# fpthink/3D-WSIS

Measured on AMD Instinct MI355X. Metric: scenes/sec fwd+bwd ScanNet 2cm (~150k voxels) @1/8 GPU; HBM GB/s vs roofline, higher is better.
Workload: dtype f32; 1 GPU; C2: 1 synthetic ScanNet-shaped scene on 1 GPU, 2 cm voxels, fwd+bwd+AdamW step (SubMConv3d UNet 32..160 + ECC GNN + edge affinity + MultiTaskLoss); per-batch segment CSRs / edge graph and all rulebooks are rebuilt inside every step; active_voxels=153685, points=199790, superpoints=2289, edges=20054, scenes_per_gpu=1, global_batch=1, parallelism=scene-sharded dp1

## Files before the change

### 3d-wsis_amd/csrc/bn.hip

```cpp
#include <cstdlib>
#include <initializer_list>

#include "common.h"

using namespace wsis;

namespace {

constexpr int BN_ROWS_PER_THREAD = 8;
__host__ __device__ inline int bn_rows_per_wg(int Cp) {
  const int G = Cp >> 2;
  const int R = 256 / G > 1 ? 256 / G : 1;
  return R * BN_ROWS_PER_THREAD;
}
constexpr int BN_THREADS = 256;

struct f4 {
  float v[4];
};
template <typename T>
__device__ __forceinline__ float4 bn_ld4(const T* p, int64_t t) {
  if constexpr (sizeof(T) == 4) {
    return reinterpret_cast<const float4*>(p)[t];
  } else {
// ... 191 lines not shown
    __syncthreads();
  }
}

template <typename T>
__global__ __launch_bounds__(BN_THREADS) void bn_stats_partial_kernel(const T* __restrict__ x, int64_t M, int C, int Cp,
                                                                      float* __restrict__ partial) {
  __shared__ float s_a[BN_THREADS * 4];
  __shared__ float s_b[BN_THREADS * 4];
  bn_partial_body(BnStatsAcc<T>{x}, M, C, Cp, partial, s_a, s_b);
}

template <typename T>
__global__ __launch_bounds__(BN_THREADS) void bn_bwd_partial_kernel(
    const T* __restrict__ x, const T* __restrict__ dy, const float* __restrict__ mean,
    const float* __restrict__ var, const float* __restrict__ gamma, const float* __restrict__ beta, float eps,
    int relu, int64_t M, int C, int Cp, float* __restrict__ partial) {
  __shared__ float s_a[BN_THREADS * 4];
  __shared__ float s_b[BN_THREADS * 4];
  bn_partial_body(BnBwdAcc<T>{x, dy, mean, var, gamma, beta, eps, relu}, M, C, Cp, partial, s_a, s_b);
}

__device__ __forceinline__ double wave_sum_f64(double v) {
#pragma unroll
  for (int off = 32; off >= 1; off >>= 1) v += __shfl_xor(v, off, 64);
  return v;
}
__device__ __forceinline__ void bn_final_sums(const float* __restrict__ partial, int nblk, int Cp, int c, double& A,
                                              double& B) {
  double a = 0.0, b = 0.0;
#pragma unroll 8
  for (int k = threadIdx.x; k < nblk; k += 64) {
    a += partial[(int64_t)k * 2 * Cp + c];
    b += partial[(int64_t)k * 2 * Cp + Cp + c];
  }
  A = wave_sum_f64(a);
  B = wave_sum_f64(b);
}

template <typename T>
__global__ __launch_bounds__(64) void bn_stats_final_kernel(const float* __restrict__ partial, int nblk, int C,
                                                            int Cp, int64_t M, const T* __restrict__ x0,
                                                            float* __restrict__ mean,
                                                            float* __restrict__ var,
                                                            float* __restrict__ running_mean,
                                                            float* __restrict__ running_var, float momentum) {
  const int c = blockIdx.x;
  double S, Q;
  bn_final_sums(partial, nblk, Cp, c, S, Q);
  if (threadIdx.x == 0)
    bn_store_stats(bn_shifted_mean_var(S, Q, bn_pivot(x0, M, C, c), M), M, c, mean, var, running_mean, running_var,
                   momentum);
}

__global__ __launch_bounds__(64) void bn_bwd_final_kernel(const float* __restrict__ partial, int nblk, int C, int Cp,
                                                          float* __restrict__ dgamma, float* __restrict__ dbeta) {
  const int c = blockIdx.x;
  double A, B;
  bn_final_sums(partial, nblk, Cp, c, A, B);
  if (threadIdx.x == 0) {
    dbeta[c] = (float)A;
    dgamma[c] = (float)B;
  }
}

int64_t bn_small_rows() {
  static const int64_t v = [] {
    const char* e = getenv("WSIS_BN_SMALL_ROWS");
    return e ? (int64_t)atoll(e) : (int64_t)4096;
  }();
  return v;
}
constexpr int BN_SMALL_THREADS = 1024;

__device__ __forceinline__ void block_sum2_f64(double (&a)[4], double (&b)[4], double* sh) {
  const int lane = threadIdx.x & 63, wave = threadIdx.x >> 6;
#pragma unroll
  for (int off = 32; off >= 1; off >>= 1) {
#pragma unroll
    for (int e = 0; e < 4; ++e) {
      a[e] += __shfl_xor(a[e], off, 64);
      b[e] += __shfl_xor(b[e], off, 64);
    }
  }
  if (lane == 0) {
#pragma unroll
    for (int e = 0; e < 4; ++e) {
      sh[wave * 8 + e] = a[e];
      sh[wave * 8 + 4 + e] = b[e];
    }
  }
  __syncthreads();
#pragma unroll
  for (int e = 0; e < 4; ++e) {
    double sa = 0.0, sb = 0.0;
    for (int w = 0; w < BN_SMALL_THREADS / 64; ++w) {
      sa += sh[w * 8 + e];
      sb += sh[w * 8 + 4 + e];
    }
    a[e] = sa;
    b[e] = sb;
  }
}

template <class Acc>
__device__ __forceinline__ void bn_small_body(Acc& acc, int64_t M, int C, int c0, double* sh, double (&a)[4],
                                              double (&b)[4]) {
  const bool vec = (C & 3) == 0;
  acc.init(M, C, c0);
  float sa[4] = {0.f, 0.f, 0.f, 0.f}, sb[4] = {0.f, 0.f, 0.f, 0.f};
#pragma unroll 8
  for (int64_t r = threadIdx.x; r < M; r += BN_SMALL_THREADS) acc.row(r, C, c0, vec, sa, sb);
#pragma unroll
  for (int e = 0; e < 4; ++e) {
    a[e] = sa[e];
    b[e] = sb[e];
  }
  block_sum2_f64(a, b, sh);
}

template <typename T>
__global__ __launch_bounds__(BN_SMALL_THREADS) void bn_stats_small_kernel(const T* __restrict__ x, int64_t M, int C,
                                                                    float* __restrict__ mean, float* __restrict__ var,
                                                                    float* __restrict__ running_mean,
                                                                    float* __restrict__ running_var, float momentum) {
  __shared__ double sh[BN_SMALL_THREADS / 64 * 8];
  const int c0 = blockIdx.x * 4;
  BnStatsAcc<T> acc{x};
  double a[4], b[4];
  bn_small_body(acc, M, C, c0, sh, a, b);
  const float K[4] = {acc.K[0], acc.K[1], acc.K[2], acc.K[3]};
  if (threadIdx.x < 4 && c0 + (int)threadIdx.x < C) {
    const int e = threadIdx.x;
    bn_store_stats(bn_shifted_mean_var(a[e], b[e], K[e], M), M, c0 + e, mean, var, running_mean, running_var, momentum);
  }
}

template <typename T>
__global__ __launch_bounds__(BN_SMALL_THREADS) void bn_bwd_small_kernel(
    const T* __restrict__ x, const T* __restrict__ dy, const float* __restrict__ mean,
    const float* __restrict__ var, const float* __restrict__ gamma, const float* __restrict__ beta, float eps,
    int relu, int64_t M, int C, float* __restrict__ dgamma, float* __restrict__ dbeta) {
  __shared__ double sh[BN_SMALL_THREADS / 64 * 8];
  const int c0 = blockIdx.x * 4;
  BnBwdAcc<T> acc{x, dy, mean, var, gamma, beta, eps, relu};
  double a[4], b[4];
  bn_small_body(acc, M, C, c0, sh, a, b);
  if (threadIdx.x < 4 && c0 + (int)threadIdx.x < C) {
    dbeta[c0 + threadIdx.x] = (float)a[threadIdx.x];
    dgamma[c0 + threadIdx.x] = (float)b[threadIdx.x];
  }
}

constexpr int BN_FIN_CHUNKS = kBnFinChunks;

template <int NT>
__device__ __forceinline__ void bn_chunk_walk(const float* __restrict__ partial, int lo, int hi, int C, int64_t M, int c,
                                              double (&t)[NT]) {
  const int pl = threadIdx.x >> 5;
  if (c < C) {
#pragma unroll 4
    for (int b = lo + pl; b < hi; b += 8) {
      const float sf = partial[(int64_t)b * 2 * C + c];
      const float qf = partial[(int64_t)b * 2 * C + C + c];
      const double si = sf;
      t[0] += si;
      t[1] += qf;
      if constexpr (NT == 3) {
        const int64_t left = M - (int64_t)b * 32;
        t[2] += si * si * (left < 32 ? 1.0 / (double)left : 0.03125);
      }
    }
  }
}
template <int NT>
__device__ __forceinline__ void bn_lane_fold(const double (&t)[NT], bool own, double (&red)[NT][8][33], double (&T)[NT]) {
  const int cl = threadIdx.x & 31, pl = threadIdx.x >> 5;
#pragma unroll
  for (int k = 0; k < NT; ++k) red[k][pl][cl] = t[k];
  __syncthreads();
#pragma unroll
  for (int k = 0; k < NT; ++k) T[k] = 0.0;
  if (own) {
#pragma unroll
    for (int j = 0; j < 8; ++j)
#pragma unroll
      for (int k = 0; k < NT; ++k) T[k] += red[k][j][cl];
  }
}
__device__ __forceinline__ void bn_chunk_range(int nblk, int G, int g, int& lo, int& hi) {
  const int per = (nblk + G - 1) / G;
  lo = g * per;
  hi = lo + per < nblk ? lo + per : nblk;
}

template <int NT>
__device__ __forceinline__ bool bn_ticket_sum(double* __restrict__ chunk, unsigned* __restrict__ ticket, int g0, int G,
                                              int cgi, int C, int c, bool own, double (&T)[NT],
                                              double (&red)[NT][8][33], int& s_last) {
  if (own) {
    double* o = chunk + (int64_t)g0 * NT * C;
#pragma unroll
    for (int k = 0; k < NT; ++k) st_sc1(o + k * C + c, T[k]);
  }
  if (!ticket) return false;
  wait_stores_left();
  __syncthreads();
  if (threadIdx.x == 0) {
    const unsigned t = atomicAdd(ticket + cgi, 1u);
    s_last = t == (unsigned)G - 1;
    if (s_last) ticket[cgi] = 0u;
  }
  __syncthreads();
  if (!s_last) return false;
  double t2[NT];
#pragma unroll
  for (int k = 0; k < NT; ++k) t2[k] = 0.0;
  if (c < C)
    for (int g = threadIdx.x >> 5; g < G; g += 8) {
      const double* o = chunk + (int64_t)g * NT * C;
#pragma unroll
      for (int k = 0; k < NT; ++k) t2[k] += ld_sc1(o + k * C + c);
    }
  __syncthreads();
  bn_lane_fold<NT>(t2, own, red, T);
  return true;
}

template <int NT, class Finish>
__device__ __forceinline__ bool bn_chunk_stage(const float* __restrict__ partial, int nblk, int C, int64_t M,
                                               double* __restrict__ chunk, unsigned* __restrict__ ticket, int g0, int G,
                                               int cgi, double (&red)[NT][8][33], int& s_last, Finish finish) {
  const int c = cgi * 32 + (threadIdx.x & 31);
  const bool own = (threadIdx.x >> 5) == 0 && c < C;
  int lo, hi;
  bn_chunk_range(nblk, G, g0, lo, hi);
  double t[NT], T[NT];
#pragma unroll
  for (int k = 0; k < NT; ++k) t[k] = 0.0;
  bn_chunk_walk<NT>(partial, lo, hi, C, M, c, t);
  bn_lane_fold<NT>(t, own, red, T);
  if (G > 1 && !bn_ticket_sum<NT>(chunk, ticket, g0, G, cgi, C, c, own, T, red, s_last)) return false;
  if (own) finish(c, T);
  return true;
}

__device__ __forceinline__ bool bn_chunk_centred_stage(const float* __restrict__ partial, int nblk, int C, int64_t M,
                                                       double* __restrict__ chunk, float* __restrict__ mean,
                                                       float* __restrict__ var, float* __restrict__ running_mean,
                                                       float* __restrict__ running_var, float momentum,
                                                       unsigned* __restrict__ ticket, int g0, int G, int cgi,
                                                       double (&red)[3][8][33], int& s_last) {
  return bn_chunk_stage<3>(partial, nblk, C, M, chunk, ticket, g0, G, cgi, red, s_last, [&](int c, const double (&T)[3]) {
    bn_finish_centred(T[0], T[1], T[2], M, c, mean, var, running_mean, running_var, momentum);
  });
}
__device__ __forceinline__ bool bn_sum_chunk_stage(const float* __restrict__ partial, int nblk, int C,
                                                   double* __restrict__ chunk, float* dbeta, float* dgamma,
                                                   unsigned* __restrict__ ticket, int g0, int G, int cgi,
                                                   double (&red)[2][8][33], int& s_last) {
  return bn_chunk_stage<2>(partial, nblk, C, 0, chunk, ticket, g0, G, cgi, red, s_last, [&](int c, const double (&T)[2]) {
    dbeta[c] = (float)T[0];
    dgamma[c] = (float)T[1];
  });
}

__global__ __launch_bounds__(256) void bn_stats_chunk_centred_kernel(const float* __restrict__ partial, int nblk, int C,
                                                                     int64_t M, double* __restrict__ chunk,
                                                                     float* __restrict__ mean, float* __restrict__ var,
                                                                     float* __restrict__ running_mean,
                                                                     float* __restrict__ running_var, float momentum,
                                                                     unsigned* __restrict__ ticket) {
  __shared__ double red[3][8][33];
  __shared__ int s_last;
  bn_chunk_centred_stage(partial, nblk, C, M, chunk, mean, var, running_mean, running_var, momentum, ticket,
                         (int)blockIdx.x, (int)gridDim.x, (int)blockIdx.y, red, s_last);
}
__global__ __launch_bounds__(256) void bn_sum_chunk_kernel(const float* __restrict__ partial, int nblk, int C,
                                                           double* __restrict__ chunk, float* __restrict__ dbeta,
                                                           float* __restrict__ dgamma, unsigned* __restrict__ ticket) {
  __shared__ double red[2][8][33];
  __shared__ int s_last;
  bn_sum_chunk_stage(partial, nblk, C, chunk, dbeta, dgamma, ticket, (int)blockIdx.x, (int)gridDim.x, (int)blockIdx.y, red,
                     s_last);
}

__global__ __launch_bounds__(256) void bn_stats_final_centred_kernel(const double* __restrict__ chunk, int G, int C,
                                                                     int64_t M, float* __restrict__ mean,
                                                                     float* __restrict__ var,
                                                                     float* __restrict__ running_mean,
                                                                     float* __restrict__ running_var, float momentum) {
  const int lane = threadIdx.x & 63;
  const int c = blockIdx.x * 4 + (threadIdx.x >> 6);
  if (c >= C) return;
  const bool in = lane < G;
  const double S = wave_sum_f64(in ? chunk[(int64_t)lane * 3 * C + c] : 0.0);
  const double Q = wave_sum_f64(in ? chunk[(int64_t)lane * 3 * C + C + c] : 0.0);
  const double W = wave_sum_f64(in ? chunk[(int64_t)lane * 3 * C + 2 * C + c] : 0.0);
  if (lane == 0) bn_finish_centred(S, Q, W, M, c, mean, var, running_mean, running_var, momentum);
}
__global__ __launch_bounds__(256) void bn_sum_final_kernel(const double* __restrict__ chunk, int G, int C,
                                                           float* __restrict__ dbeta, float* __restrict__ dgamma) {
  const int lane = threadIdx.x & 63;
  const int c = blockIdx.x * 4 + (threadIdx.x >> 6);
  if (c >= C) return;
  const bool in = lane < G;
  const double A = wave_sum_f64(in ? chunk[(int64_t)lane * 2 * C + c] : 0.0);
  const double B = wave_sum_f64(in ? chunk[(int64_t)lane * 2 * C + C + c] : 0.0);
  if (lane == 0) {
    dbeta[c] = (float)A;
    dgamma[c] = (float)B;
  }
}


template <bool COHERENT>
__device__ __forceinline__ float bn_ld_stat(const float* p) {
  if (COHERENT) return __hip_atomic_load(p, __ATOMIC_RELAXED, __HIP_MEMORY_SCOPE_AGENT);
  return *p;
}

template <bool COHERENT, typename TI = float, typename TO = float>
__device__ __forceinline__ void bn_apply_body(const TI* __restrict__ x, const float* mean,
                                              const float* var, const float* __restrict__ gamma,
                                              const float* __restrict__ beta, float eps, int relu,
                                              TO* __restrict__ y, int64_t M, int C) {
  const int64_t total = M * C;
  if ((C & 3) == 0) {
    const int64_t total4 = total >> 2;
    const unsigned C4 = (unsigned)(C >> 2);
    const int64_t stride = (int64_t)gridDim.x * blockDim.x;
    int64_t t = blockIdx.x * (int64_t)blockDim.x + threadIdx.x;
    const bool fixed_c = (stride % C4) == 0;
    unsigned cg = (unsigned)(t % C4);
    float sc[4], mu[4], bt[4];
    auto coef = [&](unsigned g) {
#pragma unroll
      for (int e = 0; e < 4; ++e) {
        const int c = (int)g * 4 + e;
        sc[e] = bn_fwd_coef(gamma ? gamma[c] : 1.0f, bn_ld_stat<COHERENT>(var + c), eps);
        mu[e] = bn_ld_stat<COHERENT>(mean + c);
        bt[e] = beta ? beta[c] : 0.0f;
      }
    };
    coef(cg);
    auto body = [&](const float4 v) {
      float o[4] = {v.x, v.y, v.z, v.w};
#pragma unroll
      for (int e = 0; e < 4; ++e) o[e] = bn_fwd_elem(o[e], mu[e], sc[e], bt[e], relu);
      return make_float4(o[0], o[1], o[2], o[3]);
    };
    if (fixed_c) {
      for (; t + stride < total4; t += 2 * stride) {
        const float4 v0 = bn_ld4(x, t);
        const float4 v1 = bn_ld4(x, t + stride);
        bn_st4(y, t, body(v0));
        bn_st4(y, t + stride, body(v1));
      }
      if (t < total4) bn_st4(y, t, body(bn_ld4(x, t)));
    } else {
      for (; t < total4; t += stride) {
        cg = (unsigned)(t % C4);
        coef(cg);
        bn_st4(y, t, body(bn_ld4(x, t)));
      }
    }
  } else {
    for (int64_t t = blockIdx.x * (int64_t)blockDim.x + threadIdx.x; t < total;
         t += (int64_t)gridDim.x * blockDim.x) {
      const int c = (int)(t % C);
      const float sc = bn_fwd_coef(gamma ? gamma[c] : 1.0f, bn_ld_stat<COHERENT>(var + c), eps);
      y[t] = (TO)bn_fwd_elem((float)x[t], bn_ld_stat<COHERENT>(mean + c), sc, beta ? beta[c] : 0.0f, relu);
    }
  }
}

__global__ void bn_apply_kernel(const float* __restrict__ x, const float* __restrict__ mean,
                                const float* __restrict__ var, const float* __restrict__ gamma,
                                const float* __restrict__ beta, float eps, int relu, float* __restrict__ y,
                                int64_t M, int C) {
  bn_apply_body<false>(x, mean, var, gamma, beta, eps, relu, y, M, C);
}

template <typename TI, typename TO>
__global__ void bn_apply_lp_kernel(const TI* __restrict__ x, const float* __restrict__ mean,
                                   const float* __restrict__ var, const float* __restrict__ gamma,
                                   const float* __restrict__ beta, float eps, int relu, TO* __restrict__ y, int64_t M,
                                   int C) {
  bn_apply_body<false, TI, TO>(x, mean, var, gamma, beta, eps, relu, y, M, C);
}

template <typename TI>
void launch_bn_apply_lp(const void* x, const float* mean, const float* var, const float* gamma, const float* beta,
                        float eps, int relu, void* y, int out_fp32, int64_t M, int C, int grid, hipStream_t st) {
  if (out_fp32)
    hipLaunchKernelGGL((bn_apply_lp_kernel<TI, float>), dim3(grid), dim3(256), 0, st, static_cast<const TI*>(x), mean,
                       var, gamma, beta, eps, relu, static_cast<float*>(y), M, C);
  else
    hipLaunchKernelGGL((bn_apply_lp_kernel<TI, TI>), dim3(grid), dim3(256), 0, st, static_cast<const TI*>(x), mean, var,
                       gamma, beta, eps, relu, static_cast<TI*>(y), M, C);
}

template <bool COHERENT, typename T, typename TO>
__device__ __forceinline__ void bn_bwd_apply_body(const T* __restrict__ x, const T* __restrict__ dy,
                                                  const float* __restrict__ mean, const float* __restrict__ var,
                                                  const float* __restrict__ gamma, const float* __restrict__ beta,
                                                  const float* dgamma, const float* dbeta,
                                                  const T* __restrict__ addend, float eps, int relu, int training,
                                                  TO* __restrict__ dx, int64_t M, int C) {
  const int64_t total = M * C;
  const float inv_m = 1.0f / (float)M;
  const bool vec = (C & 3) == 0;
  const int W = vec ? 4 : 1;
  const int64_t totalw = total / W;
  const unsigned Cw = (unsigned)(C / W);
  const int64_t stride = (int64_t)gridDim.x * blockDim.x;
  int64_t t = blockIdx.x * (int64_t)blockDim.x + threadIdx.x;
  const bool fixed_c = (stride % Cw) == 0;
  BnBwdCoef k;
  float k1[4], k2[4];
  auto coef = [&](int c0) {
#pragma unroll
    for (int e = 0; e < 4; ++e) {
      if (e < W) {
        const int c = c0 + e;
        k.load(e, c, mean, var, gamma, beta, eps);
        k1[e] = training ? bn_ld_stat<COHERENT>(dbeta + c) * inv_m : 0.0f;
        k2[e] = training ? bn_ld_stat<COHERENT>(dgamma + c) * inv_m : 0.0f;
      }
    }
  };
  if (t < totalw) coef((int)(t % Cw) * W);
  auto one = [&](const float (&xv)[4], const float (&dv)[4], const float (&av)[4], float (&ov)[4]) {
#pragma unroll
    for (int e = 0; e < 4; ++e) {
      if (e < W)
        ov[e] = bn_bwd_dx(bn_bwd_elem(xv[e], dv[e], k, e, relu), k, e, k1[e], k2[e], training, addend != nullptr, av[e]);
    }
  };
  if (vec && fixed_c) {
    for (; t + stride < totalw; t += 2 * stride) {
      const int64_t u = t + stride;
      const f4 tx0 = ld4(x + t * 4, true), td0 = ld4(dy + t * 4, true);
      const f4 tx1 = ld4(x + u * 4, true), td1 = ld4(dy + u * 4, true);
      f4 ta0, ta1;
#pragma unroll
      for (int e = 0; e < 4; ++e) ta0.v[e] = ta1.v[e] = 0.f;
      if (addend) {
        ta0 = ld4(addend + t * 4, true);
        ta1 = ld4(addend + u * 4, true);
      }
      float o0[4], o1[4];
      one(tx0.v, td0.v, ta0.v, o0);
      one(tx1.v, td1.v, ta1.v, o1);
      bn_st4(dx, t, make_float4(o0[0], o0[1], o0[2], o0[3]));
      bn_st4(dx, u, make_float4(o1[0], o1[1], o1[2], o1[3]));
    }
  }
  for (; t < totalw; t += stride) {
    if (!fixed_c) coef((int)(t % Cw) * W);
    float xv[4], dv[4], av[4] = {0.f, 0.f, 0.f, 0.f}, ov[4];
    if (vec) {
      const f4 tx = ld4(x + t * 4, true), td = ld4(dy + t * 4, true);
#pragma unroll
      for (int e = 0; e < 4; ++e) {
        xv[e] = tx.v[e];
        dv[e] = td.v[e];
      }
      if (addend) {
        const f4 ta = ld4(addend + t * 4, true);
#pragma unroll
        for (int e = 0; e < 4; ++e) av[e] = ta.v[e];
      }
    } else {
      xv[0] = (float)x[t];
      dv[0] = (float)dy[t];
      if (addend) av[0] = (float)addend[t];
    }
    one(xv, dv, av, ov);
    if (vec)
      bn_st4(dx, t, make_float4(ov[0], ov[1], ov[2], ov[3]));
    else
      dx[t] = (TO)ov[0];
  }
}

template <typename T, typename TO>
__global__ void bn_bwd_apply_kernel(const T* __restrict__ x, const T* __restrict__ dy,
                                    const float* __restrict__ mean, const float* __restrict__ var,
                                    const float* __restrict__ gamma, const float* __restrict__ beta,
                                    const float* __restrict__ dgamma, const float* __restrict__ dbeta,
                                    const T* __restrict__ addend, float eps, int relu, int training,
                                    TO* __restrict__ dx, int64_t M, int C) {
  bn_bwd_apply_body<false>(x, dy, mean, var, gamma, beta, dgamma, dbeta, addend, eps, relu, training, dx, M, C);
}

constexpr int BN_SF_ROWS = 256;

template <int NT>
__device__ __forceinline__ void bn_small_totals(const float* __restrict__ partial, int nblk, int C, int64_t M, int G, int c,
                                                bool own, double (&red)[NT][8][33], double (&T)[NT]) {
#pragma unroll
  for (int k = 0; k < NT; ++k) T[k] = 0.0;
  for (int g = 0; g < G; ++g) {
    int lo, hi;
    bn_chunk_range(nblk, G, g, lo, hi);
    double t[NT], Tg[NT];
#pragma unroll
    for (int k = 0; k < NT; ++k) t[k] = 0.0;
    bn_chunk_walk<NT>(partial, lo, hi, C, M, c, t);
    if (g) __syncthreads();
    bn_lane_fold<NT>(t, own, red, Tg);
    if (own) {
#pragma unroll
      for (int k = 0; k < NT; ++k) {
        if (G == 1)
          T[k] = Tg[k];
        else
          T[k] += Tg[k];
      }
    }
  }
}

__global__ __launch_bounds__(256) void bn_small_finish_apply_kernel(
    const float* __restrict__ partial, int nblk, int C, int64_t M, float* __restrict__ mean, float* __restrict__ var,
    float* __restrict__ running_mean, float* __restrict__ running_var, float momentum, const float* __restrict__ x,
    const float* __restrict__ gamma, const float* __restrict__ beta, float eps, int relu, float* __restrict__ y, int G) {
  __shared__ double red[3][8][33];
  __shared__ float s_mu[32], s_sc[32], s_bt[32];
  const int cgi = blockIdx.y;
  const int cl = threadIdx.x & 31;
  const int c = cgi * 32 + cl;
  const bool own = (threadIdx.x >> 5) == 0 && c < C;
  double T[3];
  bn_small_totals<3>(partial, nblk, C, M, G, c, own, red, T);
  if (own) {
    const BnMeanVar s = bn_centred_mean_var(T[0], T[1], T[2], M);
    if (blockIdx.x == 0) bn_store_stats(s, M, c, mean, var, running_mean, running_var, momentum);
    s_mu[cl] = (float)s.mu;
    s_sc[cl] = bn_fwd_coef(gamma ? gamma[c] : 1.0f, (float)s.v, eps);
    s_bt[cl] = beta ? beta[c] : 0.0f;
  }
  __syncthreads();
  const int q4 = threadIdx.x & 7, rl = threadIdx.x >> 3;
  const int c4 = cgi * 32 + q4 * 4;
  if (c4 >= C) return;
  float mu4[4], sc4[4], bt4[4];
#pragma unroll
  for (int e = 0; e < 4; ++e) {
    mu4[e] = s_mu[q4 * 4 + e];
    sc4[e] = s_sc[q4 * 4 + e];
    bt4[e] = s_bt[q4 * 4 + e];
  }
  const int64_t r0 = (int64_t)blockIdx.x * BN_SF_ROWS;
#pragma unroll 4
  for (int it = 0; it < BN_SF_ROWS / 32; ++it) {
    const int64_t r = r0 + it * 32 + rl;
    if (r < M) {
      const float4 vx = *reinterpret_cast<const float4*>(x + r * C + c4);
      float o[4] = {vx.x, vx.y, vx.z, vx.w};
#pragma unroll
      for (int e = 0; e < 4; ++e) o[e] = bn_fwd_elem(o[e], mu4[e], sc4[e], bt4[e], relu);
      *reinterpret_cast<float4*>(y + r * C + c4) = make_float4(o[0], o[1], o[2], o[3]);
    }
  }
}

__global__ __launch_bounds__(256) void bn_small_bwd_finish_apply_kernel(
    const float* __restrict__ partial, int nblk, int C, int64_t M, const float* __restrict__ x,
    const float* __restrict__ dy, const float* __restrict__ mean, const float* __restrict__ var,
    const float* __restrict__ gamma, const float* __restrict__ beta, const float* __restrict__ addend, float eps, int relu,
    float* __restrict__ dx, float* __restrict__ dgamma, float* __restrict__ dbeta, int G) {
  __shared__ double red[2][8][33];
  __shared__ float s_k1[32], s_k2[32];
  const int cgi = blockIdx.y;
  const int cl = threadIdx.x & 31;
  const int c = cgi * 32 + cl;
  const bool own = (threadIdx.x >> 5) == 0 && c < C;
  double T[2];
  bn_small_totals<2>(partial, nblk, C, M, G, c, own, red, T);
  if (own) {
    const float db = (float)T[0], dg = (float)T[1];
    if (blockIdx.x == 0) {
      dbeta[c] = db;
      dgamma[c] = dg;
    }
    const float inv_m = 1.0f / (float)M;
    s_k1[cl] = db * inv_m;
    s_k2[cl] = dg * inv_m;
  }
  __syncthreads();
  const int q4 = threadIdx.x & 7, rl = threadIdx.x >> 3;
  const int c4 = cgi * 32 + q4 * 4;
  if (c4 >= C) return;
  BnBwdCoef k;
  float k1[4], k2[4];
#pragma unroll
  for (int e = 0; e < 4; ++e) {
    k.load(e, c4 + e, mean, var, gamma, beta, eps);
    k1[e] = s_k1[q4 * 4 + e];
    k2[e] = s_k2[q4 * 4 + e];
  }
  const int64_t r0 = (int64_t)blockIdx.x * BN_SF_ROWS;
#pragma unroll 2
  for (int it = 0; it < BN_SF_ROWS / 32; ++it) {
    const int64_t r = r0 + it * 32 + rl;
    if (r < M) {
      const float4 vx = *reinterpret_cast<const float4*>(x + r * C + c4);
      const float4 vd = *reinterpret_cast<const float4*>(dy + r * C + c4);
      float4 va = make_float4(0.f, 0.f, 0.f, 0.f);
      if (addend) va = *reinterpret_cast<const float4*>(addend + r * C + c4);
      const float xv[4] = {vx.x, vx.y, vx.z, vx.w}, dv[4] = {vd.x, vd.y, vd.z, vd.w}, av[4] = {va.x, va.y, va.z, va.w};
      float ov[4];
#pragma unroll
      for (int e = 0; e < 4; ++e)
        ov[e] = bn_bwd_dx(bn_bwd_elem(xv[e], dv[e], k, e, relu), k, e, k1[e], k2[e], 1, addend != nullptr, av[e]);
      *reinterpret_cast<float4*>(dx + r * C + c4) = make_float4(ov[0], ov[1], ov[2], ov[3]);
    }
  }
}

static int bn_small_gmax() {
  const char* e = getenv("WSIS_BN_SMALL_G");
  const int g = e ? atoi(e) : 4;
  return g < 1 ? 1 : g > 8 ? 8 : g;
}
static bool bn_small_fused_on() {
  const char* e = getenv("WSIS_BN_SMALL_FUSED");
  return !e || atoi(e) != 0;
}

int bn_nblk(int64_t M, int Cp) { return (int)ceil_div(M > 0 ? M : 1, (int64_t)bn_rows_per_wg(Cp)); }

#if WSIS_EXPERIMENTAL
constexpr int BN_POLL_SLEEP = 12;
constexpr unsigned long long BN_SPIN_LIMIT = 200000000ull;

__device__ __forceinline__ void bn_wait_published(SyncSlot* s) {
  if (threadIdx.x == 0) {
    const unsigned long long t0 = __builtin_amdgcn_s_memrealtime();
    while (__hip_atomic_load(&s->flag, __ATOMIC_RELAXED, __HIP_MEMORY_SCOPE_AGENT) == 0u) {
      __builtin_amdgcn_s_sleep(BN_POLL_SLEEP);
      if (__builtin_amdgcn_s_memrealtime() - t0 > BN_SPIN_LIMIT) {
        __hip_atomic_store(&s->err, 1u, __ATOMIC_RELAXED, __HIP_MEMORY_SCOPE_AGENT);
        break;
      }
    }
    const unsigned l = atomicAdd(&s->left, 1u);
    if (l == gridDim.x - 1) {
      __hip_atomic_store(&s->left, 0u, __ATOMIC_RELAXED, __HIP_MEMORY_SCOPE_AGENT);
      __hip_atomic_store(&s->flag, 0u, __ATOMIC_RELAXED, __HIP_MEMORY_SCOPE_AGENT);
    }
  }
  __syncthreads();
}
__device__ __forceinline__ void bn_publish(bool fin, SyncSlot* s, int CG) {
  if (!fin) return;
  __threadfence();
  __syncthreads();
  if (threadIdx.x == 0) {
    const unsigned d = atomicAdd(&s->done, 1u);
    if (d == (unsigned)CG - 1) {
      __hip_atomic_store(&s->done, 0u, __ATOMIC_RELAXED, __HIP_MEMORY_SCOPE_AGENT);
      __threadfence();
      __hip_atomic_store(&s->flag, 1u, __ATOMIC_RELEASE, __HIP_MEMORY_SCOPE_AGENT);
    }
  }
}

__global__ __launch_bounds__(256) void bn_finalize_apply_kernel(
    const float* __restrict__ partial, int nblk, int C, int64_t M, double* __restrict__ chunk, int G,
    float* mean, float* var, float* __restrict__ running_mean,
    float* __restrict__ running_var, float momentum, SyncSlot* __restrict__ sync, const float* __restrict__ x,
    const float* __restrict__ gamma, const float* __restrict__ beta, float eps, int relu, float* __restrict__ y) {
  __shared__ double red[3][8][33];
  __shared__ int s_last;
  const int CG = (C + 31) / 32;
  if ((int)blockIdx.x < G * CG)
    bn_publish(bn_chunk_centred_stage(partial, nblk, C, M, chunk, mean, var, running_mean, running_var, momentum,
                                      sync->ticket, (int)blockIdx.x % G, G, (int)blockIdx.x / G, red, s_last),
               sync, CG);
  bn_wait_published(sync);
  bn_apply_body<true>(x, mean, var, gamma, beta, eps, relu, y, M, C);
}

__global__ __launch_bounds__(256) void bn_bwd_finish_apply_kernel(
    const float* __restrict__ partial, int nblk, int C, double* __restrict__ chunk, int G, float* dbeta, float* dgamma,
    SyncSlot* __restrict__ sync, const float* __restrict__ x, const float* __restrict__ dy, const float* __restrict__ mean,
    const float* __restrict__ var, const float* __restrict__ gamma, const float* __restrict__ beta,
    const float* __restrict__ addend, float eps, int relu, float* __restrict__ dx, int64_t M) {
  __shared__ double red[2][8][33];
  __shared__ int s_last;
  const int CG = (C + 31) / 32;
  if ((int)blockIdx.x < G * CG)
    bn_publish(bn_sum_chunk_stage(partial, nblk, C, chunk, dbeta, dgamma, sync->ticket, (int)blockIdx.x % G, G,
                                  (int)blockIdx.x / G, red, s_last),
               sync, CG);
  bn_wait_published(sync);
  bn_bwd_apply_body<true>(x, dy, mean, var, gamma, beta, dgamma, dbeta, addend, eps, relu, 1, dx, M, C);
}

static int bn_fused_grid(int64_t M, int C, int need_chunk_wgs, int which = 0) {
  const char* e = getenv("WSIS_BN_FUSED_APPLY");
  const int on = e ? atoi(e) : 0;
  const char* ed = getenv(which ? "WSIS_BN_FUSED_BWD" : "WSIS_BN_FUSED_FWD");
  const int on_dir = ed ? atoi(ed) : on;
  const char* g = tune_env("WSIS_BN_FUSED_GRID");
  int gmax = g ? atoi(g) : 256;
  if (gmax < 64 || gmax > 512) gmax = 256;
  int n_cu = 0;
  {
    int dev = 0, v = 0;
    n_cu = (hipGetDevice(&dev) == hipSuccess &&
            hipDeviceGetAttribute(&v, hipDeviceAttributeMultiprocessorCount, dev) == hipSuccess) ? v : 0;
  }
  if (!on_dir || (C & 3) != 0) return 0;
  const int cw = C >> 2;
  const int64_t work = (M * C) >> 2;
  int gcap = (work > 600000 && gmax == 256) ? 512 : gmax;
  if (gcap > 2 * n_cu) gcap = 2 * n_cu;
  if (gcap < 1) return 0;
  int grid = gcap - (gcap % cw);
  const int need = grid_for(work, 256);
  if (need < grid) {
    grid = need;
    if (grid > cw) grid -= grid % cw;
  }
  return (grid >= need_chunk_wgs && grid >= 1) ? grid : 0;
}
#endif


static int bn_apply_grid(int64_t M, int C) {
  const bool vec = (C & 3) == 0;
  const int64_t work = vec ? (M * C) >> 2 : M * C;
  const int cw = vec ? C >> 2 : C;
  int64_t g = ceil_div(work, (int64_t)256 * 8);
  if (g < 512) {
    g = ceil_div(work, 256);
    if (g > 512) g = 512;
  }
  if (g > 16384) g = 16384;
  if (g < 1) g = 1;
  if (g > cw) g -= g % cw;
  return (int)g;
}

template <typename T, typename TO>
static int launch_bn_bwd_apply(const T* d_x, const T* d_dy, const float* d_mean, const float* d_var,
                               const float* d_gamma, const float* d_beta, const float* d_dgamma, const float* d_dbeta,
                               const T* d_addend, float eps, int relu, int training, TO* d_dx, int64_t M, int C,
                               hipStream_t st) {
  hipLaunchKernelGGL((bn_bwd_apply_kernel<T, TO>), dim3(bn_apply_grid(M, C)), dim3(256), 0, st, d_x, d_dy, d_mean, d_var,
                     d_gamma, d_beta, d_dgamma, d_dbeta, d_addend, eps, relu, training, d_dx, M, C);
  WSIS_LAUNCH_CHECK();
  return WSIS_OK;
}

template <typename T>
static int bn_stats_run(const T* d_x, int64_t M, int C, float* d_mean, float* d_var, float* d_running_mean,
                        float* d_running_var, float momentum, void* d_ws, hipStream_t st) {
  const int Cp = (C + 3) / 4 * 4;
  const int nblk = bn_nblk(M, Cp);
  float* partial = static_cast<float*>(d_ws);
  WSIS_REQUIRE(Cp / 4 <= BN_THREADS, "C > 1024 is not supported");
  if (M <= bn_small_rows()) {
    hipLaunchKernelGGL(bn_stats_small_kernel<T>, dim3(Cp / 4), dim3(BN_SMALL_THREADS), 0, st, d_x, M, C, d_mean, d_var,
                       d_running_mean, d_running_var, momentum);
    WSIS_LAUNCH_CHECK();
    return WSIS_OK;
  }
  hipLaunchKernelGGL(bn_stats_partial_kernel<T>, dim3(nblk), dim3(BN_THREADS), 0, st, d_x, M, C, Cp, partial);
  WSIS_LAUNCH_CHECK();
  hipLaunchKernelGGL(bn_stats_final_kernel<T>, dim3(C), dim3(64), 0, st, partial, nblk, C, Cp, M, d_x, d_mean, d_var,
                     d_running_mean, d_running_var, momentum);
  WSIS_LAUNCH_CHECK();
  return WSIS_OK;
}
template <typename T>
static int bn_bwd_reduce_run(const T* d_x, const T* d_dy, const float* d_mean, const float* d_var, const float* d_gamma,
                             const float* d_beta, float eps, int relu, float* d_dgamma, float* d_dbeta, int64_t M, int C,
                             void* d_ws, hipStream_t st) {
  const int Cp = (C + 3) / 4 * 4;
  const int nblk = bn_nblk(M, Cp);
  float* partial = static_cast<float*>(d_ws);
  WSIS_REQUIRE(Cp / 4 <= BN_THREADS, "C > 1024 is not supported");
  if (M <= bn_small_rows()) {
    hipLaunchKernelGGL(bn_bwd_small_kernel<T>, dim3(Cp / 4), dim3(BN_SMALL_THREADS), 0, st, d_x, d_dy, d_mean, d_var,
                       d_gamma, d_beta, eps, relu, M, C, d_dgamma, d_dbeta);
    WSIS_LAUNCH_CHECK();
  } else {
    hipLaunchKernelGGL(bn_bwd_partial_kernel<T>, dim3(nblk), dim3(BN_THREADS), 0, st, d_x, d_dy, d_mean, d_var, d_gamma,
                       d_beta, eps, relu, M, C, Cp, partial);
    WSIS_LAUNCH_CHECK();
    hipLaunchKernelGGL(bn_bwd_final_kernel, dim3(C), dim3(64), 0, st, partial, nblk, C, Cp, d_dgamma, d_dbeta);
    WSIS_LAUNCH_CHECK();
  }
  return WSIS_OK;
}
template <typename T>
static int bn_bwd_apply_lp_run(const void* d_x, const void* d_dy, const float* d_mean, const float* d_var,
                               const float* d_gamma, const float* d_beta, const float* d_dgamma, const float* d_dbeta,
                               const void* d_addend, float eps, int relu, int training, void* d_dx, int out_fp32, int64_t M,
                               int C, hipStream_t st) {
  const T *x = static_cast<const T*>(d_x), *dy = static_cast<const T*>(d_dy), *ad = static_cast<const T*>(d_addend);
  if (out_fp32)
    return launch_bn_bwd_apply(x, dy, d_mean, d_var, d_gamma, d_beta, d_dgamma, d_dbeta, ad, eps, relu, training,
                               static_cast<float*>(d_dx), M, C, st);
  return launch_bn_bwd_apply(x, dy, d_mean, d_var, d_gamma, d_beta, d_dgamma, d_dbeta, ad, eps, relu, training,
                             static_cast<T*>(d_dx), M, C, st);
}
template <typename T>
static int bn_bwd_lp_run(const void* d_x, const void* d_dy, const float* d_mean, const float* d_var, const float* d_gamma,
                         const float* d_beta, float eps, int relu, int training, void* d_dx, int out_fp32,
                         float* d_dgamma, float* d_dbeta, const void* d_addend, int64_t M, int C, void* d_ws,
                         hipStream_t st) {
  const int rc = bn_bwd_reduce_run(static_cast<const T*>(d_x), static_cast<const T*>(d_dy), d_mean, d_var, d_gamma, d_beta,
                                   eps, relu, d_dgamma, d_dbeta, M, C, d_ws, st);
  if (rc != WSIS_OK || !d_dx) return rc;
  return bn_bwd_apply_lp_run<T>(d_x, d_dy, d_mean, d_var, d_gamma, d_beta, d_dgamma, d_dbeta, d_addend, eps, relu, training,
                                d_dx, out_fp32, M, C, st);
}

static unsigned* bn_tickets(void* d_sync) {
  static const int on = [] {
    const char* e = tune_env("WSIS_BN_TICKET");
    return e ? atoi(e) : 1;
  }();
  if (!on || !d_sync) return nullptr;
  return static_cast<SyncSlot*>(d_sync)->ticket;
}

static bool bn_aligned16(std::initializer_list<const void*> ps) {
  for (const void* p : ps)
    if (reinterpret_cast<uintptr_t>(p) & 15) return false;
  return true;
}
static void* bn_align256(void* p) {
  return reinterpret_cast<void*>((reinterpret_cast<uintptr_t>(p) + 255) & ~(uintptr_t)255);
}

struct BnCentredPlan {
  int G, CG;
  bool ws_ok;
  double* chunk;
  unsigned* tickets;
};
static BnCentredPlan bn_centred_plan(int64_t n_part, int C, void* d_ws, int64_t ws_bytes, void* d_sync) {
  BnCentredPlan p;
  p.G = bn_fin_chunks(n_part);
  p.CG = (C + 31) / 32;
  p.ws_ok = p.G == 1 || (d_ws && ws_bytes >= wsis_bn_stats_finalize_workspace_bytes(n_part, C));
  p.chunk = static_cast<double*>(bn_align256(d_ws));
  p.tickets = bn_tickets(d_sync);
  return p;
}
static bool bn_small_fused_ok(const BnCentredPlan& p, int C, std::initializer_list<const void*> rows) {
  return p.G <= bn_small_gmax() && (p.G == 1 || p.tickets) && (C & 3) == 0 && bn_small_fused_on() && bn_aligned16(rows);
}

constexpr int BN_SYNC_THREADS = 64;

__global__ __launch_bounds__(BN_SYNC_THREADS) void bn_sync_pack_kernel(const float* __restrict__ mean,
                                                                       const float* __restrict__ var, int64_t M, int C,
                                                                       double* __restrict__ out) {
  const int c = blockIdx.x * BN_SYNC_THREADS + threadIdx.x;
  if (c >= C) return;
  out[c] = M > 0 ? (double)mean[c] : 0.0;
  out[C + c] = M > 0 ? (double)var[c] : 0.0;
  if (c == 0) out[2 * C] = (double)M;
}

__global__ __launch_bounds__(BN_SYNC_THREADS) void bn_sync_combine_kernel(const double* __restrict__ g, int R, int C,
                                                                          float* __restrict__ mean, float* __restrict__ var,
                                                                          float* __restrict__ running_mean,
                                                                          float* __restrict__ running_var, float momentum,
                                                                          double* __restrict__ count) {
  const int c = blockIdx.x * BN_SYNC_THREADS + threadIdx.x;
  if (c >= C) return;
  const int64_t P = 2 * (int64_t)C + 1;
  double N = g[2 * C];
  for (int r = 1; r < R; ++r) N += g[r * P + 2 * C];
  if (c == 0) count[0] = N;
  if (!(N > 0.0)) {
    mean[c] = 0.0f;
    var[c] = 0.0f;
    return;
  }
  double s = g[c] * g[2 * C];
  for (int r = 1; r < R; ++r) s += g[r * P + c] * g[r * P + 2 * C];
  const double mean64 = s / N;
  double q = 0.0;
  for (int r = 0; r < R; ++r) {
    const double dm = g[r * P + c] - mean64;
    const double t = (g[r * P + C + c] + dm * dm) * g[r * P + 2 * C];
    q = r == 0 ? t : q + t;
  }
  const double var64 = q / N;
  const float m32 = (float)mean64;
  mean[c] = m32;
  var[c] = (float)var64;
  if (running_mean) {
    const double n1 = N - 1.0 > 1.0 ? N - 1.0 : 1.0;
    running_mean[c] = (1.0f - momentum) * running_mean[c] + momentum * m32;
    running_var[c] = (1.0f - momentum) * running_var[c] + momentum * (float)(var64 * N / n1);
// ... 54 lines not shown
  if (dtype == 0)
    return bn_stats_run(static_cast<const __bf16*>(d_x), M, C, d_mean, d_var, d_running_mean, d_running_var, momentum,
                        d_ws, st);
  return bn_stats_run(static_cast<const _Float16*>(d_x), M, C, d_mean, d_var, d_running_mean, d_running_var, momentum,
                      d_ws, st);
}


__device__ __forceinline__ void colsum_block(const bool IN, const bool OUT, const float* __restrict__ x, int64_t lo,
                                             int64_t hi, int C4, float4* red, float* __restrict__ out) {
  const int RL = 256 / C4;
  const int cl = threadIdx.x % C4, rl = threadIdx.x / C4;
  float4 a = {0.f, 0.f, 0.f, 0.f};
  if (rl < RL) {
    const float4* x4 = reinterpret_cast<const float4*>(x);
#pragma unroll 8
    for (int64_t r = lo + rl; r < hi; r += RL) {
      float4 v;
      if (IN) {
        const float* p = x + (r * C4 + cl) * 4;
        v = make_float4(ld_sc1(p), ld_sc1(p + 1), ld_sc1(p + 2), ld_sc1(p + 3));
      } else {
        v = x4[r * C4 + cl];
      }
      a.x += v.x;
      a.y += v.y;
      a.z += v.z;
      a.w += v.w;
    }
    red[rl * C4 + cl] = a;
  }
  __syncthreads();
  if (threadIdx.x < C4) {
    float4 s = red[threadIdx.x];
    for (int j = 1; j < RL; ++j) {
      const float4 v = red[j * C4 + threadIdx.x];
      s.x += v.x;
      s.y += v.y;
      s.z += v.z;
      s.w += v.w;
    }
    if (OUT) {
      float* p = out + threadIdx.x * 4;
      st_sc1(p, s.x);
      st_sc1(p + 1, s.y);
      st_sc1(p + 2, s.z);
      st_sc1(p + 3, s.w);
    } else {
      reinterpret_cast<float4*>(out)[threadIdx.x] = s;
    }
  }
}

__global__ __launch_bounds__(256) void colsum_kernel(const float* __restrict__ x, int64_t M, int C, int64_t per,
                                                     float* __restrict__ chunk, float* __restrict__ out,
                                                     unsigned* __restrict__ ticket) {
  __shared__ float4 red[256];
  __shared__ int s_last;
  const int C4 = C >> 2;
  const int64_t lo = (int64_t)blockIdx.x * per;
  const int64_t hi = lo + per < M ? lo + per : M;
  if (gridDim.x == 1) {
    colsum_block(false, false, x, lo, hi, C4, red, out);
    return;
  }
  colsum_block(false, true, x, lo, hi, C4, red, chunk + (int64_t)blockIdx.x * C);
  wait_stores_left();
  __syncthreads();
  if (threadIdx.x == 0) {
    const unsigned t = atomicAdd(ticket, 1u);
    s_last = t == gridDim.x - 1;
    if (s_last) *ticket = 0u;
  }
  __syncthreads();
  if (!s_last) return;
  __syncthreads();
  colsum_block(true, false, chunk, 0, gridDim.x, C4, red, out);
}

static void colsum_plan(int64_t M, int64_t* per, int64_t* G) {
  *per = (M + 127) / 128;
  if (*per < 256) *per = 256;
  *G = (M + *per - 1) / *per;
}

int64_t wsis_bn_stats_finalize_workspace_bytes(int64_t n_part, int32_t C) {
  return (int64_t)bn_fin_chunks(n_part) * 3 * C * (int64_t)sizeof(double) + 256;
}

int wsis_bn_stats_finalize(const float* d_partials, int64_t n_part, int64_t M, int32_t C, float* d_mean, float* d_var,
                           float* d_running_mean, float* d_running_var, float momentum, void* d_ws, int64_t ws_bytes,
                           void* d_sync, void* stream) {
  WSIS_REQUIRE(n_part >= 1 && M >= 1 && C >= 1 && d_partials && d_mean && d_var, "bad args");
  WSIS_REQUIRE(n_part < ((int64_t)1 << 31), "too many partials");
  WSIS_REQUIRE((d_running_mean == nullptr) == (d_running_var == nullptr), "running stats come in pairs");
  WSIS_REQUIRE(n_part == (M + 31) / 32, "one partial per 32-row slice");
  const BnCentredPlan p = bn_centred_plan(n_part, C, d_ws, ws_bytes, d_sync);
  WSIS_REQUIRE(p.ws_ok, "workspace too small");
  WSIS_REQUIRE(C <= 512, "more than 512 channels");
  hipLaunchKernelGGL(bn_stats_chunk_centred_kernel, dim3(p.G, p.CG), dim3(256), 0, as_stream(stream), d_partials,
                     (int)n_part, C, M, p.chunk, d_mean, d_var, d_running_mean, d_running_var, momentum, p.tickets);
  WSIS_LAUNCH_CHECK();
  if (p.G > 1 && !p.tickets) {
    hipLaunchKernelGGL(bn_stats_final_centred_kernel, dim3((C + 3) / 4), dim3(256), 0, as_stream(stream), p.chunk, p.G, C,
                       M, d_mean, d_var, d_running_mean, d_running_var, momentum);
    WSIS_LAUNCH_CHECK();
  }
  return WSIS_OK;
}

int wsis_bn_stats_finalize_apply(const float* d_partials, int64_t n_part, int64_t M, int32_t C, float* d_mean,
                                 float* d_var, float* d_running_mean, float* d_running_var, float momentum,
                                 const float* d_x, const float* d_gamma, const float* d_beta, float eps, int32_t relu,
                                 float* d_y, void* d_ws, int64_t ws_bytes, void* d_sync, void* stream) {
  WSIS_REQUIRE(n_part >= 1 && M >= 1 && C >= 1 && d_partials && d_mean && d_var && d_x && d_y, "bad args");
  WSIS_REQUIRE(n_part == (M + 31) / 32 && n_part < ((int64_t)1 << 31), "one partial per 32-row slice");
  WSIS_REQUIRE(C <= 512, "more than 512 channels");
  hipStream_t st = as_stream(stream);
  const BnCentredPlan p = bn_centred_plan(n_part, C, d_ws, ws_bytes, d_sync);
  WSIS_REQUIRE(p.ws_ok, "workspace too small");
  if (bn_small_fused_ok(p, C, {d_x, d_y})) {
    hipLaunchKernelGGL(bn_small_finish_apply_kernel, dim3((unsigned)ceil_div(M, BN_SF_ROWS), (unsigned)p.CG), dim3(256), 0,
                       st, d_partials, (int)n_part, (int)C, M, d_mean, d_var, d_running_mean, d_running_var, momentum, d_x,
                       d_gamma, d_beta, eps, (int)relu, d_y, p.G);
    WSIS_LAUNCH_CHECK();
    return WSIS_OK;
  }
#if WSIS_EXPERIMENTAL
  if (const int grid = p.tickets ? bn_fused_grid(M, C, p.G * p.CG) : 0) {
    hipLaunchKernelGGL(bn_finalize_apply_kernel, dim3(grid), dim3(256), 0, st, d_partials, (int)n_part, (int)C, M, p.chunk,
                       p.G, d_mean, d_var, d_running_mean, d_running_var, momentum, static_cast<SyncSlot*>(d_sync), d_x,
                       d_gamma, d_beta, eps, (int)relu, d_y);
    WSIS_LAUNCH_CHECK();
    return WSIS_OK;
  }
#endif
  const int rc = wsis_bn_stats_finalize(d_partials, n_part, M, C, d_mean, d_var, d_running_mean, d_running_var, momentum,
                                        d_ws, ws_bytes, d_sync, stream);
  if (rc != WSIS_OK) return rc;
  return wsis_bn_apply(d_x, d_mean, d_var, d_gamma, d_beta, eps, relu, d_y, M, C, stream);
}

int wsis_bn_apply(const float* d_x, const float* d_mean, const float* d_var, const float* d_gamma,
                  const float* d_beta, float eps, int32_t relu, float* d_y, int64_t M, int32_t C, void* stream) {
  WSIS_REQUIRE(M >= 0 && C >= 1, "bad sizes");
  if (M == 0) return WSIS_OK;
  WSIS_REQUIRE(d_x && d_mean && d_var && d_y, "null pointer");
  hipLaunchKernelGGL(bn_apply_kernel, dim3(bn_apply_grid(M, C)), dim3(256), 0, as_stream(stream), d_x, d_mean, d_var,
                     d_gamma, d_beta, eps, relu, d_y, M, C);
  WSIS_LAUNCH_CHECK();
  return WSIS_OK;
}

int wsis_bn_apply_lp(const void* d_x, const float* d_mean, const float* d_var, const float* d_gamma,
                     const float* d_beta, float eps, int32_t relu, void* d_y, int32_t out_fp32, int64_t M, int32_t C,
                     int32_t dtype, void* stream) {
  WSIS_REQUIRE(M >= 0 && C >= 1, "bad sizes");
  WSIS_REQUIRE(dtype == 0 || dtype == 1, "dtype must be 0 (bf16) or 1 (fp16)");
  if (M == 0) return WSIS_OK;
  WSIS_REQUIRE(d_x && d_mean && d_var && d_y, "null pointer");
  const int grid = bn_apply_grid(M, C);
  if ((C & 3) == 0)
    WSIS_REQUIRE((reinterpret_cast<uintptr_t>(d_x) & 7) == 0 &&
                     (reinterpret_cast<uintptr_t>(d_y) & (out_fp32 ? 15 : 7)) == 0,
                 "x and y must be aligned to a quad of elements");
  hipStream_t st = as_stream(stream);
  if (dtype == 0)
    launch_bn_apply_lp<__bf16>(d_x, d_mean, d_var, d_gamma, d_beta, eps, relu, d_y, out_fp32, M, C, grid, st);
  else
    launch_bn_apply_lp<_Float16>(d_x, d_mean, d_var, d_gamma, d_beta, eps, relu, d_y, out_fp32, M, C, grid, st);
  WSIS_LAUNCH_CHECK();
  return WSIS_OK;
}

int wsis_bn_bwd_from_partials(const float* d_partials, int64_t n_part, const float* d_x, const float* d_dy,
                              const float* d_mean, const float* d_var, const float* d_gamma, const float* d_beta,
                              float eps, int32_t relu, float* d_dx, float* d_dgamma, float* d_dbeta,
                              const float* d_addend, int64_t M, int32_t C, void* d_ws, int64_t ws_bytes, void* d_sync,
                              void* stream) {
  WSIS_REQUIRE(M >= 1 && C >= 1 && d_partials && d_x && d_dy && d_mean && d_var && d_dgamma && d_dbeta, "bad args");
  WSIS_REQUIRE(n_part == (M + 31) / 32 && n_part < ((int64_t)1 << 31), "one partial per 32-row slice");
  const BnCentredPlan p = bn_centred_plan(n_part, C, d_ws, ws_bytes, d_sync);
  WSIS_REQUIRE(p.ws_ok, "workspace too small");
  hipStream_t st = as_stream(stream);
  WSIS_REQUIRE(C <= 512, "more than 512 channels");
  if (d_dx && bn_small_fused_ok(p, C, {d_x, d_dy, d_dx, d_addend})) {
    hipLaunchKernelGGL(bn_small_bwd_finish_apply_kernel, dim3((unsigned)ceil_div(M, BN_SF_ROWS), (unsigned)p.CG), dim3(256),
                       0, st, d_partials, (int)n_part, (int)C, M, d_x, d_dy, d_mean, d_var, d_gamma, d_beta, d_addend, eps,
                       (int)relu, d_dx, d_dgamma, d_dbeta, p.G);
    WSIS_LAUNCH_CHECK();
    return WSIS_OK;
  }
#if WSIS_EXPERIMENTAL
  if (const int grid = d_dx && p.tickets ? bn_fused_grid(M, C, p.G * p.CG, 1) : 0) {
    hipLaunchKernelGGL(bn_bwd_finish_apply_kernel, dim3(grid), dim3(256), 0, st, d_partials, (int)n_part, (int)C, p.chunk,
                       p.G, d_dbeta, d_dgamma, static_cast<SyncSlot*>(d_sync), d_x, d_dy, d_mean, d_var, d_gamma, d_beta,
                       d_addend, eps, (int)relu, d_dx, M);
    WSIS_LAUNCH_CHECK();
    return WSIS_OK;
  }
#endif
  hipLaunchKernelGGL(bn_sum_chunk_kernel, dim3(p.G, p.CG), dim3(256), 0, st, d_partials, (int)n_part, C, p.chunk, d_dbeta,
                     d_dgamma, p.tickets);
  WSIS_LAUNCH_CHECK();
  if (p.G > 1 && !p.tickets) {
    hipLaunchKernelGGL(bn_sum_final_kernel, dim3((C + 3) / 4), dim3(256), 0, st, p.chunk, p.G, C, d_dbeta, d_dgamma);
    WSIS_LAUNCH_CHECK();
  }
  if (!d_dx) return WSIS_OK;
  return launch_bn_bwd_apply(d_x, d_dy, d_mean, d_var, d_gamma, d_beta, d_dgamma, d_dbeta, d_addend, eps, relu, 1, d_dx, M,
                             C, st);
}

int wsis_bn_bwd_apply(const float* d_x, const float* d_dy, const float* d_mean, const float* d_var,
                      const float* d_gamma, const float* d_beta, const float* d_sum_dz_xhat, const float* d_sum_dz,
                      float eps, int32_t relu, float* d_dx, const float* d_addend, int64_t M, int32_t C, void* stream) {
  WSIS_REQUIRE(M >= 1 && C >= 1 && d_x && d_dy && d_mean && d_var && d_sum_dz_xhat && d_sum_dz && d_dx, "bad args");
  return launch_bn_bwd_apply(d_x, d_dy, d_mean, d_var, d_gamma, d_beta, d_sum_dz_xhat, d_sum_dz, d_addend, eps, relu, 1,
                             d_dx, M, C, as_stream(stream));
}

int wsis_bn_bwd(const float* d_x, const float* d_dy, const float* d_mean, const float* d_var,
                const float* d_gamma, const float* d_beta, float eps, int32_t relu, int32_t training,
                float* d_dx, float* d_dgamma, float* d_dbeta, const float* d_addend, int64_t M, int32_t C, void* d_ws,
                int64_t ws_bytes, void* stream) {
  WSIS_REQUIRE(M >= 1 && C >= 1 && d_x && d_dy && d_mean && d_var && d_dgamma && d_dbeta && d_ws, "bad args");
  WSIS_REQUIRE(ws_bytes >= wsis_bn_workspace_bytes(M, C), "workspace too small");
  hipStream_t st = as_stream(stream);
  const int rc = bn_bwd_reduce_run(d_x, d_dy, d_mean, d_var, d_gamma, d_beta, eps, relu, d_dgamma, d_dbeta, M, C, d_ws, st);
  if (rc != WSIS_OK || !d_dx) return rc;
  return launch_bn_bwd_apply(d_x, d_dy, d_mean, d_var, d_gamma, d_beta, d_dgamma, d_dbeta, d_addend, eps, relu, training,
                             d_dx, M, C, st);
}

int wsis_bn_bwd_lp(const void* d_x, const void* d_dy, const float* d_mean, const float* d_var, const float* d_gamma,
                   const float* d_beta, float eps, int32_t relu, int32_t training, void* d_dx, int32_t out_fp32,
                   float* d_dgamma, float* d_dbeta, const void* d_addend, int64_t M, int32_t C, int32_t dtype, void* d_ws,
                   int64_t ws_bytes, void* stream) {
  WSIS_REQUIRE(M >= 1 && C >= 1 && d_x && d_dy && d_mean && d_var && d_dgamma && d_dbeta && d_ws, "bad args");
  WSIS_REQUIRE(bn_lp_domain(C, dtype, {d_x, d_dy, d_dx, d_addend}),
               "16-bit BatchNorm: dtype 0 / 1, C % 8 == 0, C <= 1024, 16-byte aligned tensors");
  WSIS_REQUIRE(ws_bytes >= wsis_bn_workspace_bytes(M, C), "workspace too small");
  hipStream_t st = as_stream(stream);
  if (dtype == 0)
    return bn_bwd_lp_run<__bf16>(d_x, d_dy, d_mean, d_var, d_gamma, d_beta, eps, relu, training, d_dx, out_fp32, d_dgamma,
                                 d_dbeta, d_addend, M, C, d_ws, st);
  return bn_bwd_lp_run<_Float16>(d_x, d_dy, d_mean, d_var, d_gamma, d_beta, eps, relu, training, d_dx, out_fp32, d_dgamma,
                                 d_dbeta, d_addend, M, C, d_ws, st);
}

int wsis_bn_bwd_apply_lp(const void* d_x, const void* d_dy, const float* d_mean, const float* d_var, const float* d_gamma,
                         const float* d_beta, const float* d_sum_dz_xhat, const float* d_sum_dz, float eps, int32_t relu,
                         void* d_dx, int32_t out_fp32, const void* d_addend, int64_t M, int32_t C, int32_t dtype,
                         void* stream) {
  WSIS_REQUIRE(M >= 1 && C >= 1 && d_x && d_dy && d_mean && d_var && d_sum_dz_xhat && d_sum_dz && d_dx, "bad args");
  WSIS_REQUIRE(bn_lp_domain(C, dtype, {d_x, d_dy, d_dx, d_addend}),
               "16-bit BatchNorm: dtype 0 / 1, C % 8 == 0, C <= 1024, 16-byte aligned tensors");
  hipStream_t st = as_stream(stream);
  if (dtype == 0)
    return bn_bwd_apply_lp_run<__bf16>(d_x, d_dy, d_mean, d_var, d_gamma, d_beta, d_sum_dz_xhat, d_sum_dz, d_addend, eps,
                                       relu, 1, d_dx, out_fp32, M, C, st);
  return bn_bwd_apply_lp_run<_Float16>(d_x, d_dy, d_mean, d_var, d_gamma, d_beta, d_sum_dz_xhat, d_sum_dz, d_addend, eps,
                                       relu, 1, d_dx, out_fp32, M, C, st);
}

int wsis_bn_sync_pack(const float* d_mean, const float* d_var, int64_t M, int32_t C, double* d_out, void* stream) {
  WSIS_REQUIRE(M >= 0 && C >= 1 && d_out && (M == 0 || (d_mean && d_var)), "bad args");
  hipLaunchKernelGGL(bn_sync_pack_kernel, dim3(bn_sync_grid(C)), dim3(BN_SYNC_THREADS), 0, as_stream(stream), d_mean, d_var,
                     M, (int)C, d_out);
  WSIS_LAUNCH_CHECK();
  return WSIS_OK;
}

int wsis_bn_sync_combine(const double* d_gathered, int32_t R, int32_t C, float* d_mean, float* d_var,
                         float* d_running_mean, float* d_running_var, float momentum, double* d_count, void* stream) {
  WSIS_REQUIRE(R >= 1 && C >= 1 && d_gathered && d_mean && d_var && d_count, "bad args");
  WSIS_REQUIRE((d_running_mean == nullptr) == (d_running_var == nullptr), "running stats come in pairs");
  hipLaunchKernelGGL(bn_sync_combine_kernel, dim3(bn_sync_grid(C)), dim3(BN_SYNC_THREADS), 0, as_stream(stream), d_gathered,
                     (int)R, (int)C, d_mean, d_var, d_running_mean, d_running_var, momentum, d_count);
  WSIS_LAUNCH_CHECK();
  return WSIS_OK;
}

int wsis_bn_sync_sums_pack(const float* d_dgamma, const float* d_dbeta, int32_t C, double* d_out, void* stream) {
  WSIS_REQUIRE(C >= 1 && d_out, "bad args");
  hipLaunchKernelGGL(bn_sync_sums_pack_kernel, dim3(bn_sync_grid(C)), dim3(BN_SYNC_THREADS), 0, as_stream(stream), d_dgamma,
                     d_dbeta, (int)C, d_out);
  WSIS_LAUNCH_CHECK();
  return WSIS_OK;
}

int wsis_bn_sync_sums_scale(const double* d_sums, int64_t M, const double* d_count, int32_t C, float* d_sum_dz_xhat,
                            float* d_sum_dz, void* stream) {
  WSIS_REQUIRE(M >= 0 && C >= 1 && d_sums && d_count && d_sum_dz_xhat && d_sum_dz, "bad args");
  hipLaunchKernelGGL(bn_sync_sums_scale_kernel, dim3(bn_sync_grid(C)), dim3(BN_SYNC_THREADS), 0, as_stream(stream), d_sums, M,
                     d_count, (int)C, d_sum_dz_xhat, d_sum_dz);
  WSIS_LAUNCH_CHECK();
  return WSIS_OK;
}

int64_t wsis_sync_bytes(void) { return (int64_t)kSyncSlotsTotal * (int64_t)sizeof(SyncSlot); }

int64_t wsis_colsum_workspace_bytes(int64_t M, int32_t C) {
  if (M < 0 || C < 4) return -1;
  int64_t per, G;
  colsum_plan(M, &per, &G);
  return (G > 1 ? G : 1) * (int64_t)C * (int64_t)sizeof(float) + 256;
}

int wsis_colsum(const float* d_x, int64_t M, int32_t C, float* d_out, void* d_ws, int64_t ws_bytes, void* d_sync,
                void* stream) {
  WSIS_REQUIRE(M >= 0 && C >= 4 && C % 4 == 0 && C <= 1024 && d_out, "colsum: C must be a multiple of 4, <= 1024");
  hipStream_t st = as_stream(stream);
  if (M == 0) {
    WSIS_HIP_CHECK(hipMemsetAsync(d_out, 0, sizeof(float) * (size_t)C, st));
    return WSIS_OK;
  }
  WSIS_REQUIRE(d_x && bn_aligned16({d_x, d_out}), "colsum: 16-byte alignment");
  int64_t per, G;
  colsum_plan(M, &per, &G);
  float* chunk = nullptr;
  unsigned* ticket = nullptr;
  if (G > 1) {
    WSIS_REQUIRE(d_ws && ws_bytes >= wsis_colsum_workspace_bytes(M, C), "workspace too small");
    chunk = static_cast<float*>(bn_align256(d_ws));
    WSIS_REQUIRE(d_sync, "colsum over more than one chunk needs a sync slot");
    ticket = static_cast<SyncSlot*>(d_sync)->ticket;
  }
  hipLaunchKernelGGL(colsum_kernel, dim3((unsigned)G), dim3(256), 0, st, d_x, M, (int)C, per, chunk, d_out, ticket);
  WSIS_LAUNCH_CHECK();
  return WSIS_OK;
}

}
```

### 3d-wsis_amd/csrc/executor.hip

```cpp
#include <condition_variable>
#include <cstdlib>
#include <deque>
#include <map>
#include <mutex>
#include <string>
#include <thread>
#include <utility>
#include <vector>

#include <unistd.h>

#include <algorithm>

#include "common.h"
#if WSIS_EXPERIMENTAL
#include "deep.h"
#endif

using namespace wsis;

namespace {

constexpr int64_t ALIGN = 256;
inline int64_t up(int64_t v) { return (v + ALIGN - 1) / ALIGN * ALIGN; }
// ... 121 lines not shown
  bool pending_join = false;
  hipStream_t stream = nullptr;
  hipEvent_t join = nullptr;
  hipEvent_t mark_main = nullptr, mark_side = nullptr;
  hipEvent_t wt_fork = nullptr, wt_done = nullptr;
  std::vector<hipEvent_t> fork;
  size_t next = 0;
};

SideStream* side_stream_for(hipStream_t main) {
  static std::mutex mu;
  static std::map<std::pair<int, hipStream_t>, SideStream> pool;
  int dev = 0;
  if (hipGetDevice(&dev) != hipSuccess) return nullptr;
  std::lock_guard<std::mutex> lock(mu);
  SideStream& s = pool[std::make_pair(dev, main)];
  if (!s.stream) {
    if (hipStreamCreateWithFlags(&s.stream, hipStreamNonBlocking) != hipSuccess) return nullptr;
    if (hipEventCreateWithFlags(&s.join, hipEventDisableTiming) != hipSuccess) return nullptr;
    if (hipEventCreateWithFlags(&s.mark_main, hipEventDisableTiming) != hipSuccess) return nullptr;
    if (hipEventCreateWithFlags(&s.mark_side, hipEventDisableTiming) != hipSuccess) return nullptr;
    if (hipEventCreateWithFlags(&s.wt_fork, hipEventDisableTiming) != hipSuccess) return nullptr;
    if (hipEventCreateWithFlags(&s.wt_done, hipEventDisableTiming) != hipSuccess) return nullptr;
  }
  return &s;
}

hipEvent_t next_fork_event(SideStream* s) {
  if (s->next == s->fork.size()) {
    hipEvent_t e = nullptr;
    if (hipEventCreateWithFlags(&e, hipEventDisableTiming) != hipSuccess) return nullptr;
    s->fork.push_back(e);
  }
  return s->fork[s->next++];
}

struct DwTask {
  std::thread::id owner;
  wsis_op op;
  hipEvent_t ev;
  int dev;
  hipStream_t side;
  char* ws;
  int64_t ws_bytes;
  DwRedRec* rec = nullptr;
  const DwRedRec* flush = nullptr;
  int flush_n = 0;
};
static int issue_dw_raw(const wsis_op& op, char* dw_ws, int64_t dw_bytes, void* dw_stream) {
  if (op.flags & WSIS_OPF_LP)
    return wsis_spconv_dw_lp(op.in[0], (const int32_t*)op.in[3], (const int32_t*)op.in[4], op.in[2], (float*)op.out[1],
                             op.M_in, op.M_out, op.K, op.Cin, op.Cout, op.reserved, dw_ws, dw_bytes, dw_stream);
  if (op.flags & WSIS_OPF_BN_IN)
    return wsis_spconv_dw_bn((const float*)op.in[0], (const float*)op.in[7], (const float*)op.in[8], (const float*)op.in[9],
                             (const float*)op.in[10], op.eps, (op.flags & WSIS_OPF_RELU) ? 1 : 0, (const int32_t*)op.in[5],
                             (const int32_t*)op.in[6], (op.flags & WSIS_OPF_FLIP) ? 1 : 0, (const float*)op.in[2],
                             (float*)op.out[1], op.M_in, op.M_out, op.K, op.Cin, op.Cout, dw_ws, dw_bytes, dw_stream);
  return wsis_spconv_dw((const float*)op.in[0], (const int32_t*)op.in[3], (const int32_t*)op.in[4], (const float*)op.in[2],
                        (float*)op.out[1], op.M_in, op.M_out, op.K, op.Cin, op.Cout, dw_ws, dw_bytes, dw_stream);
}
int issue_dw(const wsis_op& op, char* dw_ws, int64_t dw_bytes, void* dw_stream, DwRedRec* rec = nullptr) {
  if (rec) *rec = DwRedRec{};
  dw2_set_defer(rec);
  const int rc = issue_dw_raw(op, dw_ws, dw_bytes, dw_stream);
  dw2_set_defer(nullptr);
  return rc;
}
class DwWorker {
 public:
  void push(DwTask t) {
    std::lock_guard<std::mutex> lock(mu_);
    const long pid = (long)getpid();
    if (started_ && pid_ != pid) {
      started_ = false;
      q_.clear();
      st_.clear();
    }
    if (!started_) {
      started_ = true;
      pid_ = pid;
      std::thread(&DwWorker::run, this).detach();
    }
    t.owner = std::this_thread::get_id();
    q_.push_back(t);
    ++st_[t.owner].pending;
    cv_.notify_one();
  }
  int drain(std::string* msg) {
    const std::thread::id me = std::this_thread::get_id();
    std::unique_lock<std::mutex> lock(mu_);
    done_.wait(lock, [&] { return st_[me].pending == 0; });
    State& s = st_[me];
    const int rc = s.err;
    if (rc != WSIS_OK && msg) *msg = s.msg;
    s.err = WSIS_OK;
    s.msg.clear();
    return rc;
  }

 private:
  struct State {
    int pending = 0, err = WSIS_OK;
    std::string msg;
  };
  void run() {
    for (;;) {
      DwTask t;
      {
        std::unique_lock<std::mutex> lock(mu_);
        cv_.wait(lock, [this] { return !q_.empty(); });
        t = q_.front();
        q_.pop_front();
      }
      int rc = WSIS_OK;
      std::string msg;
      hipError_t he = hipSetDevice(t.dev);
      if (he == hipSuccess && t.ev) he = hipStreamWaitEvent(t.side, t.ev, 0);
      if (he != hipSuccess) {
        rc = WSIS_ERR_HIP;
        msg = std::string("dW worker: ") + hipGetErrorString(he);
      } else {
        rc = t.flush ? dw2_reduce_batch(t.flush, t.flush_n, t.side) : issue_dw(t.op, t.ws, t.ws_bytes, t.side, t.rec);
        if (rc != WSIS_OK) msg = wsis_last_error();
      }
      std::lock_guard<std::mutex> lock(mu_);
      State& s = st_[t.owner];
      if (rc != WSIS_OK && s.err == WSIS_OK) {
        s.err = rc;
        s.msg = msg;
      }
      if (--s.pending == 0) done_.notify_all();
    }
  }
  std::mutex mu_;
  std::condition_variable cv_, done_;
  std::deque<DwTask> q_;
  std::map<std::thread::id, State> st_;
  bool started_ = false;
  long pid_ = 0;
};
DwWorker& dw_worker() {
  static DwWorker* w = new DwWorker();
  return *w;
}
struct PassOptions {
  bool fwd2;
  bool dw_stream;
  bool dw_thread;
  bool dw_batch_reduce;
  bool dw_tail_main;
  bool wt_side;
  bool dw_early;
  bool slab_bn_partials;
  bool prof;
  bool capturing;
  bool dw_defer() const { return dw_batch_reduce && !prof; }
};
inline bool env_flag(const char* e, bool dflt) { return e ? atoi(e) != 0 : dflt; }
PassOptions read_pass_options(const hipStream_t* st) {
  PassOptions o;
  o.fwd2 = env_flag(getenv("WSIS_FWD2"), true);
  o.dw_stream = env_flag(getenv("WSIS_DW_STREAM"), true);
  o.dw_thread = env_flag(tune_env("WSIS_DW_THREAD"), true);
  o.dw_batch_reduce = env_flag(getenv("WSIS_DW_BATCH_REDUCE"), false);
  o.dw_tail_main = env_flag(getenv("WSIS_DW_TAIL_MAIN"), true);
  o.wt_side = env_flag(getenv("WSIS_WT_SIDE"), true);
  const char* rows = getenv("WSIS_DW_EARLY_ROWS");
  o.dw_early = env_flag(getenv("WSIS_DW_EARLY"), dw2_batch_rows() < (rows ? atoll(rows) : 500000));
  o.slab_bn_partials = env_flag(getenv("WSIS_SLAB_BN_PARTIALS"), false);
  o.prof = g_prof_on;
  hipStreamCaptureStatus cs = hipStreamCaptureStatusNone;
  o.capturing = st && (hipStreamIsCapturing(*st, &cs) != hipSuccess || cs != hipStreamCaptureStatusNone);
  return o;
}
inline bool dw_tail_on_main(const wsis_op* ops, int n, int i) {
  return i == n - 1 && ops[i].kind == WSIS_OP_CONV_BWD && ops[i].out[1] && !ops[i].out[0];
}

inline int64_t wt_bytes_of(const wsis_op& op) {
  return up((int64_t)op.K * op.Cin * op.Cout * (int64_t)sizeof(float));
}

inline bool use_fwd2(const wsis_op& op, bool on) {
  const int64_t gathered = op.kind == WSIS_OP_CONV ? op.M_in * op.Cin : op.M_out * op.Cout;
  return on && wsis_spconv_fwd_t_supported(op.K, op.Cin, op.Cout) != 0 && gathered * 4 < ((int64_t)1 << 31);
}
inline bool needs_wt(const wsis_op& op, bool on) {
  if (op.flags & WSIS_OPF_LP) return false;
  if (op.kind == WSIS_OP_CONV) return use_fwd2(op, on);
  if (op.kind == WSIS_OP_CONV_BWD) return op.out[0] != nullptr && !use_fwd2(op, on);
  return false;
}

inline bool is_lp(const wsis_op& op) { return (op.flags & WSIS_OPF_LP) != 0; }
inline bool is_lp_conv(const wsis_op& op) {
  return is_lp(op) && (op.kind == WSIS_OP_CONV || (op.kind == WSIS_OP_CONV_BWD && op.out[0]));
}
inline int64_t lp_wt_bytes_of(const wsis_op& op) { return up((int64_t)op.K * op.Cin * op.Cout * 2); }
inline bool lp_below_2g(int64_t rows, int C) { return rows * C * 2 < ((int64_t)1 << 31); }
const char* lp_refusal(const wsis_op& op) {
  if (op.kind == WSIS_OP_CAST_LP && !is_lp(op)) return "CAST_LP without WSIS_OPF_LP (its dtype)";
  if (!is_lp(op)) return (op.flags & WSIS_OPF_LP_TRAIN) ? "WSIS_OPF_LP_TRAIN without WSIS_OPF_LP" : nullptr;
  const bool train_form = (op.kind == WSIS_OP_BN_RELU && (op.flags & WSIS_OPF_TRAINING)) || op.kind == WSIS_OP_BN_RELU_BWD ||
                          op.kind == WSIS_OP_CONV_BWD || op.kind == WSIS_OP_SPLIT;
  if (train_form && !(op.flags & WSIS_OPF_LP_TRAIN))
    return "16-bit training form (training BatchNorm, CONV_BWD, BN_RELU_BWD, SPLIT) without WSIS_OPF_LP_TRAIN";
  if (op.reserved != 0 && op.reserved != 1) return "16-bit op with a dtype other than 0 (bf16) or 1 (fp16)";
  if (op.flags & (WSIS_OPF_BN_IN | WSIS_OPF_STAT_FIN | WSIS_OPF_STATS))
    return "16-bit op with a fused BatchNorm form or epilogue statistics (16-bit passes run every BatchNorm as an op)";
  switch (op.kind) {
    case WSIS_OP_CONV:
      if (!wsis_spconv_lp_supported(op.K, op.Cin, op.Cout))
        return "16-bit convolution outside wsis_spconv_lp_supported (channels multiples of 32, at most 512)";
      if (op.M_in * op.Cin * 2 >= ((int64_t)1 << 31)) return "16-bit convolution input of 2 GiB or more";
      if (!op.in[3]) return "16-bit convolution without weights";
      return nullptr;
    case WSIS_OP_BN_RELU:
      if (!op.out[0]) return "16-bit BatchNorm without output";
      if (op.flags & WSIS_OPF_TRAINING) {
        if (!op.out[1] || !op.out[2]) return "16-bit training BatchNorm without mean / var outputs";
        if (op.Cin % 8 != 0 || op.Cin > 1024) return "16-bit training BatchNorm outside C % 8 == 0, C <= 1024";
        if ((op.flags & WSIS_OPF_UPDATE_RUNNING) && (!op.in[3] || !op.in[4]))
          return "16-bit BatchNorm updates running statistics it does not have";
        return nullptr;
      }
      if (op.flags & WSIS_OPF_UPDATE_RUNNING) return "16-bit evaluation BatchNorm with WSIS_OPF_UPDATE_RUNNING";
      if (!op.in[3] || !op.in[4]) return "16-bit evaluation BatchNorm without running statistics";
      return nullptr;
    case WSIS_OP_BN_RELU_BWD:
      if (op.Cin % 8 != 0 || op.Cin > 1024) return "16-bit BatchNorm backward outside C % 8 == 0, C <= 1024";
      if (!op.in[0] || !op.in[1] || !op.in[2] || !op.in[3] || !op.out[1] || !op.out[2])
        return "16-bit BatchNorm backward without x, dy, statistics or parameter-gradient outputs";
      return nullptr;
    case WSIS_OP_CAT:
    case WSIS_OP_SPLIT:
      if ((op.Cin | op.Cout) & 1) return "16-bit concatenation / split of an odd channel count";
      return nullptr;
    case WSIS_OP_CAST_LP:
      return nullptr;
    case WSIS_OP_CONV_BWD:
      if (!op.in[0] || !op.in[2]) return "16-bit backward convolution without X or dY";
      if (!lp_below_2g(op.M_out, op.Cout)) return "16-bit backward convolution with a dY of 2 GiB or more";
      if (op.out[0]) {
        if (!wsis_spconv_lp_supported(op.K, op.Cout, op.Cin))
          return "16-bit dIn product outside wsis_spconv_lp_supported (channels multiples of 32, at most 512)";
        if (!op.in[1]) return "16-bit dIn product without weights";
      }
      if (op.out[1] && (!wsis_spconv_lp_supported(op.K, op.Cin, op.Cout) || !lp_below_2g(op.M_in, op.Cin)))
        return "16-bit weight gradient outside wsis_spconv_lp_supported or with an input of 2 GiB or more";
      return nullptr;
    default:
      return "16-bit form of an op kind that has none";
  }
}

inline int64_t dw_ws_of(const wsis_op& op) {
  if (is_lp(op)) return up(wsis_spconv_dw_lp_workspace_bytes(op.M_out, op.K, op.Cin, op.Cout));
  if (op.flags & WSIS_OPF_BN_IN) return up(wsis_spconv_dw_bn_workspace_bytes(op.M_in, op.K, op.Cin, op.Cout));
  return up(wsis_spconv_dw_workspace_bytes(op.M_out, op.K, op.Cin, op.Cout));
}

int64_t op_ws_bytes(const wsis_op& op, bool on) {
  if (lp_refusal(op)) return -1;
  switch (op.kind) {
    case WSIS_OP_CONV:
      if (is_lp(op)) return up(wsis_spconv_fwd_lp_workspace_bytes(op.M_out, op.K, op.Cin, op.Cout));
#if WSIS_EXPERIMENTAL
      if (op.flags & (WSIS_OPF_BN_IN | WSIS_OPF_STAT_FIN))
        return up(std::max(wsis_spconv_fwd_f_workspace_bytes(op.M_out, op.K, op.Cin, op.Cout),
                           wsis_spconv_fwd_t_workspace_bytes(op.M_out, op.K, op.Cin, op.Cout)));
#else
      if (op.flags & (WSIS_OPF_BN_IN | WSIS_OPF_STAT_FIN)) return -1;
#endif
      if (use_fwd2(op, on)) return up(wsis_spconv_fwd_t_workspace_bytes(op.M_out, op.K, op.Cin, op.Cout));
      return up(wsis_spconv_fwd_workspace_bytes(op.M_out, op.K, op.Cin, op.Cout));
    case WSIS_OP_BN_RELU:
      if (!(op.flags & WSIS_OPF_TRAINING)) return 0;
      return up(std::max(wsis_bn_workspace_bytes(op.M_in, op.Cin),
                         wsis_bn_stats_finalize_workspace_bytes((op.M_in + 31) / 32, op.Cin)));
    case WSIS_OP_BN_RELU_BWD:
      return up(std::max(wsis_bn_workspace_bytes(op.M_in, op.Cin),
                         wsis_bn_stats_finalize_workspace_bytes((op.M_in + 31) / 32, op.Cin)));
    case WSIS_OP_CONV_BWD:
      if (!op.out[0]) return 0;
      if (is_lp(op)) return up(wsis_spconv_fwd_lp_workspace_bytes(op.M_in, op.K, op.Cout, op.Cin));
      if (use_fwd2(op, on)) return up(wsis_spconv_fwd_t_workspace_bytes(op.M_in, op.K, op.Cout, op.Cin));
      return up(wsis_spconv_fwd_workspace_bytes(op.M_in, op.K, op.Cout, op.Cin));
    default:
      return 0;
  }
}

inline int paired_bn(const wsis_op* ops, int n, int i) {
  const wsis_op& op = ops[i];
  for (int j = i + 1; j < n && j <= i + 4; ++j)
    if (ops[j].kind == WSIS_OP_BN_RELU_BWD && ops[j].in[1] == op.out[0] && (ops[j].flags & WSIS_OPF_STATS)) return j;
  return -1;
}

struct PassPlan {
  enum { LP, WT, DW, DEEP, OP, REGIONS };
  int64_t at[REGIONS], bytes[REGIONS], total = 0;
  std::vector<int64_t> lp_off, wt_off;
  int64_t dw_max = 0;
  int n_dw = 0;
};

struct PassRun {
  const wsis_op* ops;
  int n, mark_op;
  void *d_sync, *stream, *waiter_stream;
  hipStream_t st;
  PassOptions opt;
  PassPlan plan;
  char *base, *ws;
  int64_t ws_bytes;
  SideStream* side = nullptr;
  SideStream* wt_side = nullptr;
  bool wt_pending = false;
  bool forked = false;
  bool use_worker = false, worker_busy = false;
  int cur_dev = 0;
  std::vector<DwRedRec> dw_recs;
  int dw_next = 0, dw_flushed = 0;
  int64_t dw_off = 0;
  std::vector<char> bn_unfused;

  char* region(int k) const { return base + plan.at[k]; }
  const float* wt_of(int i) const { return reinterpret_cast<const float*>(region(PassPlan::WT) + plan.wt_off[i]); }
  int start();
  int fork_weight_transposes();
  int await_transposes_before(int i);
  int dw_issue(const wsis_op& op);
  int dw_flush();
  int drain_worker();
  int milestone();
  int finish(int first_err, bool defer_join);
};

#if WSIS_EXPERIMENTAL
inline int64_t deep_rows(const wsis_op& op) {
  switch (op.kind) {
    case WSIS_OP_CONV: return op.M_out;
    case WSIS_OP_CONV_BWD: return op.out[0] ? op.M_in : 0;
    default: return op.M_in;
  }
}
inline bool aligned16(const void* p) { return (reinterpret_cast<uintptr_t>(p) & 15) == 0; }

bool deep_op_ok(const wsis_op* ops, int n, int i, bool fwd2_on) {
  const wsis_op& op = ops[i];
  if (is_lp(op)) return false;
  const int64_t R = deep_max_rows();
  int nw = 0, zs = 0;
  switch (op.kind) {
    case WSIS_OP_CONV:
      if (op.flags & (WSIS_OPF_BN_IN | WSIS_OPF_STAT_FIN)) return false;
      if (!use_fwd2(op, fwd2_on) || op.M_out < 1 || op.M_out > R) return false;
      if ((int64_t)op.K * op.M_out * 4 >= ((int64_t)1 << 31)) return false;
      return deep_conv_plan(op.M_out, op.K, op.Cin, op.Cout, &nw, &zs) && aligned16(op.in[0]) && aligned16(op.out[0]);
    case WSIS_OP_CONV_BWD: {
      if (op.flags & WSIS_OPF_BN_IN) return false;
      if (!op.out[0]) return op.M_in <= R;
      if (!use_fwd2(op, fwd2_on) || op.M_in < 1 || op.M_in > R) return false;
      if (!deep_conv_plan(op.M_in, op.K, op.Cout, op.Cin, &nw, &zs)) return false;
      if (op.flags & WSIS_OPF_STATS) {
        const int j = paired_bn(ops, n, i);
        if (j < 0 || !ops[j].in[7] || ops[j].M_in != op.M_in || ops[j].Cin != op.Cin) return false;
      }
      return aligned16(op.in[2]) && aligned16(op.out[0]);
    }
    case WSIS_OP_BN_RELU:
      if (op.M_in < 1 || op.M_in > R || op.Cin % 32 || !deep_bn_rows_ok(op.M_in)) return false;
      if (op.flags & WSIS_OPF_TRAINING) {
        if (!(op.flags & WSIS_OPF_STATS) || !op.in[5]) return false;
        if (op.in[6] && (op.K % 32 || op.K <= 0 || op.K >= op.Cin)) return false;
      } else if (!op.out[0]) {
        return false;
      }
      return aligned16(op.in[0]) && (!op.out[0] || aligned16(op.out[0]));
    case WSIS_OP_BN_RELU_BWD:
      if (op.M_in < 1 || op.M_in > R || op.Cin % 32 || !deep_bn_rows_ok(op.M_in)) return false;
      if (!(op.flags & WSIS_OPF_TRAINING) || !(op.flags & WSIS_OPF_STATS) || !op.in[7]) return false;
      return aligned16(op.in[0]) && aligned16(op.in[1]) && aligned16(op.out[0]) && (!op.in[6] || aligned16(op.in[6]));
    case WSIS_OP_CAT:
      return op.M_in >= 1 && op.M_in <= R && vec4_ok(op, op.in[0], op.in[1], op.out[0]);
    case WSIS_OP_SPLIT:
      return op.M_in >= 1 && op.M_in <= R && vec4_ok(op, op.in[0], op.out[0], op.out[1]);
    default:
      return false;
  }
}

int deep_run_end(const wsis_op* ops, int n, int i0, int stop, bool fwd2_on) {
  int i1 = i0;
  while (i1 < n && (stop < 0 || i1 <= stop) && deep_op_ok(ops, n, i1, fwd2_on)) ++i1;
  for (int i = i0; i < i1; ++i)
    if (ops[i].kind == WSIS_OP_CONV_BWD && ops[i].out[0] && (ops[i].flags & WSIS_OPF_STATS)) {
      const int j = paired_bn(ops, n, i);
      if (j >= i1) {
        i1 = i;
        break;
      }
    }
  for (int j = i0; j < i1; ++j)
    if (ops[j].kind == WSIS_OP_BN_RELU_BWD) {
      bool found = false;
      for (int i = j - 1; i >= i0 && i >= j - 4 && !found; --i)
        found = ops[i].kind == WSIS_OP_CONV_BWD && ops[i].out[0] == ops[j].in[1] && (ops[i].flags & WSIS_OPF_STATS);
      if (!found) {
        i1 = j;
        break;
      }
    }
  return i1;
}

constexpr int kDeepMinOps = 4;
std::vector<std::pair<std::vector<DeepOp>, const unsigned long long*>> g_deep_log;
inline int64_t deep_table_bytes(int n_ops) { return up((int64_t)(2 * n_ops + 2) * (int64_t)sizeof(DeepOp)); }

int64_t deep_slab_bytes(const wsis_op* ops, int i0, int i1) {
  int64_t b = 0;
  for (int i = i0; i < i1; ++i) {
    const wsis_op& op = ops[i];
    int nw = 0, zs = 1;
    if (op.kind == WSIS_OP_CONV && deep_conv_plan(op.M_out, op.K, op.Cin, op.Cout, &nw, &zs) && zs > 1)
      b += up((int64_t)zs * op.M_out * op.Cout * 4);
    if (op.kind == WSIS_OP_CONV_BWD && op.out[0] && deep_conv_plan(op.M_in, op.K, op.Cout, op.Cin, &nw, &zs) && zs > 1)
      b += up((int64_t)zs * op.M_in * op.Cin * 4);
  }
  return b;
}

int64_t deep_ws_bytes(const wsis_op* ops, int n, bool fwd2_on) {
  if (!deep_enabled()) return 0;
  int64_t best = 0;
  for (int i = 0; i < n;) {
    if (!deep_op_ok(ops, n, i, fwd2_on)) {
      ++i;
      continue;
    }
    const int i1 = deep_run_end(ops, n, i, -1, fwd2_on);
    if (i1 - i >= kDeepMinOps) best = std::max(best, deep_table_bytes(i1 - i) + deep_slab_bytes(ops, i, i1));
    i = i1 > i ? i1 : i + 1;
  }
  return best;
}

struct DeepBuild {
  const char* wt_base;
  const std::vector<int64_t>& wt_off;
  char* slab;
  bool stamps;
  std::vector<DeepOp>& tab;
  std::vector<std::pair<int, std::pair<int, int>>>& conv_stamps;
  void push(DeepOp& d) {
    d.stamp = stamps ? (int)tab.size() + 1 : -1;
    tab.push_back(d);
  }
};

int deep_build_conv(DeepBuild& b, const wsis_op* ops, int n, int i) {
  const wsis_op& op = ops[i];
  DeepOp d{};
  const bool fwd = op.kind == WSIS_OP_CONV;
  if (!fwd && !op.out[0]) return WSIS_OK;
  const int64_t Mo = fwd ? op.M_out : op.M_in, Mg = fwd ? op.M_in : op.M_out;
  const int Ci = fwd ? op.Cin : op.Cout, Co = fwd ? op.Cout : op.Cin;
  int nw = 1, zs = 1;
  if (!deep_conv_plan(Mo, op.K, Ci, Co, &nw, &zs)) return fail(WSIS_ERR_ARG, "deep: op %d has no plan", i);
  d.kind = DK_CONV;
  d.NW = nw;
  d.ZS = zs;
  d.K = op.K;
  d.Cin = Ci;
  d.Cout = Co;
  d.M_in = Mg;
  d.M_out = Mo;
  d.x_bytes = (uint32_t)(Mg * Ci * 4);
  const void* stats = nullptr;
  DeepOp epi{};
// ... 110 lines not shown
        d.p[8] = op.out[0];
        d.p[9] = op.out[1];
        d.p[10] = op.out[2];
        b.push(d);
        break;
      case WSIS_OP_CAT:
        d.kind = DK_CAT;
        d.Cin = op.Cin;
        d.Cout = op.Cout;
        d.M_in = op.M_in;
        d.p[0] = op.in[0];
        d.p[1] = op.in[1];
        d.p[2] = op.out[0];
        b.push(d);
        break;
      case WSIS_OP_SPLIT:
        d.kind = DK_SPLIT;
        d.Cin = op.Cin;
        d.Cout = op.Cout;
        d.M_in = op.M_in;
        d.p[0] = op.in[0];
        d.p[1] = op.out[0];
        d.p[2] = op.out[1];
        b.push(d);
        break;
      default:
        return fail(WSIS_ERR_ARG, "deep: op %d of kind %d is not a phase", i, op.kind);
    }
  }
  return WSIS_OK;
}

int deep_issue_run(PassRun& r, int i, int* next) {
  *next = i;
  if (r.plan.bytes[PassPlan::DEEP] == 0 || !r.d_sync || r.opt.capturing || !deep_op_ok(r.ops, r.n, i, r.opt.fwd2)) return WSIS_OK;
  const int i1 = deep_run_end(r.ops, r.n, i, r.mark_op >= i ? r.mark_op : -1, r.opt.fwd2);
  if (i1 - i < kDeepMinOps) return WSIS_OK;
  *next = i1;
  std::vector<DeepOp> tab;
  std::vector<std::pair<int, std::pair<int, int>>> convs;
  char* const deep_ws = r.region(PassPlan::DEEP);
  char* slab = deep_ws + deep_table_bytes(i1 - i);
  int rc = deep_build(r.ops, r.n, i, i1, r.region(PassPlan::WT), r.plan.wt_off, slab, g_prof_on, tab, convs);
  if (rc != WSIS_OK) return rc;
  unsigned long long* d_stamps = nullptr;
  if (g_prof_on && !tab.empty()) {
    if (hipMalloc((void**)&d_stamps, (tab.size() + 1) * sizeof(unsigned long long)) != hipSuccess)
      return fail(WSIS_ERR_HIP, "deep: stamp buffer allocation failed");
    g_prof_bufs.push_back(d_stamps);
  }
  rc = deep_launch(tab.data(), (int)tab.size(), deep_ws, deep_sync_slot(r.d_sync), d_stamps, r.st);
  if (rc != WSIS_OK) return rc;
  if (d_stamps) {
    if (g_deep_log.size() > 64) g_deep_log.clear();
    g_deep_log.push_back({tab, d_stamps});
    for (const auto& cs : convs) {
      ProfRec p{};
      p.d_stamps = d_stamps;
      p.s0 = cs.second.first;
      p.sm = cs.second.first + 1;
      p.s1 = cs.second.second;
      g_prof[0].push_back(p);
    }
  }
  for (int k = i; k < i1 && rc == WSIS_OK; ++k)
    if (r.ops[k].kind == WSIS_OP_CONV_BWD && r.ops[k].out[1]) rc = r.dw_issue(r.ops[k]);
  return rc;
}

int issue_conv_fused_bn(PassRun& r, const wsis_op& op, int i) {
  if (r.plan.wt_off[i] < 0)
    return fail(WSIS_ERR_ARG, "op %d: fused BatchNorm requested from a convolution that is not on wsis_spconv_fwd_t", i);
  wsis_bn_in bi;
  bi.mean = (const float*)op.in[6];
  bi.var = (const float*)op.in[7];
  bi.gamma = (const float*)op.in[8];
  bi.beta = (const float*)op.in[9];
  bi.eps = op.eps;
  bi.relu = (op.flags & WSIS_OPF_RELU) ? 1 : 0;
  wsis_stat_target tg[2];
  int nt = 0;
  if (op.flags & WSIS_OPF_STAT_FIN) {
    tg[0].mean = (float*)op.out[2];
    tg[0].var = (float*)op.out[3];
    tg[0].running_mean = (float*)const_cast<void*>(op.in[10]);
    tg[0].running_var = (float*)const_cast<void*>(op.in[11]);
    tg[0].momentum = op.momentum;
    tg[0].reserved = 0;
    nt = 1;
    if (op.out[4]) {
      tg[1].mean = (float*)op.out[4];
      tg[1].var = (float*)op.out[5];
      tg[1].running_mean = (float*)op.out[6];
      tg[1].running_var = (float*)op.out[7];
      tg[1].momentum = op.momentum2;
      tg[1].reserved = 0;
      nt = 2;
    }
  }
  return wsis_spconv_fwd_f((const float*)op.in[0], (op.flags & WSIS_OPF_BN_IN) ? &bi : nullptr, (const int32_t*)op.in[1],
                           (const int32_t*)op.in[2], r.wt_of(i), 0, (const float*)op.in[4], (const float*)op.in[5],
                           (float*)op.out[0], (op.flags & WSIS_OPF_STATS) ? (float*)op.out[1] : nullptr, tg, nt, op.M_in,
                           op.M_out, op.K, op.Cin, op.Cout, r.ws, r.ws_bytes, sync_slot(r.d_sync, i), r.stream);
}

#else
inline int64_t deep_ws_bytes(const wsis_op*, int, bool) { return 0; }
inline int deep_issue_run(PassRun&, int i, int* next) {
  *next = i;
  return WSIS_OK;
}
inline int issue_conv_fused_bn(PassRun&, const wsis_op&, int i) {
  return fail(WSIS_ERR_ARG, "op %d: the fused BatchNorm forms of the convolution are in the EXPERIMENTAL build only", i);
}
#endif

int plan_pass(const wsis_op* ops, int n, const PassOptions& o, PassPlan& p) {
  p.lp_off.assign(n, -1);
  p.wt_off.assign(n, -1);
  int64_t lp = 0, wt = 0, dw_sum = 0, need = ALIGN;
  for (int i = 0; i < n; ++i) {
    const wsis_op& op = ops[i];
    const char* why = lp_refusal(op);
    if (why) return fail(WSIS_ERR_ARG, "wsis_run_ops: op %d: %s", i, why);
    int64_t b = op_ws_bytes(op, o.fwd2);
    if (b < 0) return fail(WSIS_ERR_ARG, "wsis_run_ops: op %d: a form this build does not run (fused BatchNorm: EXPERIMENTAL)", i);
    if (dw_tail_on_main(ops, n, i)) b = std::max(b, dw_ws_of(op));
    need = std::max(need, b);
    if (is_lp_conv(op)) {
      p.lp_off[i] = lp;
      lp += lp_wt_bytes_of(op);
    }
    if (needs_wt(op, o.fwd2)) {
      if (!(op.kind == WSIS_OP_CONV ? op.in[3] : op.in[1]))
        return fail(WSIS_ERR_ARG, "wsis_run_ops: op %d: convolution without weights", i);
      p.wt_off[i] = wt;
      wt += wt_bytes_of(op);
    }
    if (op.kind == WSIS_OP_CONV_BWD && op.out[1]) {
      const int64_t d = dw_ws_of(op);
      p.dw_max = std::max(p.dw_max, d);
      dw_sum += d;
      ++p.n_dw;
    }
  }
  const int64_t sizes[PassPlan::REGIONS] = {lp, wt, o.dw_batch_reduce ? dw_sum : p.dw_max, deep_ws_bytes(ops, n, o.fwd2),
                                            need + ALIGN};
  p.total = 0;
  for (int k = 0; k < PassPlan::REGIONS; ++k) {
    p.at[k] = p.total;
    p.bytes[k] = sizes[k];
    p.total += sizes[k];
  }
  return WSIS_OK;
}

template <typename T>
int launch_weight_batches(const wsis_op* ops, int n, const std::vector<int64_t>& off, char* base, hipStream_t st) {
  constexpr bool lp = sizeof(T) == 2;
  WtBatch b;
  b.n = 0;
  b.start[0] = 0;
  int dtype = 0;
  auto flush = [&]() -> int {
    if (b.n == 0) return WSIS_OK;
    if (!lp)
      hipLaunchKernelGGL(weight_transpose_batch_kernel<float>, dim3(b.start[b.n]), dim3(256), 0, st, b);
    else if (dtype == 0)
      hipLaunchKernelGGL(weight_transpose_batch_kernel<__bf16>, dim3(b.start[b.n]), dim3(256), 0, st, b);
    else
      hipLaunchKernelGGL(weight_transpose_batch_kernel<_Float16>, dim3(b.start[b.n]), dim3(256), 0, st, b);
    WSIS_LAUNCH_CHECK();
    b.n = 0;
    return WSIS_OK;
  };
  for (int i = 0; i < n; ++i) {
    if (off[i] < 0) continue;
    const wsis_op& op = ops[i];
    if (b.n == WT_MAX || (lp && b.n > 0 && op.reserved != dtype)) {
      const int rc = flush();
      if (rc != WSIS_OK) return rc;
    }
    const bool fwd = op.kind == WSIS_OP_CONV;
    dtype = op.reserved;
    b.src[b.n] = (const float*)(fwd ? op.in[3] : op.in[1]);
    b.dst[b.n] = base + off[i];
    b.K[b.n] = op.K;
    b.Cin[b.n] = op.Cin;
    b.Cout[b.n] = op.Cout;
    b.plain[b.n] = (lp && !fwd) ? 1 : 0;
    b.flip[b.n] = (!b.plain[b.n] && (lp || !fwd) && (op.flags & WSIS_OPF_FLIP)) ? 1 : 0;
    b.start[b.n + 1] = b.start[b.n] + op.K * ((op.Cin + WT_TILE - 1) / WT_TILE) * ((op.Cout + WT_TILE - 1) / WT_TILE);
    ++b.n;
  }
  return flush();
}

int PassRun::start() {
  side = (plan.dw_max > 0 && opt.dw_stream) ? side_stream_for(st) : nullptr;
  if (side) side->next = 0;
  use_worker = side != nullptr && opt.dw_thread && !opt.prof && !opt.capturing;
  if (use_worker && hipGetDevice(&cur_dev) != hipSuccess) return fail(WSIS_ERR_HIP, "hipGetDevice failed");
  dw_recs.resize((size_t)(opt.dw_defer() ? plan.n_dw : 0));
  bn_unfused.assign(n, 0);
  return launch_weight_batches<uint16_t>(ops, n, plan.lp_off, region(PassPlan::LP), st);
}

int PassRun::fork_weight_transposes() {
  bool any_wt = false;
  for (int i = 0; i < n && !any_wt; ++i) any_wt = plan.wt_off[i] >= 0;
  if (opt.wt_side && opt.dw_stream && !opt.capturing && any_wt && plan.wt_off[0] < 0 && !opt.prof &&
      plan.bytes[PassPlan::DEEP] == 0)
    wt_side = side_stream_for(st);
  if (wt_side) {
    hipError_t e = hipEventRecord(wt_side->wt_fork, st);
    if (e == hipSuccess) e = hipStreamWaitEvent(wt_side->stream, wt_side->wt_fork, 0);
    if (e != hipSuccess) return fail(WSIS_ERR_HIP, "weight-transpose fork failed: %s", hipGetErrorString(e));
  }
  int rc = launch_weight_batches<float>(ops, n, plan.wt_off, region(PassPlan::WT), wt_side ? wt_side->stream : st);
  if (wt_side) {
    const hipError_t e = hipEventRecord(wt_side->wt_done, wt_side->stream);
    wt_pending = e == hipSuccess;
    if (!wt_pending && rc == WSIS_OK) rc = fail(WSIS_ERR_HIP, "weight-transpose event failed: %s", hipGetErrorString(e));
  }
  return rc;
}

int PassRun::await_transposes_before(int i) {
  if (!wt_pending || plan.wt_off[i] < 0) return WSIS_OK;
  wt_pending = false;
  const hipError_t e = hipStreamWaitEvent(st, wt_side->wt_done, 0);
  return e == hipSuccess ? WSIS_OK : fail(WSIS_ERR_HIP, "weight-transpose join failed: %s", hipGetErrorString(e));
}

int PassRun::drain_worker() {
  if (!worker_busy) return WSIS_OK;
  worker_busy = false;
  std::string msg;
  const int wrc = dw_worker().drain(&msg);
  return wrc == WSIS_OK ? WSIS_OK : fail(wrc, "%s", msg.c_str());
}

int PassRun::dw_issue(const wsis_op& op) {
  void* dw_stream = stream;
  char* my_ws = region(PassPlan::DW);
  int64_t my_bytes = plan.dw_max;
  DwRedRec* rec = nullptr;
  if (opt.dw_defer() && dw_next < plan.n_dw) {
    my_bytes = dw_ws_of(op);
    my_ws += dw_off;
    dw_off += my_bytes;
    rec = &dw_recs[(size_t)dw_next++];
  }
  if (side) {
    hipEvent_t e = next_fork_event(side);
    hipError_t he = e ? hipEventRecord(e, st) : hipErrorOutOfMemory;
    if (he == hipSuccess && !use_worker) he = hipStreamWaitEvent(side->stream, e, 0);
    if (he != hipSuccess) return fail(WSIS_ERR_HIP, "dW side-stream fork failed: %s", hipGetErrorString(he));
    dw_stream = side->stream;
    forked = true;
    if (use_worker) {
      DwTask t;
      t.op = op;
      t.ev = e;
      t.dev = cur_dev;
      t.side = side->stream;
      t.ws = my_ws;
      t.ws_bytes = my_bytes;
      t.rec = rec;
      dw_worker().push(t);
      worker_busy = true;
      return WSIS_OK;
    }
  }
  return issue_dw(op, my_ws, my_bytes, dw_stream, rec);
}

int PassRun::dw_flush() {
  if (dw_flushed == dw_next) return WSIS_OK;
  const DwRedRec* recs = dw_recs.data() + dw_flushed;
  const int cnt = dw_next - dw_flushed;
  dw_flushed = dw_next;
  if (side && use_worker) {
    DwTask t;
    t.ev = nullptr;
    t.dev = cur_dev;
    t.side = side->stream;
    t.ws = nullptr;
    t.ws_bytes = 0;
    t.flush = recs;
    t.flush_n = cnt;
    dw_worker().push(t);
    worker_busy = true;
    return WSIS_OK;
  }
  return dw2_reduce_batch(recs, cnt, side ? side->stream : st);
}

int PassRun::milestone() {
  SideStream* ms = side ? side : side_stream_for(st);
  int wrc = dw_flush();
  if (wrc == WSIS_OK) wrc = drain_worker();
  if (wrc != WSIS_OK) return wrc;
  hipError_t e = ms ? hipEventRecord(ms->mark_main, st) : hipErrorOutOfMemory;
  if (e == hipSuccess) e = hipStreamWaitEvent(as_stream(waiter_stream), ms->mark_main, 0);
  if (e == hipSuccess && forked) {
    e = hipEventRecord(ms->mark_side, side->stream);
    if (e == hipSuccess) e = hipStreamWaitEvent(as_stream(waiter_stream), ms->mark_side, 0);
  }
  return e == hipSuccess ? WSIS_OK : fail(WSIS_ERR_HIP, "wsis_run_ops: milestone failed: %s", hipGetErrorString(e));
}

int PassRun::finish(int first_err, bool defer_join) {
  int wrc = first_err == WSIS_OK ? dw_flush() : WSIS_OK;
  if (wrc != WSIS_OK && first_err == WSIS_OK) first_err = wrc;
  wrc = drain_worker();
  if (wrc != WSIS_OK && first_err == WSIS_OK) first_err = wrc;
  if (wt_pending) {
    wt_pending = false;
    const hipError_t e = hipStreamWaitEvent(st, wt_side->wt_done, 0);
    if (e != hipSuccess && first_err == WSIS_OK)
      first_err = fail(WSIS_ERR_HIP, "weight-transpose join failed: %s", hipGetErrorString(e));
  }
  if (defer_join && first_err == WSIS_OK) {
    if (forked) side->pending_join = true;
    return WSIS_OK;
  }
  if (!forked && !side && opt.dw_stream) {
    SideStream* s2 = side_stream_for(st);
    if (s2 && s2->pending_join) {
      side = s2;
      forked = true;
    }
  } else if (side && side->pending_join) {
    forked = true;
  }
  if (forked) {
    side->pending_join = false;
    const hipError_t e1 = hipEventRecord(side->join, side->stream);
    const hipError_t e2 = e1 == hipSuccess ? hipStreamWaitEvent(st, side->join, 0) : e1;
    if (e2 != hipSuccess && first_err == WSIS_OK)
      return fail(WSIS_ERR_HIP, "side-stream join failed: %s", hipGetErrorString(e2));
  }
  return first_err;
}

inline int launch_status() {
  const hipError_t e = hipGetLastError();
  return e == hipSuccess ? WSIS_OK : fail(WSIS_ERR_HIP, "wsis_run_ops: launch failed: %s", hipGetErrorString(e));
}
inline int relu_of(const wsis_op& op) { return (op.flags & WSIS_OPF_RELU) ? 1 : 0; }
inline int flip_of(const wsis_op& op) { return (op.flags & WSIS_OPF_FLIP) ? 1 : 0; }

int issue_conv(PassRun& r, const wsis_op& op, int i) {
  if (is_lp(op))
    return wsis_spconv_fwd_lp_res(op.in[0], (const int32_t*)op.in[1], (const int32_t*)op.in[2], r.region(PassPlan::LP) + r.plan.lp_off[i],
                                  0, (const float*)op.in[4], op.in[5], op.out[0], op.M_in, op.M_out, op.K, op.Cin,
                                  op.Cout, op.reserved, r.ws, r.ws_bytes, r.stream);
  if (op.flags & (WSIS_OPF_BN_IN | WSIS_OPF_STAT_FIN)) return issue_conv_fused_bn(r, op, i);
  if (r.plan.wt_off[i] >= 0)
    return wsis_spconv_fwd_t((const float*)op.in[0], (const int32_t*)op.in[1], (const int32_t*)op.in[2], r.wt_of(i), 0,
                             (const float*)op.in[4], (const float*)op.in[5], (float*)op.out[0],
                             (op.flags & WSIS_OPF_STATS) ? (float*)op.out[1] : nullptr, op.M_in, op.M_out, op.K, op.Cin,
                             op.Cout, r.ws, r.ws_bytes, sync_slot(r.d_sync, i), r.stream);
  if (op.flags & WSIS_OPF_STATS)
    return fail(WSIS_ERR_ARG, "op %d: statistics requested from a convolution that is not on wsis_spconv_fwd_t", i);
  return wsis_spconv_fwd((const float*)op.in[0], (const int32_t*)op.in[1], (const int32_t*)op.in[2], (const float*)op.in[3],
                         (const float*)op.in[4], (const float*)op.in[5], (float*)op.out[0], op.M_in, op.M_out, op.K,
                         op.Cin, op.Cout, r.ws, r.ws_bytes, r.stream);
}

int bn_training_stats(PassRun& r, const wsis_op& op, int i, bool* applied) {
  const bool upd = (op.flags & WSIS_OPF_UPDATE_RUNNING) != 0;
  float* rm = upd ? (float*)op.in[3] : nullptr;
  float* rv = upd ? (float*)op.in[4] : nullptr;
  if (!(op.flags & WSIS_OPF_STATS) || op.M_in <= 0)
    return wsis_bn_stats((const float*)op.in[0], op.M_in, op.Cin, (float*)op.out[1], (float*)op.out[2], rm, rv,
                         op.momentum, r.ws, r.ws_bytes, r.stream);
  const int64_t n_part = (op.M_in + 31) / 32;
  const int C0 = op.in[6] ? op.K : op.Cin;
  if (!op.in[6] && op.out[0]) {
    *applied = true;
    return wsis_bn_stats_finalize_apply((const float*)op.in[5], n_part, op.M_in, op.Cin, (float*)op.out[1],
                                        (float*)op.out[2], rm, rv, op.momentum, (const float*)op.in[0],
                                        (const float*)op.in[1], (const float*)op.in[2], op.eps, relu_of(op),
                                        (float*)op.out[0], r.ws, r.ws_bytes, sync_slot(r.d_sync, i), r.stream);
  }
  int rc = wsis_bn_stats_finalize((const float*)op.in[5], n_part, op.M_in, C0, (float*)op.out[1], (float*)op.out[2], rm,
                                  rv, op.momentum, r.ws, r.ws_bytes, sync_slot(r.d_sync, i), r.stream);
  if (rc == WSIS_OK && op.in[6])
    rc = wsis_bn_stats_finalize((const float*)op.in[6], n_part, op.M_in, op.Cin - C0, (float*)op.out[1] + C0,
                                (float*)op.out[2] + C0, rm ? rm + C0 : nullptr, rv ? rv + C0 : nullptr, op.momentum,
                                r.ws, r.ws_bytes, sync_slot(r.d_sync, i), r.stream);
  return rc;
}

int bn_relu_launches(PassRun& r, const wsis_op& op, int i) {
  const bool training = (op.flags & WSIS_OPF_TRAINING) != 0;
  if (is_lp(op)) {
    if (training) {
      if (op.M_in <= 0) return WSIS_OK;
      const bool upd = (op.flags & WSIS_OPF_UPDATE_RUNNING) != 0;
      const int rc = wsis_bn_stats_lp(op.in[0], op.M_in, op.Cin, (float*)op.out[1], (float*)op.out[2],
                                      upd ? (float*)op.in[3] : nullptr, upd ? (float*)op.in[4] : nullptr, op.momentum, r.ws,
                                      r.ws_bytes, op.reserved, r.stream);
      if (rc != WSIS_OK) return rc;
    }
    return wsis_bn_apply_lp(op.in[0], (const float*)(training ? op.out[1] : op.in[3]),
                            (const float*)(training ? op.out[2] : op.in[4]), (const float*)op.in[1], (const float*)op.in[2],
                            op.eps, relu_of(op), op.out[0], (op.flags & WSIS_OPF_OUT_F32) ? 1 : 0, op.M_in, op.Cin,
                            op.reserved, r.stream);
  }
  if (training) {
    bool applied = false;
    const int rc = bn_training_stats(r, op, i, &applied);
    if (rc != WSIS_OK || applied) return rc;
  }
  if (!op.out[0]) return WSIS_OK;
  return wsis_bn_apply((const float*)op.in[0], (const float*)(training ? op.out[1] : op.in[3]),
                       (const float*)(training ? op.out[2] : op.in[4]), (const float*)op.in[1], (const float*)op.in[2],
                       op.eps, relu_of(op), (float*)op.out[0], op.M_in, op.Cin, r.stream);
}

int issue_bn_relu(PassRun& r, const wsis_op& op, int i) {
  ProfScope prof(2, r.st);
  const int rc = bn_relu_launches(r, op, i);
  prof.stop();
  return rc;
}

int issue_cat(PassRun& r, const wsis_op& op, int) {
  if (op.M_in <= 0) return WSIS_OK;
  wsis_op c = op;
  if (is_lp(op)) {
    c.Cin /= 2;
    c.Cout /= 2;
  }
  if (vec4_ok(c, c.in[0], c.in[1], c.out[0]))
    hipLaunchKernelGGL(cat_rows_kernel<4>, dim3(grid_for(c.M_in * (c.Cin + c.Cout) / 4, 256)), dim3(256), 0, r.st,
                       (const float*)c.in[0], (const float*)c.in[1], (float*)c.out[0], c.M_in, c.Cin, c.Cout);
  else
    hipLaunchKernelGGL(cat_rows_kernel<1>, dim3(grid_for(c.M_in * (c.Cin + c.Cout), 256)), dim3(256), 0, r.st,
                       (const float*)c.in[0], (const float*)c.in[1], (float*)c.out[0], c.M_in, c.Cin, c.Cout);
  return launch_status();
}

int issue_cast_lp(PassRun& r, const wsis_op& op, int) {
  const int64_t ne = op.M_in * op.Cin;
  if (ne <= 0) return WSIS_OK;
  const bool vec = ne % 4 == 0 && ((reinterpret_cast<uintptr_t>(op.in[0]) & 15) | (reinterpret_cast<uintptr_t>(op.out[0]) & 7)) == 0;
  const int64_t items = vec ? ne / 4 : ne;
  if (op.reserved == 0)
    hipLaunchKernelGGL(cast_lp_kernel<__bf16>, dim3(grid_for(items, 256)), dim3(256), 0, r.st, (const float*)op.in[0],
                       (__bf16*)op.out[0], ne, vec ? 1 : 0);
  else
    hipLaunchKernelGGL(cast_lp_kernel<_Float16>, dim3(grid_for(items, 256)), dim3(256), 0, r.st, (const float*)op.in[0],
                       (_Float16*)op.out[0], ne, vec ? 1 : 0);
  return launch_status();
}

int issue_split(PassRun& r, const wsis_op& op, int) {
  if (op.M_in <= 0) return WSIS_OK;
  wsis_op c = op;
  if (is_lp(op)) {
    c.Cin /= 2;
    c.Cout /= 2;
  }
  if (vec4_ok(c, c.in[0], c.out[0], c.out[1]))
    hipLaunchKernelGGL(split_rows_kernel<4>, dim3(grid_for(c.M_in * (c.Cin + c.Cout) / 4, 256)), dim3(256), 0, r.st,
                       (const float*)c.in[0], (float*)c.out[0], (float*)c.out[1], c.M_in, c.Cin, c.Cout);
  else
    hipLaunchKernelGGL(split_rows_kernel<1>, dim3(grid_for(c.M_in * (c.Cin + c.Cout), 256)), dim3(256), 0, r.st,
                       (const float*)c.in[0], (float*)c.out[0], (float*)c.out[1], c.M_in, c.Cin, c.Cout);
  return launch_status();
}

int issue_add(PassRun& r, const wsis_op& op, int) {
  if (op.M_in * op.Cin <= 0) return WSIS_OK;
  hipLaunchKernelGGL(add_inplace_kernel, dim3(grid_for(op.M_in * op.Cin, 256)), dim3(256), 0, r.st, (float*)op.out[0],
                     (const float*)op.in[0], op.M_in * op.Cin);
  return launch_status();
}

int issue_din(PassRun& r, const wsis_op& op, int i) {
  const float* dY = (const float*)op.in[2];
  const int32_t *nbr = (const int32_t*)op.in[5], *order = (const int32_t*)op.in[6];
  float* dX = (float*)op.out[0];
  const bool stats = (op.flags & WSIS_OPF_STATS) != 0;
  if (is_lp(op))
    return wsis_spconv_fwd_lp(op.in[2], nbr, order, r.region(PassPlan::LP) + r.plan.lp_off[i], flip_of(op), nullptr, op.out[0],
                              op.M_out, op.M_in, op.K, op.Cout, op.Cin, op.reserved, r.ws, r.ws_bytes, r.stream);
  if (r.plan.wt_off[i] >= 0) {
    if (stats)
      return fail(WSIS_ERR_ARG, "op %d: BatchNorm partials requested from a dIn pass that is not on wsis_spconv_fwd_t", i);
    return wsis_spconv_fwd(dY, nbr, order, r.wt_of(i), nullptr, nullptr, dX, op.M_out, op.M_in, op.K, op.Cout, op.Cin, r.ws,
                           r.ws_bytes, r.stream);
  }
  const int j = stats ? paired_bn(r.ops, r.n, i) : -1;
  if (stats && (j < 0 || !r.ops[j].in[7] || r.ops[j].M_in != op.M_in || r.ops[j].Cin != op.Cin))
    return fail(WSIS_ERR_ARG, "op %d: no BatchNorm backward takes the partials of this dIn pass", i);
  const bool unfused = stats && !r.opt.slab_bn_partials && wsis_spconv_fwd_t_slabs(op.M_in, op.K, op.Cout, op.Cin) > 1;
  if (unfused) r.bn_unfused[j] = 1;
  if (!stats || unfused)
    return wsis_spconv_fwd_t(dY, nbr, order, (const float*)op.in[1], flip_of(op), nullptr, nullptr, dX, nullptr, op.M_out,
                             op.M_in, op.K, op.Cout, op.Cin, r.ws, r.ws_bytes, sync_slot(r.d_sync, i), r.stream);
  const wsis_op& bn = r.ops[j];
  return wsis_spconv_fwd_t_bn(dY, nbr, order, (const float*)op.in[1], flip_of(op), dX, (float*)const_cast<void*>(bn.in[7]),
                              (const float*)bn.in[0], (const float*)bn.in[2], (const float*)bn.in[3], (const float*)bn.in[4],
                              (const float*)bn.in[5], bn.eps, relu_of(bn), op.M_out, op.M_in, op.K, op.Cout, op.Cin, r.ws,
                              r.ws_bytes, sync_slot(r.d_sync, i), r.stream);
}

int issue_conv_bwd(PassRun& r, const wsis_op& op, int i) {
  const bool early = r.opt.dw_early && op.out[1] && op.out[0] && r.side;
  int rc = early ? r.dw_issue(op) : WSIS_OK;
  if (rc == WSIS_OK && op.out[0]) rc = issue_din(r, op, i);
  if (rc != WSIS_OK || !op.out[1] || early) return rc;
  if (r.opt.dw_tail_main && r.side && dw_tail_on_main(r.ops, r.n, i))
    return issue_dw(op, r.ws, r.ws_bytes, r.stream, nullptr);
  return r.dw_issue(op);
}

int issue_bn_relu_bwd(PassRun& r, const wsis_op& op, int i) {
  ProfScope prof(2, r.st);
  int rc;
  if (is_lp(op)) {
    rc = op.M_in <= 0 ? WSIS_OK
                      : wsis_bn_bwd_lp(op.in[0], op.in[1], (const float*)op.in[2], (const float*)op.in[3],
                                       (const float*)op.in[4], (const float*)op.in[5], op.eps, relu_of(op),
                                       (op.flags & WSIS_OPF_TRAINING) ? 1 : 0, op.out[0], (op.flags & WSIS_OPF_OUT_F32) ? 1 : 0,
                                       (float*)op.out[1], (float*)op.out[2], op.in[6], op.M_in, op.Cin, op.reserved, r.ws,
                                       r.ws_bytes, r.stream);
  } else if ((op.flags & WSIS_OPF_STATS) && !r.bn_unfused[i]) {
    if (!op.in[7] || !(op.flags & WSIS_OPF_TRAINING))
      rc = fail(WSIS_ERR_ARG, "op %d: BatchNorm backward from partials needs in[7] and training mode", i);
    else
      rc = wsis_bn_bwd_from_partials((const float*)op.in[7], (op.M_in + 31) / 32, (const float*)op.in[0],
                                     (const float*)op.in[1], (const float*)op.in[2], (const float*)op.in[3],
                                     (const float*)op.in[4], (const float*)op.in[5], op.eps, relu_of(op), (float*)op.out[0],
                                     (float*)op.out[1], (float*)op.out[2], (const float*)op.in[6], op.M_in, op.Cin, r.ws,
                                     r.ws_bytes, sync_slot(r.d_sync, i), r.stream);
  } else {
    rc = wsis_bn_bwd((const float*)op.in[0], (const float*)op.in[1], (const float*)op.in[2], (const float*)op.in[3],
                     (const float*)op.in[4], (const float*)op.in[5], op.eps, relu_of(op),
                     (op.flags & WSIS_OPF_TRAINING) ? 1 : 0, (float*)op.out[0], (float*)op.out[1], (float*)op.out[2],
                     (const float*)op.in[6], op.M_in, op.Cin, r.ws, r.ws_bytes, r.stream);
  }
  prof.stop();
  return rc;
}

int issue_op(PassRun& r, const wsis_op& op, int i) {
  switch (op.kind) {
    case WSIS_OP_CONV: return issue_conv(r, op, i);
    case WSIS_OP_BN_RELU: return issue_bn_relu(r, op, i);
    case WSIS_OP_CAT: return issue_cat(r, op, i);
    case WSIS_OP_CAST_LP: return issue_cast_lp(r, op, i);
    case WSIS_OP_SPLIT: return issue_split(r, op, i);
    case WSIS_OP_ADD: return issue_add(r, op, i);
    case WSIS_OP_CONV_BWD: return issue_conv_bwd(r, op, i);
    case WSIS_OP_BN_RELU_BWD: return issue_bn_relu_bwd(r, op, i);
    default: return fail(WSIS_ERR_ARG, "wsis_run_ops: unknown op kind");
  }
}

int run_ops_impl(const wsis_op* ops, int32_t n, void* d_ws, int64_t ws_bytes, void* d_sync, void* stream, int32_t mark_op,
                 void* waiter_stream, bool defer_join = false) {
  WSIS_REQUIRE((ops || n == 0) && n >= 0, "bad op list");
  WSIS_REQUIRE(mark_op < n && (mark_op < 0 || waiter_stream), "bad milestone");
  PassRun r{ops, n, mark_op, d_sync, stream, waiter_stream, as_stream(stream)};
  r.opt = read_pass_options(&r.st);
  int err = plan_pass(ops, n, r.opt, r.plan);
  if (err != WSIS_OK) return err;
  WSIS_REQUIRE((n == 0 || ws_bytes >= r.plan.total) && (d_ws || n == 0), "workspace too small");
  r.base = static_cast<char*>(d_ws);
  r.ws = r.region(PassPlan::OP);
  r.ws_bytes = ws_bytes - r.plan.at[PassPlan::OP];
  err = r.start();
  if (err != WSIS_OK) return err;
  err = r.fork_weight_transposes();
  for (int i = 0; i < n && err == WSIS_OK; ++i) {
    err = r.await_transposes_before(i);
    int next = i;
    if (err == WSIS_OK) err = deep_issue_run(r, i, &next);
    if (err == WSIS_OK && next == i) err = issue_op(r, ops[i], i);
    if (next > i) i = next - 1;
    if (err == WSIS_OK && i == mark_op) err = r.milestone();
  }
  return r.finish(err, defer_join);
}

}

__global__ void warm_stream_kernel(int* p) {
  if (p && threadIdx.x == 0xffff) p[0] = 0;
}

extern "C" {

int wsis_warm_streams(void* stream) {
  hipStream_t st = as_stream(stream);
  SideStream* side = side_stream_for(st);
  WSIS_REQUIRE(side != nullptr, "side stream creation failed");
  hipLaunchKernelGGL(warm_stream_kernel, dim3(1), dim3(64), 0, st, (int*)nullptr);
  hipLaunchKernelGGL(warm_stream_kernel, dim3(1), dim3(64), 0, side->stream, (int*)nullptr);
  WSIS_LAUNCH_CHECK();
  WSIS_HIP_CHECK(hipStreamSynchronize(side->stream));
  return WSIS_OK;
}

int64_t wsis_run_ops_workspace_bytes(const wsis_op* ops, int32_t n) {
  if (!ops || n < 0) return -1;
  PassPlan plan;
  return plan_pass(ops, n, read_pass_options(nullptr), plan) == WSIS_OK ? plan.total : -1;
}

int wsis_debug_run_ops_layout(const wsis_op* ops, int32_t n, int64_t* out) {
  WSIS_REQUIRE((ops || n == 0) && n >= 0 && out, "bad arguments");
  PassPlan plan;
  const int rc = plan_pass(ops, n, read_pass_options(nullptr), plan);
  if (rc != WSIS_OK) return rc;
  for (int k = 0; k < PassPlan::REGIONS; ++k) {
    out[2 * k] = plan.at[k];
    out[2 * k + 1] = plan.bytes[k];
  }
  out[10] = plan.total;
  std::copy(plan.lp_off.begin(), plan.lp_off.end(), out + 11);
  std::copy(plan.wt_off.begin(), plan.wt_off.end(), out + 11 + n);
  return WSIS_OK;
}

int wsis_run_ops(const wsis_op* ops, int32_t n, void* d_ws, int64_t ws_bytes, void* d_sync, void* stream) {
  return wsis_run_ops_marked(ops, n, d_ws, ws_bytes, d_sync, stream, -1, nullptr);
}

int wsis_run_ops_part(const wsis_op* ops, int32_t n, void* d_ws, int64_t ws_bytes, void* d_sync, void* stream, int32_t last) {
  return run_ops_impl(ops, n, d_ws, ws_bytes, d_sync, stream, -1, nullptr, last == 0);
}

int wsis_run_ops_marked(const wsis_op* ops, int32_t n, void* d_ws, int64_t ws_bytes, void* d_sync, void* stream,
                        int32_t mark_op, void* waiter_stream) {
#if !WSIS_EXPERIMENTAL
  return run_ops_impl(ops, n, d_ws, ws_bytes, d_sync, stream, mark_op, waiter_stream);
#else
  const char* ge = getenv("WSIS_GRAPH");
  const int graph_mode = ge ? atoi(ge) : 0;
  if (!graph_mode || mark_op >= 0 || g_prof_on || n == 0)
    return run_ops_impl(ops, n, d_ws, ws_bytes, d_sync, stream, mark_op, waiter_stream);
  hipStream_t st = as_stream(stream);
  static std::map<std::pair<hipStream_t, int64_t>, hipGraphExec_t> cache;
  static hipStream_t cap = nullptr;
  if (!cap) WSIS_HIP_CHECK(hipStreamCreateWithFlags(&cap, hipStreamNonBlocking));
  const int target = graph_mode >= 4 ? graph_mode : 1 << 30;
  int chunk_no = 0;
  for (int i0 = 0; i0 < n; ++chunk_no) {
    int i1 = i0, pending = 0;
    while (i1 < n) {
      const wsis_op& op = ops[i1];
      if (op.kind == WSIS_OP_CONV_BWD && (op.flags & WSIS_OPF_STATS) && op.out[0]) ++pending;
      if (op.kind == WSIS_OP_BN_RELU_BWD && (op.flags & WSIS_OPF_STATS) && pending > 0) --pending;
      ++i1;
      if (i1 - i0 >= target && pending == 0) break;
    }
    WSIS_HIP_CHECK(hipStreamBeginCapture(cap, hipStreamCaptureModeRelaxed));
    const int rc = run_ops_impl(ops + i0, i1 - i0, d_ws, ws_bytes, d_sync, cap, -1, nullptr);
    hipGraph_t g = nullptr;
    const hipError_t ec = hipStreamEndCapture(cap, &g);
    if (ec != hipSuccess || !g) return fail(WSIS_ERR_HIP, "graph capture failed: %s", hipGetErrorString(ec));
    if (rc != WSIS_OK) {
      (void)hipGraphDestroy(g);
      return rc;
    }
    const auto key = std::make_pair(st, ((int64_t)ops[0].kind * 4096 + n) * 64 + chunk_no);
    hipGraphExec_t& ex = cache[key];
    bool ready = false;
    if (ex) {
      hipGraphNode_t bad = nullptr;
      hipGraphExecUpdateResult res;
      if (hipGraphExecUpdate(ex, g, &bad, &res) == hipSuccess && res == hipGraphExecUpdateSuccess) {
        ready = true;
      } else {
        (void)hipGetLastError();
        (void)hipGraphExecDestroy(ex);
        ex = nullptr;
      }
    }
    if (!ready) {
      const hipError_t ei = hipGraphInstantiate(&ex, g, nullptr, nullptr, 0);
      if (ei != hipSuccess) {
        (void)hipGraphDestroy(g);
        ex = nullptr;
        return fail(WSIS_ERR_HIP, "graph instantiate failed: %s", hipGetErrorString(ei));
      }
    }
    const hipError_t el = hipGraphLaunch(ex, st);
    (void)hipGraphDestroy(g);
    if (el != hipSuccess) return fail(WSIS_ERR_HIP, "graph launch failed: %s", hipGetErrorString(el));
    i0 = i1;
  }
  return WSIS_OK;
#endif
}

#if WSIS_EXPERIMENTAL
int wsis_debug_deep_phases(int32_t which, int32_t* info, double* us, int32_t cap) {
  if (which < 0 || which >= (int)g_deep_log.size()) return -1;
  const auto& rec = g_deep_log[which];
  const int n = (int)rec.first.size();
  if (n > cap) return -1;
  std::vector<unsigned long long> t(n + 1);
  if (hipDeviceSynchronize() != hipSuccess) return -1;
  if (hipMemcpy(t.data(), rec.second, (n + 1) * sizeof(unsigned long long), hipMemcpyDeviceToHost) != hipSuccess) return -1;
  for (int i = 0; i < n; ++i) {
    const DeepOp& d = rec.first[i];
    info[i * 8 + 0] = d.kind;
    info[i * 8 + 1] = d.NW;
    info[i * 8 + 2] = d.ZS;
    info[i * 8 + 3] = (int32_t)(d.kind == DK_CONV || d.kind == DK_REDUCE ? d.M_out : d.M_in);
    info[i * 8 + 4] = d.Cin;
    info[i * 8 + 5] = d.Cout;
    info[i * 8 + 6] = d.K;
    info[i * 8 + 7] = (int32_t)d.M_in;
    us[i] = (double)(t[i + 1] - t[i]) * 0.01;
  }
  return n;
}

#endif

}
```

### 3d-wsis_amd/wsis_native/__init__.py

```python
import ctypes
import os
from ctypes import c_char_p, c_double, c_float, c_int32, c_int64, c_void_p

_HERE = os.path.dirname(os.path.abspath(__file__))
_PKG = os.path.dirname(_HERE)

_host = None
_hip = None

I32 = c_int32
I64 = c_int64
F32 = c_float
F64 = c_double
P = c_void_p


class WsisError(RuntimeError):
    pass


def _load(name):
    path = os.path.join(_PKG, name)
    if not os.path.exists(path):
        raise WsisError(
            f"{name} not found at {path}: build it with `python -c 'import __graft_entry__ as g; g.build()'` "
            f"or `make -C 3d-wsis_amd/csrc` (no CPU fallback exists for this path)")
    return ctypes.CDLL(path)


_HOST_SIGS = {
    "wsis_host_version": (I32, []),
    "wsis_host_last_error": (c_char_p, []),
    "wsis_host_voxelize_idx_map": (I32, [P, I64, P, P, P]),
    "wsis_host_voxelize_idx_fill": (I32, [P, I64, P, I64, I32, P, P]),
    "wsis_host_bfs_cluster_count": (I32, [P, P, P, I64, I32, P, P, P, P]),
    "wsis_host_bfs_cluster_fill": (I32, [P, P, I64, I64, I64, P, P]),
    "wsis_host_graph_bfs": (I32, [P, P, I32, P, P, P, P, I64, P, P]),
}

_HIP_SIGS = {
    "wsis_version": (I32, []),
    "wsis_last_error": (c_char_p, []),
    "wsis_device_count": (I32, []),
    "wsis_voxelize_fwd": (I32, [P, P, P, I64, I32, I32, I32, P]),
    "wsis_voxelize_bwd": (I32, [P, P, P, I64, I32, I32, I32, P]),
    "wsis_voxelize_idx_workspace_bytes": (I64, [I64]),
    "wsis_voxelize_idx_map": (I32, [P, I64, P, P, P, I64, P]),
    "wsis_voxelize_idx_fill": (I32, [P, I64, I64, I32, P, P, P, I64, P]),
    "wsis_hash_build": (I32, [P, I64, P, P, P, I64, P]),
    "wsis_rulebook_subm": (I32, [P, I64, P, P, P, P, P, I64, P, P, P]),
    "wsis_rulebook_down_ncand": (I64, [I64, P, P, P]),
    "wsis_rulebook_down_workspace_bytes": (I64, [I64]),
    "wsis_rulebook_down_keys": (I32, [P, I64, P, P, P, P, P, P, P, P, P, I64, P]),
    "wsis_rulebook_down_fill": (I32, [P, I64, P, P, P, P, P, P, I64, P, P, P, I64, P, P, P, P, P]),
    "wsis_mask_order_workspace_bytes": (I64, [I64]),
    "wsis_mask_order": (I32, [P, I64, P, P, I64, P]),
    "wsis_tile_order_workspace_bytes": (I64, [I64]),
    "wsis_tile_order": (I32, [P, P, I64, I32, P, P, I64, P]),
    "wsis_tile_order_batch_workspace_bytes": (I64, [I64]),
    "wsis_tile_order_batch": (I32, [I32, P, P, P, I32, I32, P, P, I64, P]),
    "wsis_spconv_fwd_workspace_bytes": (I64, [I64, I32, I32, I32]),
    "wsis_spconv_fwd": (I32, [P, P, P, P, P, P, P, I64, I64, I32, I32, I32, P, I64, P]),
    "wsis_spconv_fwd_t_supported": (I32, [I32, I32, I32]),
    "wsis_spconv_fwd_t_workspace_bytes": (I64, [I64, I32, I32, I32]),
    "wsis_spconv_fwd_t": (I32, [P, P, P, P, I32, P, P, P, P, I64, I64, I32, I32, I32, P, I64, P, P]),
    "wsis_spconv_fwd_t_slabs": (I32, [I64, I32, I32, I32]),
    "wsis_bn_bwd_from_partials": (I32, [P, I64, P, P, P, P, P, P, F32, I32, P, P, P, P, I64, I32, P, I64, P, P]),
    "wsis_sync_bytes": (I64, []),
    "wsis_run_ops_part": (I32, [P, I32, P, I64, P, P, I32]),
    "wsis_bn_bwd_apply": (I32, [P, P, P, P, P, P, P, P, F32, I32, P, P, I64, I32, P]),
    "wsis_spconv_fwd_t_bn": (I32, [P, P, P, P, I32, P, P, P, P, P, P, P, F32, I32, I64, I64, I32, I32, I32, P, I64, P, P]),
    "wsis_bn_stats_finalize_workspace_bytes": (I64, [I64, I32]),
    "wsis_bn_stats_finalize": (I32, [P, I64, I64, I32, P, P, P, P, F32, P, I64, P, P]),
    "wsis_bn_stats_finalize_apply": (I32, [P, I64, I64, I32, P, P, P, P, F32, P, P, P, F32, I32, P, P, I64, P, P]),
    "wsis_weight_transpose": (I32, [P, P, I32, I32, I32, I32, P]),
    "wsis_spconv_dw_workspace_bytes": (I64, [I64, I32, I32, I32]),
    "wsis_spconv_dw": (I32, [P, P, P, P, P, I64, I64, I32, I32, I32, P, I64, P]),
    "wsis_spconv_lp_supported": (I32, [I32, I32, I32]),
    "wsis_spconv_lp_plan": (I32, [I64, I32, I32, I32, P]),
    "wsis_spconv_fwd_lp_workspace_bytes": (I64, [I64, I32, I32, I32]),
    "wsis_spconv_fwd_lp": (I32, [P, P, P, P, I32, P, P, I64, I64, I32, I32, I32, I32, P, I64, P]),
    "wsis_spconv_fwd_lp_res": (I32, [P, P, P, P, I32, P, P, P, I64, I64, I32, I32, I32, I32, P, I64, P]),
    "wsis_spconv_dw_lp_workspace_bytes": (I64, [I64, I32, I32, I32]),
    "wsis_spconv_dw_lp": (I32, [P, P, P, P, P, I64, I64, I32, I32, I32, I32, P, I64, P]),
    "wsis_weight_cast_lp": (I32, [P, P, I32, I32, I32, I32, I32, I32, P]),
    "wsis_spconv_dw_bn_supported": (I32, [I32, I32, I32]),
    "wsis_spconv_dw_bn_workspace_bytes": (I64, [I64, I32, I32, I32]),
    "wsis_spconv_dw_bn": (I32, [P, P, P, P, P, F32, I32, P, P, I32, P, P, I64, I64, I32, I32, I32, P, I64, P]),
    "wsis_rulebook_pyramid_layout": (I64, [I64, P, I32, P]),
    "wsis_rulebook_pyramid": (I32, [P, I64, P, P, I32, I32, I32, P, I64, P]),
    "wsis_rulebook_down_form": (I32, [I64, P, P, P, P, I32]),
    "wsis_rulebook_pack": (I32, [P, P, P, I64, I32, P]),
    "wsis_rulebook_pack_batch": (I32, [I32, P, P, P, P, P, P]),
    "wsis_prof_enable": (I32, [I32]),
    "wsis_prof_summary": (I32, [I32, P, P]),
    "wsis_prof_records": (I32, [I32, P, P, I64, P]),
    "wsis_bn_workspace_bytes": (I64, [I64, I32]),
    "wsis_bn_stats": (I32, [P, I64, I32, P, P, P, P, F32, P, I64, P]),
    "wsis_bn_apply": (I32, [P, P, P, P, P, F32, I32, P, I64, I32, P]),
    "wsis_bn_apply_lp": (I32, [P, P, P, P, P, F32, I32, P, I32, I64, I32, I32, P]),
    "wsis_bn_stats_lp": (I32, [P, I64, I32, P, P, P, P, F32, P, I64, I32, P]),
    "wsis_bn_bwd_lp": (I32, [P, P, P, P, P, P, F32, I32, I32, P, I32, P, P, P, I64, I32, I32, P, I64, P]),
    "wsis_bn_bwd": (I32, [P, P, P, P, P, P, F32, I32, I32, P, P, P, P, I64, I32, P, I64, P]),
    "wsis_bn_bwd_apply_lp": (I32, [P, P, P, P, P, P, P, P, F32, I32, P, I32, P, I64, I32, I32, P]),
    "wsis_bn_sync_pack": (I32, [P, P, I64, I32, P, P]),
    "wsis_bn_sync_combine": (I32, [P, I32, I32, P, P, P, P, F32, P, P]),
    "wsis_bn_sync_sums_pack": (I32, [P, P, I32, P, P]),
    "wsis_bn_sync_sums_scale": (I32, [P, I64, P, I32, P, P, P]),
    "wsis_segment_csr_workspace_bytes": (I64, [I64, I64]),
    "wsis_segment_csr": (I32, [P, I64, I64, P, P, P, I64, P]),
    "wsis_segment_csr_batch_workspace_bytes": (I64, [I64]),
    "wsis_segment_csr_batch": (I32, [I32, P, P, P, P, P, P, I64, P]),
    "wsis_segment_reduce_fwd": (I32, [P, P, P, P, P, I64, I64, I32, I32, P]),
    "wsis_segment_reduce_bwd": (I32, [P, P, P, P, P, I64, I64, I32, I32, P]),
    "wsis_gather_rows": (I32, [P, P, I32, P, I64, I32, P]),
    "wsis_edge_affinity_fwd": (I32, [P, P, P, P, P, P, P, P, F32, P, P, I64, I64, I32, P]),
    "wsis_edge_affinity_bwd": (I32, [P] * 11 + [F32] + [P] * 7 + [I64, I64, I64, I32, P]),
    "wsis_ecc_message_fwd": (I32, [P, P, P, P, P, P, I64, I64, I32, P]),
    "wsis_ecc_message_bwd": (I32, [P, P, P, P, P, P, P, P, P, I64, I64, I32, P]),
    "wsis_ecc_contract_fwd": (I32, [P, P, P, P, P, I64, I64, P]),
    "wsis_ecc_contract_bwd": (I32, [P, P, P, P, P, P, P, I64, I64, P]),
    "wsis_ecc_contract_bwd_acc": (I32, [P, P, P, P, P, P, P, I64, I64, I32, P]),
    "wsis_ecc_contract_bwd_mean": (I32, [P, P, P, P, P, P, P, P, P, I64, I64, I32, P]),
    "wsis_ecc_u_fwd": (I32, [P, P, P, I64, P]),
    "wsis_gru_cell_workspace_bytes": (I64, [I64]),
    "wsis_gru_cell_fwd": (I32, [P] * 9 + [I64, I32, P]),
    "wsis_gru_cell_bwd": (I32, [P] * 17 + [I64, I32, P, I64, P]),
    "wsis_colsum_workspace_bytes": (I64, [I64, I32]),
    "wsis_colsum": (I32, [P, I64, I32, P, P, I64, P, P]),
    "wsis_pos_enc_workspace_bytes": (I64, [I64]),
    "wsis_pos_enc_fwd": (I32, [P, P, P, P, P, P, P, P, I64, P]),
    "wsis_pos_enc_bwd": (I32, [P, P, P, P, P, P, P, P, P, P, P, I64, P, I64, P]),
    "wsis_heads_workspace_bytes": (I64, [I64, I32, I32]),
    "wsis_heads_fwd": (I32, [P, P, I64, F32, F32, I32, P, P, I64, P]),
    "wsis_heads_bwd": (I32, [P, P, I64, I32, P, P, P, I64, P]),
    "wsis_gru_cell_bwd_seq": (I32, [P] * 10 + [I64] + [P] * 8 + [I64, I32, I32, I32, I32, P, I64, P]),
    "wsis_gru_cell_fwd_mean": (I32, [P] * 12 + [I64, I32, P]),
    "wsis_affinity_dense_build": (I32, [P, P, P, I64, P, I64, P]),
    "wsis_affinity_transition": (I32, [P, P, P, P, P, I32, F32, P, I64, P]),
    "wsis_dgemm": (I32, [P, P, P, I64, I64, I64, P]),
    "wsis_affinity_colmax": (I32, [P, P, I32, P, P, I64, P]),
    "wsis_affinity_propagate_sparse_workspace_bytes": (I64, [I64, I32]),
    "wsis_affinity_propagate_sparse": (I32, [P, P, P, P, P, P, P, I32, I32, F32, I32, I64, P, P, I64, P, P, P, I64, P]),
    "wsis_ballquery_workspace_bytes": (I64, [I64]),
    "wsis_ballquery_count": (I32, [P, P, P, I64, I32, F32, P, P, P, I64, P]),
    "wsis_ballquery_fill": (I32, [P, P, P, I64, I32, F32, P, P, I64, P, I64, P]),
    "wsis_cc_same_label": (I32, [P, P, P, I64, P, P, P, P]),
    "wsis_bfs_order": (I32, [P, P, P, P, P, I64, P, P, P, P]),
    "wsis_plane_score_workspace_bytes": (I64, [I64, I32]),
    "wsis_plane_score": (I32, [P, I64, P, I32, F64, P, P, P, I64, P]),
    "wsis_plane_mark": (I32, [P, I64, P, F64, P, P]),
    "wsis_wl_sp_stats": (I32, [P, P, P, I64, I64, P, P, P, P]),
    "wsis_wl_neighbor_source": (I32, [P, I64, P, P, P, P, F64, I64, P, P]),
    "wsis_wl_apply_source": (I32, [P, P, P, P, P, P, I64, I64, P, P, P, P, P]),
    "wsis_wl_scene_assign": (I32, [P, I64, P, P, P, P, P, P, P, P, F64, I64, P, P, P, P, P, P]),
    "wsis_wl_point_labels": (I32, [P, I64, P, P, P, P, P]),
    "wsis_wl_occupancy_workspace_bytes": (I64, [I64]),
    "wsis_wl_occupancy": (I32, [P, P, P, I64, I32, F32, P, P, I64, P]),
    "wsis_wl_instance_size": (I32, [P, P, I64, I32, P, P, P]),
    "wsis_wl_label_stats": (I32, [P, P, P, P, I64, P, I32, P, P]),
    "wsis_sp_state_bytes": (I64, []),
    "wsis_sp_state_init": (I32, [P, P]),
    "wsis_sp_affine": (I32, [P, I32, P, I64, I64, P, F64, P, P, P, P]),
    "wsis_sp_crop_mask": (I32, [P, I64, P, I32, P, P, P, P, I32, P]),
    "wsis_sp_emit_workspace_bytes": (I64, [I64, I64, I64]),
    "wsis_sp_emit": (I32, [P, P, I64, I64, I64, P, P, P, P, P, P, P, P, P, I64, I64] + [P] * 9 + [P, I64, P]),
    "wsis_sp_tables": (I32, [P, I64, I64, P, P, P, P, P, P]),
    "wsis_sp_relabel": (I32, [P, P, I64, P, I64, P, I64, P, P, P, P]),
    "wsis_sp_instance_info": (I32, [P, P, P, I64, I64, P, P, P]),
    "wsis_gp_sp_moments": (I32, [P, P, P, I64, I64, P, P, P, P, P, P, P, P]),
    "wsis_gp_label_mode": (I32, [P, P, P, I64, I64, P, P, P]),
    "wsis_gp_neighbors": (I32, [P, I64, I32, F64, P, P, P, P]),
    "wsis_gp_edge_features": (I32, [P, P, P, I64, I64, P, I64, P, P, P, P, P, P, P, P]),
    "wsis_pt_bins_workspace_bytes": (I64, [I64]),
    "wsis_pt_bins": (I32, [P, I64, F32, P, P, P, P, I64, P]),
    "wsis_pt_prune_accumulate": (I32, [P, P, P, I32, P, P, I64, I64, P, P, P, P, P]),
    "wsis_pt_knn_workspace_bytes": (I64, [I64]),
    "wsis_pt_knn": (I32, [P, I64, I32, F64, P, P, P, P, I64, P]),
    "wsis_pt_geof": (I32, [P, P, I64, I32, P, P, P, P]),
    "wsis_pt_edge_features_workspace_bytes": (I64, [I64, I32]),
    "wsis_pt_edge_features": (I32, [P, P, P, P, I64, I32, I32, F32, P, P, P, P, P, P, P, I64, P]),
    "wsis_mask_overlap_chunk": (I32, []),
    "wsis_mask_overlap_tile_rows": (I32, [I32]),
    "wsis_mask_overlap_workspace_bytes": (I64, [I64, I64, I32]),
    "wsis_mask_overlap": (I32, [P, I32, I64, I64, P, I32, P, P, P, I64, P]),
    "wsis_label_pairs": (I32, [P, P, I64, I32, I32, P, P]),
    "wsis_semantic_loss_workspace_bytes": (I64, [I64]),
    "wsis_semantic_loss_fwd": (I32, [P, P, I64, I32, I64, P, P, P, I64, P]),
    "wsis_semantic_loss_bwd": (I32, [P, P, I64, I32, I64, P, P, P, P]),
    "wsis_sp_ce_loss_workspace_bytes": (I64, [I64]),
    "wsis_sp_ce_loss_fwd": (I32, [P, P, I64, I32, I64, P, P, I64, P, P]),
    "wsis_sp_ce_loss_bwd": (I32, [P, P, I64, I32, I64, P, P, P, P]),
    "wsis_loss_sum": (I32, [P, I32, ctypes.c_uint32, P, P]),
    "wsis_sp_regression_loss_fwd": (I32, [P] * 8 + [I64, I64, P, P]),
    "wsis_sp_regression_loss_bwd": (I32, [P] * 8 + [I64, I64] + [P] * 8 + [P]),
    "wsis_disc_loss_saved_floats": (I32, []),
    "wsis_disc_loss_fwd": (I32, [P, P, P, I64, I32, I32, I64, F32, F32, F32, F32, F32, P, P, P]),
    "wsis_disc_loss_bwd": (I32, [P, P, P, I64, I32, I32, I64, F32, F32, F32, F32, F32, P, P, P, P]),
    "wsis_adamw_segment_bytes": (I32, []),
    "wsis_adamw_chunk": (I32, []),
    "wsis_adamw_step": (I32, [P, P, I64, F64, F64, F64, F64, F64, P]),
    "wsis_grad_nonfinite": (I32, [P, P, I64, P, P]),
    "wsis_adamw_step_scaled": (I32, [P, P, I64, F64, F64, F64, F64, F64, P, P, P, P]),
    "wsis_loss_scale_update": (I32, [P, P, P, F64, F64, I32, P]),
    "wsis_run_ops_workspace_bytes": (I64, [P, I32]),
    "wsis_run_ops": (I32, [P, I32, P, I64, P, P]),
    "wsis_run_ops_marked": (I32, [P, I32, P, I64, P, P, I32, P]),
    "wsis_experimental": (I32, []),
    "wsis_warm_streams": (I32, [P]),
    "wsis_hint_batch_rows": (I32, [I64]),
}

_HIP_SIGS_EXPERIMENTAL = {
    "wsis_spconv_fwd_f_workspace_bytes": (I64, [I64, I32, I32, I32]),
    "wsis_spconv_fwd_f": (I32, [P, P, P, P, P, I32, P, P, P, P, P, I32, I64, I64, I32, I32, I32, P, I64, P, P]),
    "wsis_deep_launches": (I64, []),
    "wsis_deep_phases": (I64, []),
}


def _bind(lib, sigs):
    for name, (res, args) in sigs.items():
        fn = getattr(lib, name)
        fn.restype = res
        fn.argtypes = args
    return lib


def host():
    global _host
    if _host is None:
        _host = _bind(_load("libwsis_host.so"), _HOST_SIGS)
    return _host


def hip():
    global _hip
    if _hip is None:
        import torch
        _hip = _bind(_load("libwsis_hip.so"), _HIP_SIGS)
        if _hip.wsis_experimental():
            _bind(_hip, _HIP_SIGS_EXPERIMENTAL)
    return _hip


def experimental():
    return bool(hip().wsis_experimental())


def require_experimental(what):
    if not experimental():
        raise WsisError(f"{what} is part of the EXPERIMENTAL build only: make -C 3d-wsis_amd/csrc EXPERIMENTAL=1 "
                        f"(or WSIS_EXPERIMENTAL=1 python -c 'import __graft_entry__ as g; g.build()')")


def declared_symbols(experimental=False):
    hip_names = sorted(list(_HIP_SIGS) + (list(_HIP_SIGS_EXPERIMENTAL) if experimental else []))
# ... 76 lines not shown
```

### include/wsis_hip.h

```cpp
#ifndef WSIS_HIP_H_
#define WSIS_HIP_H_

#include <stdint.h>

#ifdef __cplusplus
extern "C" {
#endif

#define WSIS_ABI_VERSION 2

#define WSIS_OK 0
#define WSIS_ERR_ARG (-1)
#define WSIS_ERR_HIP (-2)
#define WSIS_ERR_OVERFLOW (-3)


int wsis_host_version(void);
const char* wsis_host_last_error(void);

int wsis_host_voxelize_idx_map(const int64_t* h_coords, int64_t N, int32_t* h_p2v, int64_t* M,
                               int32_t* max_active);
int wsis_host_voxelize_idx_fill(const int64_t* h_coords, int64_t N, const int32_t* h_p2v, int64_t M,
                                int32_t max_active, int64_t* h_voxel_locs, int32_t* h_v2p);

// ... 18 lines not shown
                      int32_t stride, int32_t mode, void* stream);
int wsis_voxelize_bwd(const float* d_dout, const int32_t* d_v2p, float* d_dfeats, int64_t M, int32_t C,
                      int32_t stride, int32_t mode, void* stream);

int64_t wsis_voxelize_idx_workspace_bytes(int64_t N);
int wsis_voxelize_idx_map(const int64_t* d_coords, int64_t N, int32_t* d_p2v, int32_t* d_counts2, void* d_ws,
                          int64_t ws_bytes, void* stream);
int wsis_voxelize_idx_fill(const int64_t* d_coords, int64_t N, int64_t M, int32_t max_active,
                           int64_t* d_voxel_locs, int32_t* d_v2p, void* d_ws, int64_t ws_bytes, void* stream);

int wsis_hash_build(const int32_t* d_indices, int64_t M, const int32_t* h_shape3, int64_t* d_keys,
                    int32_t* d_vals, int64_t cap, void* stream);
int wsis_rulebook_subm(const int32_t* d_indices, int64_t M, const int32_t* h_shape3,
                       const int32_t* h_ksize3, const int32_t* h_pad3, const int64_t* d_keys,
                       const int32_t* d_vals, int64_t cap, int32_t* d_nbr, uint32_t* d_mask,
                       void* stream);
int64_t wsis_rulebook_down_ncand(int64_t M_in, const int32_t* h_ksize3, const int32_t* h_stride3,
                                 const int32_t* h_pad3);
int64_t wsis_rulebook_down_workspace_bytes(int64_t n_cand);
int wsis_rulebook_down_keys(const int32_t* d_indices_in, int64_t M_in, const int32_t* h_in_shape3,
                            const int32_t* h_out_shape3, const int32_t* h_ksize3,
                            const int32_t* h_stride3, const int32_t* h_pad3, int64_t* d_cand,
                            int64_t* d_out_keys, int32_t* d_count, void* d_ws, int64_t ws_bytes,
                            void* stream);
int wsis_rulebook_down_fill(const int32_t* d_indices_in, int64_t M_in, const int32_t* h_in_shape3,
                            const int32_t* h_out_shape3, const int32_t* h_ksize3,
                            const int32_t* h_stride3, const int32_t* h_pad3,
                            const int64_t* d_out_keys, int64_t M_out, int32_t* d_indices_out,
                            int64_t* d_keys, int32_t* d_vals, int64_t cap, int32_t* d_nbr_down,
                            int32_t* d_nbr_up, uint32_t* d_mask_down, uint32_t* d_mask_up,
                            void* stream);
int64_t wsis_mask_order_workspace_bytes(int64_t M);
int64_t wsis_tile_order_workspace_bytes(int64_t M);
int wsis_tile_order(const int32_t* d_indices, const uint32_t* d_mask, int64_t M, int32_t block_shift,
                    int32_t* d_order, void* d_ws, int64_t ws_bytes, void* stream);
int wsis_mask_order(const uint32_t* d_mask, int64_t M, int32_t* d_order, void* d_ws, int64_t ws_bytes,
                    void* stream);
int64_t wsis_tile_order_batch_workspace_bytes(int64_t N);
int wsis_tile_order_batch(int32_t n, const void* const* h_indices, const void* const* h_mask, const int64_t* h_M,
                          int32_t block_shift, int32_t batch_size, int32_t* d_order_all, void* d_ws,
                          int64_t ws_bytes, void* stream);

int wsis_rulebook_pack(const int32_t* d_nbr, const int32_t* d_order, int32_t* d_nbr_packed, int64_t M,
                       int32_t K, void* stream);
int wsis_rulebook_pack_batch(int32_t n, const void* const* h_nbr, const void* const* h_order,
                             void* const* h_nbr_packed, const int64_t* h_M, const int32_t* h_K, void* stream);

enum {
  WSIS_PYR_ROWS = 0, WSIS_PYR_CAP, WSIS_PYR_INDICES, WSIS_PYR_KEYS, WSIS_PYR_VALS, WSIS_PYR_SUBM_NBR, WSIS_PYR_SUBM_MASK,
  WSIS_PYR_SUBM_ORDER, WSIS_PYR_SUBM_NBR_P, WSIS_PYR_CAND, WSIS_PYR_OUT_KEYS, WSIS_PYR_COUNT, WSIS_PYR_DOWN_WS,
  WSIS_PYR_DOWN_NBR, WSIS_PYR_UP_NBR, WSIS_PYR_DOWN_MASK, WSIS_PYR_UP_MASK, WSIS_PYR_DOWN_ORDER, WSIS_PYR_UP_ORDER,
  WSIS_PYR_DOWN_NBR_P, WSIS_PYR_UP_NBR_P, WSIS_PYR_FIELDS
};
int64_t wsis_rulebook_pyramid_layout(int64_t M0, const int64_t* h_counts, int32_t n_levels, int64_t* h_layout);
int wsis_rulebook_pyramid(const int32_t* d_indices0, int64_t M0, const int32_t* h_shape3, const int64_t* h_counts,
                          int32_t n_levels, int32_t batch_size, int32_t block_shift, void* d_arena, int64_t arena_bytes,
                          void* stream);
int32_t wsis_rulebook_down_form(int64_t M_in, const int32_t* h_out_shape3, const int32_t* h_ksize3,
                                const int32_t* h_stride3, const int32_t* h_pad3, int32_t batch_size);

int64_t wsis_spconv_fwd_workspace_bytes(int64_t M_out, int32_t K, int32_t Cin, int32_t Cout);
int wsis_spconv_fwd(const float* d_X, const int32_t* d_nbr, const int32_t* d_order, const float* d_W,
                    const float* d_bias, const float* d_residual, float* d_out, int64_t M_in,
                    int64_t M_out, int32_t K, int32_t Cin, int32_t Cout, void* d_ws, int64_t ws_bytes,
                    void* stream);
int32_t wsis_spconv_fwd_t_supported(int32_t K, int32_t Cin, int32_t Cout);
int32_t wsis_spconv_fwd_t_slabs(int64_t M_out, int32_t K, int32_t Cin, int32_t Cout);
int64_t wsis_spconv_fwd_t_workspace_bytes(int64_t M_out, int32_t K, int32_t Cin, int32_t Cout);
int wsis_spconv_fwd_t(const float* d_X, const int32_t* d_nbr, const int32_t* d_order, const float* d_WT, int32_t flip,
                      const float* d_bias, const float* d_residual, float* d_out, float* d_stats, int64_t M_in,
                      int64_t M_out, int32_t K, int32_t Cin, int32_t Cout, void* d_ws, int64_t ws_bytes,
                      void* d_sync, void* stream);
int wsis_spconv_fwd_t_bn(const float* d_X, const int32_t* d_nbr, const int32_t* d_order, const float* d_WT, int32_t flip,
                         float* d_out, float* d_partials, const float* d_bn_x, const float* d_bn_mean,
                         const float* d_bn_var, const float* d_bn_gamma, const float* d_bn_beta, float eps, int32_t relu,
                         int64_t M_in, int64_t M_out, int32_t K, int32_t Cin, int32_t Cout, void* d_ws, int64_t ws_bytes,
                         void* d_sync, void* stream);
typedef struct wsis_bn_in {
  const float* mean;
  const float* var;
  const float* gamma;
  const float* beta;
  float eps;
  int32_t relu;
} wsis_bn_in;
typedef struct wsis_stat_target {
  float* mean;
  float* var;
  float* running_mean;
  float* running_var;
  float momentum;
  int32_t reserved;
} wsis_stat_target;
#if defined(WSIS_EXPERIMENTAL) && WSIS_EXPERIMENTAL
int64_t wsis_spconv_fwd_f_workspace_bytes(int64_t M_out, int32_t K, int32_t Cin, int32_t Cout);
int wsis_spconv_fwd_f(const float* d_X, const wsis_bn_in* bn_in, const int32_t* d_nbr, const int32_t* d_order,
                      const float* d_WT, int32_t flip, const float* d_bias, const float* d_residual, float* d_out,
                      float* d_stats, const wsis_stat_target* targets, int32_t n_targets, int64_t M_in, int64_t M_out,
                      int32_t K, int32_t Cin, int32_t Cout, void* d_ws, int64_t ws_bytes, void* d_sync, void* stream);
#endif
int wsis_weight_transpose(const float* d_W, float* d_WT, int32_t K, int32_t Cin, int32_t Cout,
                          int32_t flip, void* stream);
int64_t wsis_spconv_dw_workspace_bytes(int64_t M_out, int32_t K, int32_t Cin, int32_t Cout);
int wsis_spconv_dw(const float* d_X, const int32_t* d_nbr, const int32_t* d_order, const float* d_dY,
                   float* d_dW, int64_t M_in, int64_t M_out, int32_t K, int32_t Cin, int32_t Cout, void* d_ws,
                   int64_t ws_bytes, void* stream);

int32_t wsis_spconv_lp_supported(int32_t K, int32_t Cin, int32_t Cout);
int32_t wsis_spconv_lp_plan(int64_t M_out, int32_t K, int32_t Cin, int32_t Cout, int32_t* out);
int64_t wsis_spconv_fwd_lp_workspace_bytes(int64_t M_out, int32_t K, int32_t Cin, int32_t Cout);
int wsis_spconv_fwd_lp(const void* d_X, const int32_t* d_nbr, const int32_t* d_order, const void* d_WT, int32_t flip,
                       const float* d_bias, void* d_out, int64_t M_in, int64_t M_out, int32_t K, int32_t Cin,
                       int32_t Cout, int32_t dtype, void* d_ws, int64_t ws_bytes, void* stream);
int wsis_spconv_fwd_lp_res(const void* d_X, const int32_t* d_nbr, const int32_t* d_order, const void* d_WT,
                           int32_t flip, const float* d_bias, const void* d_residual, void* d_out, int64_t M_in,
                           int64_t M_out, int32_t K, int32_t Cin, int32_t Cout, int32_t dtype, void* d_ws,
                           int64_t ws_bytes, void* stream);
int64_t wsis_spconv_dw_lp_workspace_bytes(int64_t M_out, int32_t K, int32_t Cin, int32_t Cout);
int wsis_spconv_dw_lp(const void* d_X, const int32_t* d_nbr, const int32_t* d_order, const void* d_dY, float* d_dW,
                      int64_t M_in, int64_t M_out, int32_t K, int32_t Cin, int32_t Cout, int32_t dtype, void* d_ws,
                      int64_t ws_bytes, void* stream);
int wsis_weight_cast_lp(const float* d_W, void* d_out, int32_t K, int32_t Cin, int32_t Cout, int32_t transpose,
                        int32_t flip, int32_t dtype, void* stream);

int32_t wsis_spconv_dw_bn_supported(int32_t K, int32_t Cin, int32_t Cout);
int64_t wsis_spconv_dw_bn_workspace_bytes(int64_t M_in, int32_t K, int32_t Cin, int32_t Cout);
int wsis_spconv_dw_bn(const float* d_X, const float* d_mean, const float* d_var, const float* d_gamma,
                      const float* d_beta, float eps, int32_t relu, const int32_t* d_nbr_b, const int32_t* d_order_b,
                      int32_t flip, const float* d_dY, float* d_dW, int64_t M_in, int64_t M_out, int32_t K, int32_t Cin,
                      int32_t Cout, void* d_ws, int64_t ws_bytes, void* stream);

int wsis_prof_enable(int32_t on);
int wsis_prof_summary(int32_t which, double* total_ms, int64_t* launches);
int wsis_prof_records(int32_t which, double* h_main_ms, double* h_total_ms, int64_t cap, int64_t* n);

int64_t wsis_sync_bytes(void);

int64_t wsis_bn_workspace_bytes(int64_t M, int32_t C);
int wsis_bn_stats(const float* d_x, int64_t M, int32_t C, float* d_mean, float* d_var, float* d_running_mean,
                  float* d_running_var, float momentum, void* d_ws, int64_t ws_bytes, void* stream);
int64_t wsis_bn_stats_finalize_workspace_bytes(int64_t n_part, int32_t C);
int wsis_bn_stats_finalize(const float* d_partials, int64_t n_part, int64_t M, int32_t C, float* d_mean, float* d_var,
                           float* d_running_mean, float* d_running_var, float momentum, void* d_ws, int64_t ws_bytes,
                           void* d_sync, void* stream);
int wsis_bn_stats_finalize_apply(const float* d_partials, int64_t n_part, int64_t M, int32_t C, float* d_mean,
                                 float* d_var, float* d_running_mean, float* d_running_var, float momentum,
                                 const float* d_x, const float* d_gamma, const float* d_beta, float eps, int32_t relu,
                                 float* d_y, void* d_ws, int64_t ws_bytes, void* d_sync, void* stream);
int wsis_bn_bwd_from_partials(const float* d_partials, int64_t n_part, const float* d_x, const float* d_dy,
                              const float* d_mean, const float* d_var, const float* d_gamma, const float* d_beta,
                              float eps, int32_t relu, float* d_dx, float* d_dgamma, float* d_dbeta,
                              const float* d_addend, int64_t M, int32_t C, void* d_ws, int64_t ws_bytes, void* d_sync,
                              void* stream);
int wsis_bn_apply(const float* d_x, const float* d_mean, const float* d_var, const float* d_gamma,
                  const float* d_beta, float eps, int32_t relu, float* d_y, int64_t M, int32_t C, void* stream);
int wsis_bn_apply_lp(const void* d_x, const float* d_mean, const float* d_var, const float* d_gamma,
                     const float* d_beta, float eps, int32_t relu, void* d_y, int32_t out_fp32, int64_t M, int32_t C,
                     int32_t dtype, void* stream);
int wsis_bn_stats_lp(const void* d_x, int64_t M, int32_t C, float* d_mean, float* d_var, float* d_running_mean,
                     float* d_running_var, float momentum, void* d_ws, int64_t ws_bytes, int32_t dtype, void* stream);
int wsis_bn_bwd_lp(const void* d_x, const void* d_dy, const float* d_mean, const float* d_var, const float* d_gamma,
                   const float* d_beta, float eps, int32_t relu, int32_t training, void* d_dx, int32_t out_fp32,
                   float* d_dgamma, float* d_dbeta, const void* d_addend, int64_t M, int32_t C, int32_t dtype, void* d_ws,
                   int64_t ws_bytes, void* stream);
int wsis_bn_bwd(const float* d_x, const float* d_dy, const float* d_mean, const float* d_var,
                const float* d_gamma, const float* d_beta, float eps, int32_t relu, int32_t training,
                float* d_dx, float* d_dgamma, float* d_dbeta, const float* d_addend, int64_t M, int32_t C, void* d_ws,
                int64_t ws_bytes, void* stream);

int wsis_bn_bwd_apply(const float* d_x, const float* d_dy, const float* d_mean, const float* d_var,
                      const float* d_gamma, const float* d_beta, const float* d_sum_dz_xhat, const float* d_sum_dz,
                      float eps, int32_t relu, float* d_dx, const float* d_addend, int64_t M, int32_t C, void* stream);
int wsis_bn_bwd_apply_lp(const void* d_x, const void* d_dy, const float* d_mean, const float* d_var, const float* d_gamma,
                         const float* d_beta, const float* d_sum_dz_xhat, const float* d_sum_dz, float eps, int32_t relu,
                         void* d_dx, int32_t out_fp32, const void* d_addend, int64_t M, int32_t C, int32_t dtype,
                         void* stream);

int wsis_bn_sync_pack(const float* d_mean, const float* d_var, int64_t M, int32_t C, double* d_out, void* stream);
int wsis_bn_sync_combine(const double* d_gathered, int32_t R, int32_t C, float* d_mean, float* d_var,
                         float* d_running_mean, float* d_running_var, float momentum, double* d_count, void* stream);
int wsis_bn_sync_sums_pack(const float* d_dgamma, const float* d_dbeta, int32_t C, double* d_out, void* stream);
int wsis_bn_sync_sums_scale(const double* d_sums, int64_t M, const double* d_count, int32_t C, float* d_sum_dz_xhat,
                            float* d_sum_dz, void* stream);

int64_t wsis_segment_csr_workspace_bytes(int64_t N, int64_t S);
int wsis_segment_csr(const int64_t* d_index, int64_t N, int64_t S, int32_t* d_perm, int32_t* d_offsets,
                     void* d_ws, int64_t ws_bytes, void* stream);
int64_t wsis_segment_csr_batch_workspace_bytes(int64_t N_all);
int wsis_segment_csr_batch(int32_t n, const void* const* h_index, const int64_t* h_N, const int64_t* h_S,
                           int32_t* d_perm_all, int32_t* d_offsets_all, void* d_ws, int64_t ws_bytes, void* stream);
int wsis_segment_reduce_fwd(const float* d_src, const int32_t* d_perm, const int32_t* d_offsets,
                            float* d_out, int32_t* d_argmax, int64_t N, int64_t S, int32_t C,
                            int32_t reduce, void* stream);
int wsis_segment_reduce_bwd(const float* d_dout, const int64_t* d_index, const int32_t* d_offsets,
                            const int32_t* d_argmax, float* d_dsrc, int64_t N, int64_t S, int32_t C,
                            int32_t reduce, void* stream);
int wsis_gather_rows(const float* d_src, const void* d_idx, int32_t idx_is_64, float* d_out, int64_t N,
                     int32_t C, void* stream);

int64_t wsis_pos_enc_workspace_bytes(int64_t E);
int wsis_pos_enc_fwd(const float* d_centre, const int64_t* d_eu, const int64_t* d_ev, const float* d_W1, const float* d_b1,
                     const float* d_W2, const float* d_b2, float* d_pos, int64_t E, void* stream);
int wsis_pos_enc_bwd(const float* d_centre, const int64_t* d_eu, const int64_t* d_ev, const float* d_W1, const float* d_b1,
                     const float* d_W2, const float* d_dpos, float* d_dW1, float* d_db1, float* d_dW2, float* d_db2, int64_t E,
                     void* d_ws, int64_t ws_bytes, void* stream);

int wsis_edge_affinity_fwd(const float* d_q, const float* d_k, const float* d_v, const float* d_pos,
                           const int64_t* d_eu, const int64_t* d_ev, const int32_t* d_perm_u,
                           const int32_t* d_off_u, float scale, float* d_aff, float* d_res, int64_t E,
                           int64_t Su, int32_t D, void* stream);
int wsis_edge_affinity_bwd(const float* d_q, const float* d_k, const float* d_v, const float* d_pos,
                           const float* d_aff, const int64_t* d_eu, const int64_t* d_ev,
                           const int32_t* d_perm_u, const int32_t* d_off_u, const int32_t* d_perm_v,
                           const int32_t* d_off_v, float scale, const float* d_daff,
                           const float* d_dres, float* d_dq, float* d_dk, float* d_dv, float* d_dpos,
                           float* d_tmp, int64_t E, int64_t S, int64_t Su, int32_t D, void* stream);

int wsis_ecc_contract_fwd(const float* d_h, const float* d_U, const int32_t* d_perm_dst, const int32_t* d_off_dst,
                          float* d_m, int64_t S, int64_t E, void* stream);
int wsis_ecc_contract_bwd(const float* d_h, const float* d_U, const float* d_dm, const int32_t* d_perm_dst,
                          const int32_t* d_off_dst, float* d_dU, float* d_dh, int64_t S, int64_t E, void* stream);
int wsis_ecc_contract_bwd_acc(const float* d_h, const float* d_U, const float* d_dm, const int32_t* d_perm_dst,
                              const int32_t* d_off_dst, float* d_dU, float* d_dh, int64_t S, int64_t E,
                              int32_t accumulate, void* stream);
int wsis_ecc_contract_bwd_mean(const float* d_h, const float* d_U, const float* d_dinp, const int64_t* d_src_index,
                               const int32_t* d_off_src, const int32_t* d_perm_dst, const int32_t* d_off_dst, float* d_dU,
                               float* d_dh, int64_t S, int64_t E, int32_t accumulate, void* stream);
int wsis_ecc_u_fwd(const float* d_hx, const float* d_W, float* d_U, int64_t S, void* stream);
int wsis_ecc_message_fwd(const float* d_x, const float* d_w, const int64_t* d_dst, const int32_t* d_perm_src,
                         const int32_t* d_off_src, float* d_out, int64_t S, int64_t E, int32_t C, void* stream);
int wsis_ecc_message_bwd(const float* d_x, const float* d_w, const float* d_dout, const int64_t* d_src,
                         const int32_t* d_perm_dst, const int32_t* d_off_dst, const int32_t* d_off_src,
                         float* d_dx, float* d_dw, int64_t S, int64_t E, int32_t C, void* stream);

int64_t wsis_colsum_workspace_bytes(int64_t M, int32_t C);
int wsis_colsum(const float* d_x, int64_t M, int32_t C, float* d_out, void* d_ws, int64_t ws_bytes, void* d_sync,
                void* stream);

#define WSIS_HEADS_MAX 8
typedef struct wsis_heads {
  int32_t n_heads, n_lin;
  int32_t cout[WSIS_HEADS_MAX];
  const float* W1[WSIS_HEADS_MAX];
  const float* b1[WSIS_HEADS_MAX];
  const float* gamma[WSIS_HEADS_MAX];
  const float* beta[WSIS_HEADS_MAX];
  const float* W2[WSIS_HEADS_MAX];
  const float* b2[WSIS_HEADS_MAX];
  float* running_mean[WSIS_HEADS_MAX];
  float* running_var[WSIS_HEADS_MAX];
  float* hidden[WSIS_HEADS_MAX];
  float* out[WSIS_HEADS_MAX];
  const float* dout[WSIS_HEADS_MAX];
  float* dW1[WSIS_HEADS_MAX];
  float* db1[WSIS_HEADS_MAX];
  float* dgamma[WSIS_HEADS_MAX];
  float* dbeta[WSIS_HEADS_MAX];
  float* dW2[WSIS_HEADS_MAX];
  float* db2[WSIS_HEADS_MAX];
} wsis_heads;
int64_t wsis_heads_workspace_bytes(int64_t S, int32_t n_heads, int32_t n_lin);
int wsis_heads_fwd(const wsis_heads* h, const float* d_x, int64_t S, float eps, float momentum, int32_t training,
                   float* d_saved, void* d_ws, int64_t ws_bytes, void* stream);
int wsis_heads_bwd(const wsis_heads* h, const float* d_x, int64_t S, int32_t training, const float* d_saved, float* d_dx,
                   void* d_ws, int64_t ws_bytes, void* stream);

int64_t wsis_gru_cell_workspace_bytes(int64_t S);
int wsis_gru_cell_fwd(const float* d_x, const float* d_h, const float* d_Wig, const float* d_big,
                      const float* d_Wih, const float* d_Whh, const float* d_bih, const float* d_bhh, float* d_hy,
                      int64_t S, int32_t C, void* stream);
int wsis_gru_cell_bwd(const float* d_x, const float* d_h, const float* d_Wig, const float* d_big,
                      const float* d_Wih, const float* d_Whh, const float* d_bih, const float* d_bhh,
                      const float* d_dhy, float* d_dx, float* d_dh, float* d_dWig, float* d_dbig, float* d_dWih,
                      float* d_dWhh, float* d_dbih, float* d_dbhh, int64_t S, int32_t C, void* d_ws,
                      int64_t ws_bytes, void* stream);
int wsis_gru_cell_bwd_seq(const float* d_x, const float* d_h, const float* d_Wig, const float* d_big,
                          const float* d_Wih, const float* d_Whh, const float* d_bih, const float* d_bhh,
                          const float* d_dhy, const float* d_dhy2, int64_t dhy2_pitch, float* d_dx, float* d_dh, float* d_dWig,
                          float* d_dbig, float* d_dWih, float* d_dWhh, float* d_dbih, float* d_dbhh, int64_t S, int32_t C,
                          int32_t slot, int32_t n_slots, int32_t finish, void* d_ws, int64_t ws_bytes, void* stream);
int wsis_gru_cell_fwd_mean(const float* d_m, const int32_t* d_perm, const int32_t* d_off, float* d_x_out, const float* d_h,
                           const float* d_Wig, const float* d_big, const float* d_Wih, const float* d_Whh, const float* d_bih,
                           const float* d_bhh, float* d_hy, int64_t S, int32_t C, void* stream);

int wsis_affinity_dense_build(const int64_t* d_eu, const int64_t* d_ev, const float* d_aff, int64_t E,
                              double* d_A, int64_t S, void* stream);
int wsis_affinity_transition(const double* d_A, const uint8_t* d_adj, const int32_t* d_pred,
                             const float* d_conf, const int32_t* d_label, int32_t cls, float thr,
                             double* d_T0, int64_t S, void* stream);
int wsis_dgemm(const double* d_A, const double* d_B, double* d_C, int64_t M, int64_t N, int64_t Kd,
               void* stream);
int wsis_affinity_colmax(const double* d_T, const int32_t* d_label, int32_t cls, double* d_scores,
                         int32_t* d_arg, int64_t S, void* stream);
int64_t wsis_affinity_propagate_sparse_workspace_bytes(int64_t S, int32_t n_present);
int wsis_affinity_propagate_sparse(const double* d_A, const uint8_t* d_adj, const int32_t* d_pred, const float* d_conf,
                                   const int32_t* d_label, const int32_t* d_cls_of, const int32_t* d_ci_of_cls,
                                   int32_t n_present, int32_t class_num, float thr, int32_t iterations, int64_t S,
                                   int32_t* d_col, double* d_val, int64_t nnz_cap, double* d_scores, int32_t* d_arg,
                                   void* d_ws, int64_t ws_bytes, void* stream);

int64_t wsis_ballquery_workspace_bytes(int64_t N);
int wsis_ballquery_count(const float* d_xyz, const int32_t* d_batch_idx, const int32_t* d_batch_off,
                         int64_t N, int32_t B, float radius, int32_t* d_start_len, int32_t* d_total,
                         void* d_ws, int64_t ws_bytes, void* stream);
int wsis_ballquery_fill(const float* d_xyz, const int32_t* d_batch_idx, const int32_t* d_batch_off,
                        int64_t N, int32_t B, float radius, const int32_t* d_start_len, int32_t* d_idx,
// ... 179 lines not shown
```

Before: 133.8 scenes/s.

## Fuse UNet skip concatenation into BatchNorm forward and split its backward gradient

Adds a planner fusion that folds a channel concatenation op into the following BatchNorm+ReLU. In the forward pass the fused kernels read the two source tensors directly and write both the concatenated tensor and the normalized output, with stats finalisation done per half. In the backward pass, dx is written straight into the two per-source gradient buffers instead of a concatenated gradient that is later split. This removes a separate concat kernel, its extra HBM round trip and the split copy in backward. The cost is more index arithmetic per element, new kernel variants, and a narrow domain (widths multiples of 32, at most 512 channels, aligned tensors).

```diff
diff --git a/3d-wsis_amd/csrc/bn.hip b/3d-wsis_amd/csrc/bn.hip
--- a/3d-wsis_amd/csrc/bn.hip
+++ b/3d-wsis_amd/csrc/bn.hip
@@ -367,6 +367,52 @@
   }
 }
 
+struct BnSplit {
+  float* dx2;
+  int Ca;
+};
+__device__ __forceinline__ float4* bn_dx_quad(float* dx, BnSplit sp, int64_t r, int C, int c4) {
+  if (!sp.dx2) return reinterpret_cast<float4*>(dx + r * C + c4);
+  if (c4 < sp.Ca) return reinterpret_cast<float4*>(dx + r * sp.Ca + c4);
+  return reinterpret_cast<float4*>(sp.dx2 + r * (C - sp.Ca) + (c4 - sp.Ca));
+}
+
+__global__ __launch_bounds__(BN_SMALL_THREADS) void bn_bwd_small_apply_kernel(
+    const float* __restrict__ x, const float* __restrict__ dy, const float* __restrict__ mean,
+    const float* __restrict__ var, const float* __restrict__ gamma, const float* __restrict__ beta,
+    const float* __restrict__ addend, float eps, int relu, int training, int64_t M, int C, float* __restrict__ dx,
+    BnSplit split, float* __restrict__ dgamma, float* __restrict__ dbeta) {
+  __shared__ double sh[BN_SMALL_THREADS / 64 * 8];
+  const int c0 = blockIdx.x * 4;
+  BnBwdAcc<float> acc{x, dy, mean, var, gamma, beta, eps, relu};
+  double a[4], b[4];
+  bn_small_body(acc, M, C, c0, sh, a, b);
+  if (threadIdx.x < 4) {
+    dbeta[c0 + threadIdx.x] = (float)a[threadIdx.x];
+    dgamma[c0 + threadIdx.x] = (float)b[threadIdx.x];
+  }
+  const float inv_m = 1.0f / (float)M;
+  float k1[4], k2[4];
+#pragma unroll
+  for (int e = 0; e < 4; ++e) {
+    k1[e] = training ? (float)a[e] * inv_m : 0.0f;
+    k2[e] = training ? (float)b[e] * inv_m : 0.0f;
+  }
+  for (int64_t r = threadIdx.x; r < M; r += BN_SMALL_THREADS) {
+    const f4 tx = ld4(x + r * C + c0, true), td = ld4(dy + r * C + c0, true);
+    f4 ta;
+#pragma unroll
+    for (int e = 0; e < 4; ++e) ta.v[e] = 0.f;
+    if (addend) ta = ld4(addend + r * C + c0, true);
+    float o[4];
+#pragma unroll
+    for (int e = 0; e < 4; ++e)
+      o[e] = bn_bwd_dx(bn_bwd_elem(tx.v[e], td.v[e], acc.k, e, relu), acc.k, e, k1[e], k2[e], training, addend != nullptr,
+                       ta.v[e]);
+    *bn_dx_quad(dx, split, r, C, c0) = make_float4(o[0], o[1], o[2], o[3]);
+  }
+}
+
 constexpr int BN_FIN_CHUNKS = kBnFinChunks;
 
 template <int NT>
@@ -490,6 +536,20 @@
   __shared__ int s_last;
   bn_chunk_centred_stage(partial, nblk, C, M, chunk, mean, var, running_mean, running_var, momentum, ticket,
                          (int)blockIdx.x, (int)gridDim.x, (int)blockIdx.y, red, s_last);
+}
+__global__ __launch_bounds__(256) void bn_stats_chunk_centred_cat_kernel(
+    const float* __restrict__ pa, const float* __restrict__ pb, int nblk, int Ca, int Cb, int64_t M,
+    double* __restrict__ chunk, float* __restrict__ mean, float* __restrict__ var, float* __restrict__ running_mean,
+    float* __restrict__ running_var, float momentum, unsigned* __restrict__ ticket) {
+  __shared__ double red[3][8][33];
+  __shared__ int s_last;
+  const int G = (int)gridDim.x, CGa = Ca >> 5;
+  const bool hb = (int)blockIdx.y >= CGa;
+  const int off = hb ? Ca : 0;
+  bn_chunk_centred_stage(hb ? pb : pa, nblk, hb ? Cb : Ca, M, chunk + (hb ? (int64_t)G * 3 * Ca : 0), mean + off, var + off,
+                         running_mean ? running_mean + off : nullptr, running_var ? running_var + off : nullptr, momentum,
+                         ticket ? ticket + (hb ? CGa : 0) : nullptr, (int)blockIdx.x, G, (int)blockIdx.y - (hb ? CGa : 0), red,
+                         s_last);
 }
 __global__ __launch_bounds__(256) void bn_sum_chunk_kernel(const float* __restrict__ partial, int nblk, int C,
                                                            double* __restrict__ chunk, float* __restrict__ dbeta,
@@ -597,6 +657,66 @@
   bn_apply_body<false>(x, mean, var, gamma, beta, eps, relu, y, M, C);
 }
 
+__global__ void bn_cat_apply_kernel(const float* __restrict__ a, const float* __restrict__ b, int Ca, int Cb,
+                                    const float* __restrict__ mean, const float* __restrict__ var,
+                                    const float* __restrict__ gamma, const float* __restrict__ beta, float eps, int relu,
+                                    float* __restrict__ cat, float* __restrict__ y, int64_t M) {
+  const unsigned C4 = (unsigned)((Ca + Cb) >> 2), Ca4 = (unsigned)(Ca >> 2);
+  const int64_t total4 = M * C4;
+  const int64_t stride = (int64_t)gridDim.x * blockDim.x;
+  int64_t t = blockIdx.x * (int64_t)blockDim.x + threadIdx.x;
+  if (t >= total4) return;
+  const bool fixed_c = (stride % C4) == 0;
+  float sc[4], mu[4], bt[4];
+  const float* src;
+  int64_t u, du;
+  auto at = [&](int64_t q) {
+    const int64_t row = q / C4;
+    const unsigned cg = (unsigned)(q - row * C4);
+    const bool hb = cg >= Ca4;
+    const unsigned Ch4 = hb ? C4 - Ca4 : Ca4;
+    src = hb ? b : a;
+    u = row * Ch4 + (hb ? cg - Ca4 : cg);
+    du = (stride / C4) * Ch4;
+#pragma unroll
+    for (int e = 0; e < 4; ++e) {
+      const int c = (int)cg * 4 + e;
+      sc[e] = bn_fwd_coef(gamma ? gamma[c] : 1.0f, var[c], eps);
+      mu[e] = mean[c];
+      bt[e] = beta ? beta[c] : 0.0f;
+    }
+  };
+  auto body = [&](const float4 v) {
+    float o[4] = {v.x, v.y, v.z, v.w};
+#pragma unroll
+    for (int e = 0; e < 4; ++e) o[e] = bn_fwd_elem(o[e], mu[e], sc[e], bt[e], relu);
+    return make_float4(o[0], o[1], o[2], o[3]);
+  };
+  at(t);
+  if (fixed_c) {
+    for (; t + stride < total4; t += 2 * stride, u += 2 * du) {
+      const float4 v0 = bn_ld4(src, u);
+      const float4 v1 = bn_ld4(src, u + du);
+      bn_st4(cat, t, v0);
+      bn_st4(cat, t + stride, v1);
+      bn_st4(y, t, body(v0));
+      bn_st4(y, t + stride, body(v1));
+    }
+    if (t < total4) {
+      const float4 v = bn_ld4(src, u);
+      bn_st4(cat, t, v);
+      bn_st4(y, t, body(v));
+    }
+  } else {
+    for (; t < total4; t += stride) {
+      at(t);
+      const float4 v = bn_ld4(src, u);
+      bn_st4(cat, t, v);
+      bn_st4(y, t, body(v));
+    }
+  }
+}
+
 template <typename TI, typename TO>
 __global__ void bn_apply_lp_kernel(const TI* __restrict__ x, const float* __restrict__ mean,
                                    const float* __restrict__ var, const float* __restrict__ gamma,
@@ -616,13 +736,13 @@
                        gamma, beta, eps, relu, static_cast<TI*>(y), M, C);
 }
 
-template <bool COHERENT, typename T, typename TO>
+template <bool COHERENT, typename T, typename TO, bool SPLIT = false>
 __device__ __forceinline__ void bn_bwd_apply_body(const T* __restrict__ x, const T* __restrict__ dy,
                                                   const float* __restrict__ mean, const float* __restrict__ var,
                                                   const float* __restrict__ gamma, const float* __restrict__ beta,
                                                   const float* dgamma, const float* dbeta,
                                                   const T* __restrict__ addend, float eps, int relu, int training,
-                                                  TO* __restrict__ dx, int64_t M, int C) {
+                                                  TO* __restrict__ dx, int64_t M, int C, BnSplit split = {}) {
   const int64_t total = M * C;
   const float inv_m = 1.0f / (float)M;
   const bool vec = (C & 3) == 0;
@@ -646,6 +766,20 @@
     }
   };
   if (t < totalw) coef((int)(t % Cw) * W);
+  TO* dq = dx;
+  int64_t u = t, du = stride;
+  auto split_at = [&](int64_t q) {
+    const int64_t row = q / Cw;
+    const unsigned cg = (unsigned)(q - row * Cw), Ca4 = (unsigned)(split.Ca >> 2);
+    const bool hb = cg >= Ca4;
+    const unsigned Ch4 = hb ? Cw - Ca4 : Ca4;
+    dq = hb ? reinterpret_cast<TO*>(split.dx2) : dx;
+    u = row * Ch4 + (hb ? cg - Ca4 : cg);
+    du = (stride / Cw) * Ch4;
+  };
+  if constexpr (SPLIT) {
+    if (t < totalw) split_at(t);
+  }
   auto one = [&](const float (&xv)[4], const float (&dv)[4], const float (&av)[4], float (&ov)[4]) {
 #pragma unroll
     for (int e = 0; e < 4; ++e) {
@@ -655,25 +789,34 @@
   };
   if (vec && fixed_c) {
     for (; t + stride < totalw; t += 2 * stride) {
-      const int64_t u = t + stride;
+      const int64_t t2 = t + stride;
       const f4 tx0 = ld4(x + t * 4, true), td0 = ld4(dy + t * 4, true);
-      const f4 tx1 = ld4(x + u * 4, true), td1 = ld4(dy + u * 4, true);
+      const f4 tx1 = ld4(x + t2 * 4, true), td1 = ld4(dy + t2 * 4, true);
       f4 ta0, ta1;
 #pragma unroll
       for (int e = 0; e < 4; ++e) ta0.v[e] = ta1.v[e] = 0.f;
       if (addend) {
         ta0 = ld4(addend + t * 4, true);
-        ta1 = ld4(addend + u * 4, true);
+        ta1 = ld4(addend + t2 * 4, true);
       }
       float o0[4], o1[4];
       one(tx0.v, td0.v, ta0.v, o0);
       one(tx1.v, td1.v, ta1.v, o1);
-      bn_st4(dx, t, make_float4(o0[0], o0[1], o0[2], o0[3]));
-      bn_st4(dx, u, make_float4(o1[0], o1[1], o1[2], o1[3]));
+      if constexpr (SPLIT) {
+        bn_st4(dq, u, make_float4(o0[0], o0[1], o0[2], o0[3]));
+        bn_st4(dq, u + du, make_float4(o1[0], o1[1], o1[2], o1[3]));
+        u += 2 * du;
+      } else {
+        bn_st4(dx, t, make_float4(o0[0], o0[1], o0[2], o0[3]));
+        bn_st4(dx, t2, make_float4(o1[0], o1[1], o1[2], o1[3]));
+      }
     }
   }
   for (; t < totalw; t += stride) {
-    if (!fixed_c) coef((int)(t % Cw) * W);
+    if (!fixed_c) {
+      coef((int)(t % Cw) * W);
+      if constexpr (SPLIT) split_at(t);
+    }
     float xv[4], dv[4], av[4] = {0.f, 0.f, 0.f, 0.f}, ov[4];
     if (vec) {
       const f4 tx = ld4(x + t * 4, true), td = ld4(dy + t * 4, true);
@@ -693,10 +836,14 @@
       if (addend) av[0] = (float)addend[t];
     }
     one(xv, dv, av, ov);
-    if (vec)
+    if constexpr (SPLIT) {
+      bn_st4(dq, u, make_float4(ov[0], ov[1], ov[2], ov[3]));
+      u += du;
+    } else if (vec) {
       bn_st4(dx, t, make_float4(ov[0], ov[1], ov[2], ov[3]));
-    else
+    } else {
       dx[t] = (TO)ov[0];
+    }
   }
 }
 
@@ -709,6 +856,15 @@
                                     TO* __restrict__ dx, int64_t M, int C) {
   bn_bwd_apply_body<false>(x, dy, mean, var, gamma, beta, dgamma, dbeta, addend, eps, relu, training, dx, M, C);
 }
+__global__ void bn_bwd_apply_split_kernel(const float* __restrict__ x, const float* __restrict__ dy,
+                                          const float* __restrict__ mean, const float* __restrict__ var,
+                                          const float* __restrict__ gamma, const float* __restrict__ beta,
+                                          const float* __restrict__ dgamma, const float* __restrict__ dbeta,
+                                          const float* __restrict__ addend, float eps, int relu, int training,
+                                          float* __restrict__ dx, BnSplit split, int64_t M, int C) {
+  bn_bwd_apply_body<false, float, float, true>(x, dy, mean, var, gamma, beta, dgamma, dbeta, addend, eps, relu, training, dx,
+                                               M, C, split);
+}
 
 constexpr int BN_SF_ROWS = 256;
 
@@ -738,13 +894,14 @@
   }
 }
 
-__global__ __launch_bounds__(256) void bn_small_finish_apply_kernel(
+template <bool CAT>
+__device__ __forceinline__ void bn_small_finish_apply_body(
     const float* __restrict__ partial, int nblk, int C, int64_t M, float* __restrict__ mean, float* __restrict__ var,
     float* __restrict__ running_mean, float* __restrict__ running_var, float momentum, const float* __restrict__ x,
-    const float* __restrict__ gamma, const float* __restrict__ beta, float eps, int relu, float* __restrict__ y, int G) {
+    const float* __restrict__ gamma, const float* __restrict__ beta, float eps, int relu, float* __restrict__ y, int ldy,
+    float* __restrict__ cat, int G, int cgi) {
   __shared__ double red[3][8][33];
   __shared__ float s_mu[32], s_sc[32], s_bt[32];
-  const int cgi = blockIdx.y;
   const int cl = threadIdx.x & 31;
   const int c = cgi * 32 + cl;
   const bool own = (threadIdx.x >> 5) == 0 && c < C;
@@ -777,16 +934,39 @@
       float o[4] = {vx.x, vx.y, vx.z, vx.w};
 #pragma unroll
       for (int e = 0; e < 4; ++e) o[e] = bn_fwd_elem(o[e], mu4[e], sc4[e], bt4[e], relu);
-      *reinterpret_cast<float4*>(y + r * C + c4) = make_float4(o[0], o[1], o[2], o[3]);
-    }
-  }
+      if (CAT) *reinterpret_cast<float4*>(cat + r * ldy + c4) = vx;
+      *reinterpret_cast<float4*>(y + r * ldy + c4) = make_float4(o[0], o[1], o[2], o[3]);
+    }
+  }
+}
+
+__global__ __launch_bounds__(256) void bn_small_finish_apply_kernel(
+    const float* __restrict__ partial, int nblk, int C, int64_t M, float* __restrict__ mean, float* __restrict__ var,
+    float* __restrict__ running_mean, float* __restrict__ running_var, float momentum, const float* __restrict__ x,
+    const float* __restrict__ gamma, const float* __restrict__ beta, float eps, int relu, float* __restrict__ y, int G) {
+  bn_small_finish_apply_body<false>(partial, nblk, C, M, mean, var, running_mean, running_var, momentum, x, gamma, beta, eps,
+                                    relu, y, C, nullptr, G, (int)blockIdx.y);
+}
+
+__global__ __launch_bounds__(256) void bn_small_cat_finish_apply_kernel(
+    const float* __restrict__ pa, const float* __restrict__ pb, int nblk, int Ca, int Cb, int64_t M,
+    float* __restrict__ mean, float* __restrict__ var, float* __restrict__ running_mean, float* __restrict__ running_var,
+    float momentum, const float* __restrict__ a, const float* __restrict__ b, const float* __restrict__ gamma,
+    const float* __restrict__ beta, float eps, int relu, float* __restrict__ cat, float* __restrict__ y, int G) {
+  const int CGa = Ca >> 5;
+  const bool hb = (int)blockIdx.y >= CGa;
+  const int off = hb ? Ca : 0;
+  bn_small_finish_apply_body<true>(hb ? pb : pa, nblk, hb ? Cb : Ca, M, mean + off, var + off,
+                                   running_mean ? running_mean + off : nullptr, running_var ? running_var + off : nullptr,
+                                   momentum, hb ? b : a, gamma ? gamma + off : nullptr, beta ? beta + off : nullptr, eps, relu,
+                                   y + off, Ca + Cb, cat + off, G, (int)blockIdx.y - (hb ? CGa : 0));
 }
 
 __global__ __launch_bounds__(256) void bn_small_bwd_finish_apply_kernel(
     const float* __restrict__ partial, int nblk, int C, int64_t M, const float* __restrict__ x,
     const float* __restrict__ dy, const float* __restrict__ mean, const float* __restrict__ var,
     const float* __restrict__ gamma, const float* __restrict__ beta, const float* __restrict__ addend, float eps, int relu,
-    float* __restrict__ dx, float* __restrict__ dgamma, float* __restrict__ dbeta, int G) {
+    float* __restrict__ dx, BnSplit split, float* __restrict__ dgamma, float* __restrict__ dbeta, int G) {
   __shared__ double red[2][8][33];
   __shared__ float s_k1[32], s_k2[32];
   const int cgi = blockIdx.y;
@@ -831,7 +1011,7 @@
 #pragma unroll
       for (int e = 0; e < 4; ++e)
         ov[e] = bn_bwd_dx(bn_bwd_elem(xv[e], dv[e], k, e, relu), k, e, k1[e], k2[e], 1, addend != nullptr, av[e]);
-      *reinterpret_cast<float4*>(dx + r * C + c4) = make_float4(ov[0], ov[1], ov[2], ov[3]);
+      *bn_dx_quad(dx, split, r, C, c4) = make_float4(ov[0], ov[1], ov[2], ov[3]);
     }
   }
 }
@@ -966,7 +1146,15 @@
 static int launch_bn_bwd_apply(const T* d_x, const T* d_dy, const float* d_mean, const float* d_var,
                                const float* d_gamma, const float* d_beta, const float* d_dgamma, const float* d_dbeta,
                                const T* d_addend, float eps, int relu, int training, TO* d_dx, int64_t M, int C,
-                               hipStream_t st) {
+                               hipStream_t st, BnSplit split = {}) {
+  if constexpr (sizeof(T) == 4 && sizeof(TO) == 4) {
+    if (split.dx2) {
+      hipLaunchKernelGGL(bn_bwd_apply_split_kernel, dim3(bn_apply_grid(M, C)), dim3(256), 0, st, d_x, d_dy, d_mean, d_var,
+                         d_gamma, d_beta, d_dgamma, d_dbeta, d_addend, eps, relu, training, d_dx, split, M, C);
+      WSIS_LAUNCH_CHECK();
+      return WSIS_OK;
+    }
+  }
   hipLaunchKernelGGL((bn_bwd_apply_kernel<T, TO>), dim3(bn_apply_grid(M, C)), dim3(256), 0, st, d_x, d_dy, d_mean, d_var,
                      d_gamma, d_beta, d_dgamma, d_dbeta, d_addend, eps, relu, training, d_dx, M, C);
   WSIS_LAUNCH_CHECK();
@@ -1327,6 +1515,59 @@
   return WSIS_OK;
 }
 
+static bool bn_cat_domain(int Ca, int Cb, std::initializer_list<const void*> rows) {
+  return Ca >= 32 && Cb >= 32 && Ca % 32 == 0 && Cb % 32 == 0 && Ca + Cb <= 512 && bn_aligned16(rows);
+}
+
+int wsis_bn_cat_apply(const float* d_a, const float* d_b, int32_t Ca, int32_t Cb, const float* d_mean, const float* d_var,
+                      const float* d_gamma, const float* d_beta, float eps, int32_t relu, float* d_cat, float* d_y,
+                      int64_t M, void* stream) {
+  WSIS_REQUIRE(M >= 1 && d_a && d_b && d_mean && d_var && d_cat && d_y, "bad args");
+  WSIS_REQUIRE(bn_cat_domain(Ca, Cb, {d_a, d_b, d_cat, d_y}),
+               "concatenation: widths multiples of 32, at most 512 channels, 16-byte aligned tensors");
+  hipLaunchKernelGGL(bn_cat_apply_kernel, dim3(bn_apply_grid(M, Ca + Cb)), dim3(256), 0, as_stream(stream), d_a, d_b, (int)Ca,
+                     (int)Cb, d_mean, d_var, d_gamma, d_beta, eps, (int)relu, d_cat, d_y, M);
+  WSIS_LAUNCH_CHECK();
+  return WSIS_OK;
+}
+
+int wsis_bn_cat_stats_apply(const float* d_partials_a, const float* d_partials_b, int64_t n_part, int64_t M,
+                            const float* d_a, const float* d_b, int32_t Ca, int32_t Cb, float* d_mean, float* d_var,
+                            float* d_running_mean, float* d_running_var, float momentum, const float* d_gamma,
+                            const float* d_beta, float eps, int32_t relu, float* d_cat, float* d_y, void* d_ws,
+                            int64_t ws_bytes, void* d_sync, void* stream) {
+  WSIS_REQUIRE(M >= 1 && d_partials_a && d_partials_b && d_a && d_b && d_mean && d_var && d_cat && d_y, "bad args");
+  WSIS_REQUIRE(n_part == (M + 31) / 32 && n_part < ((int64_t)1 << 31), "one partial per 32-row slice");
+  WSIS_REQUIRE((d_running_mean == nullptr) == (d_running_var == nullptr), "running stats come in pairs");
+  WSIS_REQUIRE(bn_cat_domain(Ca, Cb, {d_a, d_b, d_cat, d_y}),
+               "concatenation: widths multiples of 32, at most 512 channels, 16-byte aligned tensors");
+  const int C = Ca + Cb;
+  hipStream_t st = as_stream(stream);
+  const BnCentredPlan p = bn_centred_plan(n_part, C, d_ws, ws_bytes, d_sync);
+  WSIS_REQUIRE(p.ws_ok, "workspace too small");
+  if (bn_small_fused_ok(p, C, {})) {
+    hipLaunchKernelGGL(bn_small_cat_finish_apply_kernel, dim3((unsigned)ceil_div(M, BN_SF_ROWS), (unsigned)p.CG), dim3(256), 0,
+                       st, d_partials_a, d_partials_b, (int)n_part, (int)Ca, (int)Cb, M, d_mean, d_var, d_running_mean,
+                       d_running_var, momentum, d_a, d_b, d_gamma, d_beta, eps, (int)relu, d_cat, d_y, p.G);
+    WSIS_LAUNCH_CHECK();
+    return WSIS_OK;
+  }
+  hipLaunchKernelGGL(bn_stats_chunk_centred_cat_kernel, dim3(p.G, p.CG), dim3(256), 0, st, d_partials_a, d_partials_b,
+                     (int)n_part, (int)Ca, (int)Cb, M, p.chunk, d_mean, d_var, d_running_mean, d_running_var, momentum,
+                     p.tickets);
+  WSIS_LAUNCH_CHECK();
+  if (p.G > 1 && !p.tickets)
+    for (int h = 0; h < 2; ++h) {
+      const int off = h ? Ca : 0, Ch = h ? Cb : Ca;
+      hipLaunchKernelGGL(bn_stats_final_centred_kernel, dim3((Ch + 3) / 4), dim3(256), 0, st,
+                         p.chunk + (h ? (int64_t)p.G * 3 * Ca : 0), p.G, Ch, M, d_mean + off, d_var + off,
+                         d_running_mean ? d_running_mean + off : nullptr, d_running_var ? d_running_var + off : nullptr,
+                         momentum);
+      WSIS_LAUNCH_CHECK();
+    }
+  return wsis_bn_cat_apply(d_a, d_b, Ca, Cb, d_mean, d_var, d_gamma, d_beta, eps, relu, d_cat, d_y, M, stream);
+}
+
 int wsis_bn_apply_lp(const void* d_x, const float* d_mean, const float* d_var, const float* d_gamma,
                      const float* d_beta, float eps, int32_t relu, void* d_y, int32_t out_fp32, int64_t M, int32_t C,
                      int32_t dtype, void* stream) {
@@ -1348,26 +1589,30 @@
   return WSIS_OK;
 }
 
-int wsis_bn_bwd_from_partials(const float* d_partials, int64_t n_part, const float* d_x, const float* d_dy,
-                              const float* d_mean, const float* d_var, const float* d_gamma, const float* d_beta,
-                              float eps, int32_t relu, float* d_dx, float* d_dgamma, float* d_dbeta,
-                              const float* d_addend, int64_t M, int32_t C, void* d_ws, int64_t ws_bytes, void* d_sync,
-                              void* stream) {
+static bool bn_split_ok(int C, int Ca, std::initializer_list<const void*> ps) {
+  return Ca > 0 && Ca < C && (Ca & 3) == 0 && (C & 3) == 0 && bn_aligned16(ps);
+}
+
+static int bn_bwd_from_partials_run(const float* d_partials, int64_t n_part, const float* d_x, const float* d_dy,
+                                    const float* d_mean, const float* d_var, const float* d_gamma, const float* d_beta,
+                                    float eps, int32_t relu, float* d_dx, BnSplit split, float* d_dgamma, float* d_dbeta,
+                                    const float* d_addend, int64_t M, int32_t C, void* d_ws, int64_t ws_bytes, void* d_sync,
+                                    void* stream) {
   WSIS_REQUIRE(M >= 1 && C >= 1 && d_partials && d_x && d_dy && d_mean && d_var && d_dgamma && d_dbeta, "bad args");
   WSIS_REQUIRE(n_part == (M + 31) / 32 && n_part < ((int64_t)1 << 31), "one partial per 32-row slice");
   const BnCentredPlan p = bn_centred_plan(n_part, C, d_ws, ws_bytes, d_sync);
   WSIS_REQUIRE(p.ws_ok, "workspace too small");
   hipStream_t st = as_stream(stream);
   WSIS_REQUIRE(C <= 512, "more than 512 channels");
-  if (d_dx && bn_small_fused_ok(p, C, {d_x, d_dy, d_dx, d_addend})) {
+  if (d_dx && bn_small_fused_ok(p, C, {d_x, d_dy, d_dx, d_addend, split.dx2})) {
     hipLaunchKernelGGL(bn_small_bwd_finish_apply_kernel, dim3((unsigned)ceil_div(M, BN_SF_ROWS), (unsigned)p.CG), dim3(256),
                        0, st, d_partials, (int)n_part, (int)C, M, d_x, d_dy, d_mean, d_var, d_gamma, d_beta, d_addend, eps,
-                       (int)relu, d_dx, d_dgamma, d_dbeta, p.G);
+                       (int)relu, d_dx, split, d_dgamma, d_dbeta, p.G);
     WSIS_LAUNCH_CHECK();
     return WSIS_OK;
   }
 #if WSIS_EXPERIMENTAL
-  if (const int grid = d_dx && p.tickets ? bn_fused_grid(M, C, p.G * p.CG, 1) : 0) {
+  if (const int grid = d_dx && !split.dx2 && p.tickets ? bn_fused_grid(M, C, p.G * p.CG, 1) : 0) {
     hipLaunchKernelGGL(bn_bwd_finish_apply_kernel, dim3(grid), dim3(256), 0, st, d_partials, (int)n_part, (int)C, p.chunk,
                        p.G, d_dbeta, d_dgamma, static_cast<SyncSlot*>(d_sync), d_x, d_dy, d_mean, d_var, d_gamma, d_beta,
                        d_addend, eps, (int)relu, d_dx, M);
@@ -1384,7 +1629,27 @@
   }
   if (!d_dx) return WSIS_OK;
   return launch_bn_bwd_apply(d_x, d_dy, d_mean, d_var, d_gamma, d_beta, d_dgamma, d_dbeta, d_addend, eps, relu, 1, d_dx, M,
-                             C, st);
+                             C, st, split);
+}
+
+int wsis_bn_bwd_from_partials(const float* d_partials, int64_t n_part, const float* d_x, const float* d_dy,
+                              const float* d_mean, const float* d_var, const float* d_gamma, const float* d_beta,
+                              float eps, int32_t relu, float* d_dx, float* d_dgamma, float* d_dbeta,
+                              const float* d_addend, int64_t M, int32_t C, void* d_ws, int64_t ws_bytes, void* d_sync,
+                              void* stream) {
+  return bn_bwd_from_partials_run(d_partials, n_part, d_x, d_dy, d_mean, d_var, d_gamma, d_beta, eps, relu, d_dx, BnSplit{},
+                                  d_dgamma, d_dbeta, d_addend, M, C, d_ws, ws_bytes, d_sync, stream);
+}
+
+int wsis_bn_bwd_from_partials_split(const float* d_partials, int64_t n_part, const float* d_x, const float* d_dy,
+                                    const float* d_mean, const float* d_var, const float* d_gamma, const float* d_beta,
+                                    float eps, int32_t relu, float* d_dx_a, float* d_dx_b, int32_t Ca, float* d_dgamma,
+                                    float* d_dbeta, const float* d_addend, int64_t M, int32_t C, void* d_ws,
+                                    int64_t ws_bytes, void* d_sync, void* stream) {
+  WSIS_REQUIRE(d_dx_a && d_dx_b && bn_split_ok(C, Ca, {d_x, d_dy, d_dx_a, d_dx_b, d_addend}),
+               "split gradient: 0 < Ca < C, both multiples of 4, 16-byte aligned tensors");
+  return bn_bwd_from_partials_run(d_partials, n_part, d_x, d_dy, d_mean, d_var, d_gamma, d_beta, eps, relu, d_dx_a,
+                                  BnSplit{d_dx_b, Ca}, d_dgamma, d_dbeta, d_addend, M, C, d_ws, ws_bytes, d_sync, stream);
 }
 
 int wsis_bn_bwd_apply(const float* d_x, const float* d_dy, const float* d_mean, const float* d_var,
@@ -1395,17 +1660,47 @@
                              d_dx, M, C, as_stream(stream));
 }
 
+static bool bn_bwd_one_launch(int64_t M, int C, std::initializer_list<const void*> rows) {
+  const char* e = getenv("WSIS_BN_BWD_ONE_LAUNCH");
+  return (!e || atoi(e) != 0) && M <= BN_SMALL_THREADS && M <= bn_small_rows() && (C & 3) == 0 && bn_aligned16(rows);
+}
+
+static int bn_bwd_run(const float* d_x, const float* d_dy, const float* d_mean, const float* d_var, const float* d_gamma,
+                      const float* d_beta, float eps, int32_t relu, int32_t training, float* d_dx, BnSplit split,
+                      float* d_dgamma, float* d_dbeta, const float* d_addend, int64_t M, int32_t C, void* d_ws,
+                      int64_t ws_bytes, void* stream) {
+  WSIS_REQUIRE(M >= 1 && C >= 1 && d_x && d_dy && d_mean && d_var && d_dgamma && d_dbeta && d_ws, "bad args");
+  WSIS_REQUIRE(ws_bytes >= wsis_bn_workspace_bytes(M, C), "workspace too small");
+  hipStream_t st = as_stream(stream);
+  if (d_dx && bn_bwd_one_launch(M, C, {d_x, d_dy, d_dx, d_addend, split.dx2})) {
+    WSIS_REQUIRE(C / 4 <= BN_THREADS, "C > 1024 is not supported");
+    hipLaunchKernelGGL(bn_bwd_small_apply_kernel, dim3(C / 4), dim3(BN_SMALL_THREADS), 0, st, d_x, d_dy, d_mean, d_var,
+                       d_gamma, d_beta, d_addend, eps, (int)relu, (int)training, M, (int)C, d_dx, split, d_dgamma, d_dbeta);
+    WSIS_LAUNCH_CHECK();
+    return WSIS_OK;
+  }
+  const int rc = bn_bwd_reduce_run(d_x, d_dy, d_mean, d_var, d_gamma, d_beta, eps, relu, d_dgamma, d_dbeta, M, C, d_ws, st);
+  if (rc != WSIS_OK || !d_dx) return rc;
+  return launch_bn_bwd_apply(d_x, d_dy, d_mean, d_var, d_gamma, d_beta, d_dgamma, d_dbeta, d_addend, eps, relu, training,
+                             d_dx, M, C, st, split);
+}
+
 int wsis_bn_bwd(const float* d_x, const float* d_dy, const float* d_mean, const float* d_var,
                 const float* d_gamma, const float* d_beta, float eps, int32_t relu, int32_t training,
                 float* d_dx, float* d_dgamma, float* d_dbeta, const float* d_addend, int64_t M, int32_t C, void* d_ws,
                 int64_t ws_bytes, void* stream) {
-  WSIS_REQUIRE(M >= 1 && C >= 1 && d_x && d_dy && d_mean && d_var && d_dgamma && d_dbeta && d_ws, "bad args");
-  WSIS_REQUIRE(ws_bytes >= wsis_bn_workspace_bytes(M, C), "workspace too small");
-  hipStream_t st = as_stream(stream);
-  const int rc = bn_bwd_reduce_run(d_x, d_dy, d_mean, d_var, d_gamma, d_beta, eps, relu, d_dgamma, d_dbeta, M, C, d_ws, st);
-  if (rc != WSIS_OK || !d_dx) return rc;
-  return launch_bn_bwd_apply(d_x, d_dy, d_mean, d_var, d_gamma, d_beta, d_dgamma, d_dbeta, d_addend, eps, relu, training,
-                             d_dx, M, C, st);
+  return bn_bwd_run(d_x, d_dy, d_mean, d_var, d_gamma, d_beta, eps, relu, training, d_dx, BnSplit{}, d_dgamma, d_dbeta,
+                    d_addend, M, C, d_ws, ws_bytes, stream);
+}
+
+int wsis_bn_bwd_split(const float* d_x, const float* d_dy, const float* d_mean, const float* d_var, const float* d_gamma,
+                      const float* d_beta, float eps, int32_t relu, int32_t training, float* d_dx_a, float* d_dx_b,
+                      int32_t Ca, float* d_dgamma, float* d_dbeta, const float* d_addend, int64_t M, int32_t C, void* d_ws,
+                      int64_t ws_bytes, void* stream) {
+  WSIS_REQUIRE(d_dx_a && d_dx_b && bn_split_ok(C, Ca, {d_x, d_dy, d_dx_a, d_dx_b, d_addend}),
+               "split gradient: 0 < Ca < C, both multiples of 4, 16-byte aligned tensors");
+  return bn_bwd_run(d_x, d_dy, d_mean, d_var, d_gamma, d_beta, eps, relu, training, d_dx_a, BnSplit{d_dx_b, Ca}, d_dgamma,
+                    d_dbeta, d_addend, M, C, d_ws, ws_bytes, stream);
 }
 
 int wsis_bn_bwd_lp(const void* d_x, const void* d_dy, const float* d_mean, const float* d_var, const float* d_gamma,
diff --git a/3d-wsis_amd/csrc/executor.hip b/3d-wsis_amd/csrc/executor.hip
--- a/3d-wsis_amd/csrc/executor.hip
+++ b/3d-wsis_amd/csrc/executor.hip
@@ -297,6 +297,7 @@
   bool wt_side;
   bool dw_early;
   bool slab_bn_partials;
+  bool skip_fuse;
   bool prof;
   bool capturing;
   bool dw_defer() const { return dw_batch_reduce && !prof; }
@@ -313,6 +314,7 @@
   const char* rows = getenv("WSIS_DW_EARLY_ROWS");
   o.dw_early = env_flag(getenv("WSIS_DW_EARLY"), dw2_batch_rows() < (rows ? atoll(rows) : 500000));
   o.slab_bn_partials = env_flag(getenv("WSIS_SLAB_BN_PARTIALS"), false);
+  o.skip_fuse = env_flag(getenv("WSIS_SKIP_FUSE"), true);
   o.prof = g_prof_on;
   hipStreamCaptureStatus cs = hipStreamCaptureStatusNone;
   o.capturing = st && (hipStreamIsCapturing(*st, &cs) != hipSuccess || cs != hipStreamCaptureStatusNone);
@@ -449,7 +451,48 @@
   std::vector<int64_t> lp_off, wt_off;
   int64_t dw_max = 0;
   int n_dw = 0;
+  std::vector<int32_t> fused_into;
 };
+
+inline bool skip_ptrs_ok(std::initializer_list<const void*> ps) {
+  for (const void* p : ps)
+    if (!p || (reinterpret_cast<uintptr_t>(p) & 15)) return false;
+  return true;
+}
+inline bool skip_widths_ok(const wsis_op& two, const wsis_op& bn) {
+  return two.Cin >= 32 && two.Cout >= 32 && two.Cin % 32 == 0 && two.Cout % 32 == 0 && bn.Cin == two.Cin + two.Cout &&
+         bn.Cin <= 512 && two.M_in >= 1 && bn.M_in == two.M_in;
+}
+bool cat_bn_fusable(const wsis_op& cat, const wsis_op& bn) {
+  if (cat.kind != WSIS_OP_CAT || bn.kind != WSIS_OP_BN_RELU || is_lp(cat) || is_lp(bn)) return false;
+  if (bn.in[0] != cat.out[0] || !skip_widths_ok(cat, bn)) return false;
+  if (!skip_ptrs_ok({cat.in[0], cat.in[1], cat.out[0], bn.out[0]})) return false;
+  if (bn.flags & (WSIS_OPF_BN_IN | WSIS_OPF_STAT_FIN)) return false;
+  if (bn.flags & WSIS_OPF_TRAINING)
+    return (bn.flags & WSIS_OPF_STATS) && bn.in[5] && bn.in[6] && bn.K == cat.Cin && bn.out[1] && bn.out[2];
+  return bn.in[3] && bn.in[4];
+}
+bool bn_bwd_split_fusable(const wsis_op* ops, int n, int i) {
+  const wsis_op &bn = ops[i], &sp = ops[i + 1];
+  if (bn.kind != WSIS_OP_BN_RELU_BWD || sp.kind != WSIS_OP_SPLIT || is_lp(bn) || is_lp(sp)) return false;
+  if (sp.in[0] != bn.out[0] || !skip_widths_ok(sp, bn)) return false;
+  if (!skip_ptrs_ok({bn.in[0], bn.in[1], bn.out[0], sp.out[0], sp.out[1]}) || (reinterpret_cast<uintptr_t>(bn.in[6]) & 15))
+    return false;
+  for (int j = 0; j < n; ++j) {
+    if (j == i + 1) continue;
+    for (const void* p : ops[j].in)
+      if (p == bn.out[0]) return false;
+    if (ops[j].kind == WSIS_OP_ADD && ops[j].out[0] == bn.out[0]) return false;
+  }
+  return true;
+}
+void plan_skip_fusions(const wsis_op* ops, int n, bool on, std::vector<int32_t>& fused_into) {
+  fused_into.assign(n, -1);
+  for (int i = 0; on && i + 1 < n; ++i) {
+    if (cat_bn_fusable(ops[i], ops[i + 1])) fused_into[i] = i + 1;
+    if (bn_bwd_split_fusable(ops, n, i)) fused_into[i + 1] = i;
+  }
+}
 
 struct PassRun {
   const wsis_op* ops;
@@ -473,6 +516,8 @@
 
   char* region(int k) const { return base + plan.at[k]; }
   const float* wt_of(int i) const { return reinterpret_cast<const float*>(region(PassPlan::WT) + plan.wt_off[i]); }
+  const wsis_op* fused_cat(int i) const { return i > 0 && plan.fused_into[i - 1] == i ? ops + i - 1 : nullptr; }
+  const wsis_op* fused_split(int i) const { return i + 1 < n && plan.fused_into[i + 1] == i ? ops + i + 1 : nullptr; }
   int start();
   int fork_weight_transposes();
   int await_transposes_before(int i);
@@ -889,6 +934,7 @@
     p.bytes[k] = sizes[k];
     p.total += sizes[k];
   }
+  plan_skip_fusions(ops, n, o.skip_fuse && p.bytes[PassPlan::DEEP] == 0, p.fused_into);
   return WSIS_OK;
 }
 
@@ -1148,6 +1194,18 @@
                             op.eps, relu_of(op), op.out[0], (op.flags & WSIS_OPF_OUT_F32) ? 1 : 0, op.M_in, op.Cin,
                             op.reserved, r.stream);
   }
+  if (const wsis_op* cat = r.fused_cat(i)) {
+    if (!training)
+      return wsis_bn_cat_apply((const float*)cat->in[0], (const float*)cat->in[1], cat->Cin, cat->Cout, (const float*)op.in[3],
+                               (const float*)op.in[4], (const float*)op.in[1], (const float*)op.in[2], op.eps, relu_of(op),
+                               (float*)cat->out[0], (float*)op.out[0], op.M_in, r.stream);
+    const bool upd = (op.flags & WSIS_OPF_UPDATE_RUNNING) != 0;
+    return wsis_bn_cat_stats_apply((const float*)op.in[5], (const float*)op.in[6], (op.M_in + 31) / 32, op.M_in,
+                                   (const float*)cat->in[0], (const float*)cat->in[1], cat->Cin, cat->Cout, (float*)op.out[1],
+                                   (float*)op.out[2], upd ? (float*)op.in[3] : nullptr, upd ? (float*)op.in[4] : nullptr,
+                                   op.momentum, (const float*)op.in[1], (const float*)op.in[2], op.eps, relu_of(op),
+                                   (float*)cat->out[0], (float*)op.out[0], r.ws, r.ws_bytes, sync_slot(r.d_sync, i), r.stream);
+  }
   if (training) {
     bool applied = false;
     const int rc = bn_training_stats(r, op, i, &applied);
@@ -1260,6 +1318,7 @@
 
 int issue_bn_relu_bwd(PassRun& r, const wsis_op& op, int i) {
   ProfScope prof(2, r.st);
+  const wsis_op* split = r.fused_split(i);
   int rc;
   if (is_lp(op)) {
     rc = op.M_in <= 0 ? WSIS_OK
@@ -1271,12 +1330,25 @@
   } else if ((op.flags & WSIS_OPF_STATS) && !r.bn_unfused[i]) {
     if (!op.in[7] || !(op.flags & WSIS_OPF_TRAINING))
       rc = fail(WSIS_ERR_ARG, "op %d: BatchNorm backward from partials needs in[7] and training mode", i);
+    else if (split)
+      rc = wsis_bn_bwd_from_partials_split((const float*)op.in[7], (op.M_in + 31) / 32, (const float*)op.in[0],
+                                           (const float*)op.in[1], (const float*)op.in[2], (const float*)op.in[3],
+                                           (const float*)op.in[4], (const float*)op.in[5], op.eps, relu_of(op),
+                                           (float*)split->out[0], (float*)split->out[1], split->Cin, (float*)op.out[1],
+                                           (float*)op.out[2], (const float*)op.in[6], op.M_in, op.Cin, r.ws, r.ws_bytes,
+                                           sync_slot(r.d_sync, i), r.stream);
     else
       rc = wsis_bn_bwd_from_partials((const float*)op.in[7], (op.M_in + 31) / 32, (const float*)op.in[0],
                                      (const float*)op.in[1], (const float*)op.in[2], (const float*)op.in[3],
                                      (const float*)op.in[4], (const float*)op.in[5], op.eps, relu_of(op), (float*)op.out[0],
                                      (float*)op.out[1], (float*)op.out[2], (const float*)op.in[6], op.M_in, op.Cin, r.ws,
                                      r.ws_bytes, sync_slot(r.d_sync, i), r.stream);
+  } else if (split) {
+    rc = wsis_bn_bwd_split((const float*)op.in[0], (const float*)op.in[1], (const float*)op.in[2], (const float*)op.in[3],
+                           (const float*)op.in[4], (const float*)op.in[5], op.eps, relu_of(op),
+                           (op.flags & WSIS_OPF_TRAINING) ? 1 : 0, (float*)split->out[0], (float*)split->out[1], split->Cin,
+                           (float*)op.out[1], (float*)op.out[2], (const float*)op.in[6], op.M_in, op.Cin, r.ws, r.ws_bytes,
+                           r.stream);
   } else {
     rc = wsis_bn_bwd((const float*)op.in[0], (const float*)op.in[1], (const float*)op.in[2], (const float*)op.in[3],
                      (const float*)op.in[4], (const float*)op.in[5], op.eps, relu_of(op),
@@ -1288,6 +1360,7 @@
 }
 
 int issue_op(PassRun& r, const wsis_op& op, int i) {
+  if (r.plan.fused_into[i] >= 0) return WSIS_OK;
   switch (op.kind) {
     case WSIS_OP_CONV: return issue_conv(r, op, i);
     case WSIS_OP_BN_RELU: return issue_bn_relu(r, op, i);
@@ -1310,6 +1383,7 @@
   int err = plan_pass(ops, n, r.opt, r.plan);
   if (err != WSIS_OK) return err;
   WSIS_REQUIRE((n == 0 || ws_bytes >= r.plan.total) && (d_ws || n == 0), "workspace too small");
+  if (mark_op >= 0 && r.plan.fused_into[mark_op] > mark_op) r.plan.fused_into[mark_op] = -1;
   r.base = static_cast<char*>(d_ws);
   r.ws = r.region(PassPlan::OP);
   r.ws_bytes = ws_bytes - r.plan.at[PassPlan::OP];
@@ -1364,6 +1438,15 @@
   out[10] = plan.total;
   std::copy(plan.lp_off.begin(), plan.lp_off.end(), out + 11);
   std::copy(plan.wt_off.begin(), plan.wt_off.end(), out + 11 + n);
+  return WSIS_OK;
+}
+
+int wsis_debug_skip_fusions(const wsis_op* ops, int32_t n, int32_t* out) {
+  WSIS_REQUIRE((ops || n == 0) && n >= 0 && out, "bad arguments");
+  PassPlan plan;
+  const int rc = plan_pass(ops, n, read_pass_options(nullptr), plan);
+  if (rc != WSIS_OK) return rc;
+  std::copy(plan.fused_into.begin(), plan.fused_into.end(), out);
   return WSIS_OK;
 }
 
diff --git a/3d-wsis_amd/wsis_native/__init__.py b/3d-wsis_amd/wsis_native/__init__.py
--- a/3d-wsis_amd/wsis_native/__init__.py
+++ b/3d-wsis_amd/wsis_native/__init__.py
@@ -103,6 +103,11 @@
     "wsis_bn_bwd_lp": (I32, [P, P, P, P, P, P, F32, I32, I32, P, I32, P, P, P, I64, I32, I32, P, I64, P]),
     "wsis_bn_bwd": (I32, [P, P, P, P, P, P, F32, I32, I32, P, P, P, P, I64, I32, P, I64, P]),
     "wsis_bn_bwd_apply_lp": (I32, [P, P, P, P, P, P, P, P, F32, I32, P, I32, P, I64, I32, I32, P]),
+    "wsis_bn_cat_apply": (I32, [P, P, I32, I32, P, P, P, P, F32, I32, P, P, I64, P]),
+    "wsis_bn_cat_stats_apply": (I32, [P, P, I64, I64, P, P, I32, I32, P, P, P, P, F32, P, P, F32, I32, P, P, P, I64, P, P]),
+    "wsis_bn_bwd_from_partials_split": (I32, [P, I64, P, P, P, P, P, P, F32, I32, P, P, I32, P, P, P, I64, I32, P, I64, P,
+                                              P]),
+    "wsis_bn_bwd_split": (I32, [P, P, P, P, P, P, F32, I32, I32, P, P, I32, P, P, P, I64, I32, P, I64, P]),
     "wsis_bn_sync_pack": (I32, [P, P, I64, I32, P, P]),
     "wsis_bn_sync_combine": (I32, [P, I32, I32, P, P, P, P, F32, P, P]),
     "wsis_bn_sync_sums_pack": (I32, [P, P, I32, P, P]),
diff --git a/include/wsis_hip.h b/include/wsis_hip.h
--- a/include/wsis_hip.h
+++ b/include/wsis_hip.h
@@ -194,6 +194,23 @@
                               float eps, int32_t relu, float* d_dx, float* d_dgamma, float* d_dbeta,
                               const float* d_addend, int64_t M, int32_t C, void* d_ws, int64_t ws_bytes, void* d_sync,
                               void* stream);
+int wsis_bn_cat_apply(const float* d_a, const float* d_b, int32_t Ca, int32_t Cb, const float* d_mean, const float* d_var,
+                      const float* d_gamma, const float* d_beta, float eps, int32_t relu, float* d_cat, float* d_y,
+                      int64_t M, void* stream);
+int wsis_bn_cat_stats_apply(const float* d_partials_a, const float* d_partials_b, int64_t n_part, int64_t M,
+                            const float* d_a, const float* d_b, int32_t Ca, int32_t Cb, float* d_mean, float* d_var,
+                            float* d_running_mean, float* d_running_var, float momentum, const float* d_gamma,
+                            const float* d_beta, float eps, int32_t relu, float* d_cat, float* d_y, void* d_ws,
+                            int64_t ws_bytes, void* d_sync, void* stream);
+int wsis_bn_bwd_from_partials_split(const float* d_partials, int64_t n_part, const float* d_x, const float* d_dy,
+                                    const float* d_mean, const float* d_var, const float* d_gamma, const float* d_beta,
+                                    float eps, int32_t relu, float* d_dx_a, float* d_dx_b, int32_t Ca, float* d_dgamma,
+                                    float* d_dbeta, const float* d_addend, int64_t M, int32_t C, void* d_ws,
+                                    int64_t ws_bytes, void* d_sync, void* stream);
+int wsis_bn_bwd_split(const float* d_x, const float* d_dy, const float* d_mean, const float* d_var, const float* d_gamma,
+                      const float* d_beta, float eps, int32_t relu, int32_t training, float* d_dx_a, float* d_dx_b,
+                      int32_t Ca, float* d_dgamma, float* d_dbeta, const float* d_addend, int64_t M, int32_t C, void* d_ws,
+                      int64_t ws_bytes, void* stream);
 int wsis_bn_apply(const float* d_x, const float* d_mean, const float* d_var, const float* d_gamma,
                   const float* d_beta, float eps, int32_t relu, float* d_y, int64_t M, int32_t C, void* stream);
 int wsis_bn_apply_lp(const void* d_x, const float* d_mean, const float* d_var, const float* d_gamma,
```

Result: no change. 135.7 scenes/s, median of 4 (+1.4%).
